# fortunalab/avida

Hardware: AMD Instinct MI355X
Metric: organism-instructions/sec + updates/sec, 1M-org logic-9 world, 1/8 GPUs (higher is better)
Workload: dtype int32; 1 GPU; configs[2]: 1024x1024 torus per GPU, logic-9, default avida.cfg mutation rates, births on, seeded with the detail-50000.pop evolved genotypes (classic instset); environment=logic9, world=1024x1024x1, burn_in_updates=150, organisms=1040165, parallelism=strips1, transport=none, ranks=1, sub_updates=0, stats_every_update=False

## Files before the change

avida_amd/csrc/births.h:

```cpp
#pragma once
#include "device.h"

namespace {

__device__ __forceinline__ int neighbours(const DevWorld& W, int cell, int* out) {
  const int X = W.world_x, R = W.rows;
  const int x = cell % X, y = cell / X;
  int n = 0;
  for (int dy = -1; dy <= 1; dy++)
    for (int dx = -1; dx <= 1; dx++) {
      if (dx == 0 && dy == 0) continue;
      int nx = x + dx, ny = y + dy;
      if (W.geometry == 1) {
        if (nx < 0 || nx >= X) continue;
      } else {
        nx = (nx + X) % X;
      }
      if (ny >= 0 && ny < R) {
        out[n++] = ny * X + nx;
      } else if (!W.tiled) {
        if (W.geometry == 1) continue;
        ny = (ny + R) % R;
        out[n++] = ny * X + nx;
      } else {
        const int gy = W.row0 + ny;
        if (W.geometry == 1 && (gy < 0 || gy >= W.global_rows)) continue;
        out[n++] = (int)W.n + (ny < 0 ? 0 : X) + nx;
      }
    }
  return n;
}

__device__ __forceinline__ void edit_back(int ew, int& src, int& val) {
  if (ew == 0 || val >= 0) return;
  const int kind = ew & 7, a = (ew >> 3) & 0xFFF, b = (ew >> 15) & 0xFFF;
  if (kind == 2) {
    if (src == a) val = b;
  } else if (kind == 3) {
    if (src == a) val = b; else if (src > a) src--;
  } else if (kind == 4) {
    if (src >= a) src++;
  }
}
__device__ __forceinline__ void slip_back(int ew, int sfm, const int32_t* fill, int& src, int& val) {
  if (ew == 0 || val >= 0) return;
  const int a = (ew >> 3) & 0xFFF, b = (ew >> 15) & 0xFFF;
  if (a > b && src >= a && src < 2 * a - b) {
    if (sfm == 4) { val = AVGPU_H_NOP_C; return; }
    if (sfm == 2 && fill) { val = fill[src - a]; return; }
    if (sfm == 3 && fill) { src = fill[src - a]; return; }
  }
  if (src >= a) src = b + (src - a);
}
__device__ __forceinline__ void trans_back(int w0, int w1, const int32_t* fill, int& src, int val) {
  if (val >= 0) return;
  const int ins = (w0 >> 3) & 0xFFF, to = (w0 >> 15) & 0xFFF, L = w1 - to;
  if (L > 0) {
    if (src >= ins + L) src -= L;
    else if (src >= ins) src = fill ? fill[src - ins] : to + (src - ins);
  } else if (L < 0 && src >= ins) {
    src -= L;
  }
}
__device__ __forceinline__ int mut_source(int j, const int* e, int sfm, int tfm, int& val, const int32_t* subs,
                                          const int* pofs, const int* pcnt) {
  constexpr int first[5] = {SEG_OSLIP, SEG_PMUT, SEG_PINS, SEG_PDEL, SEG_SMUT};
  constexpr int last[5] = {SEG_STRANS, SEG_PMUT, SEG_PINS, SEG_PDEL, SEG_SUNI};
  const bool sdata = sfm == 2 || sfm == 3;
  const int tw = tfm == 1 ? 3 : 2;
  int src = j;
  val = -1;
#pragma unroll
  for (int k = 4; k >= 0; k--) {
#pragma unroll
    for (int g = last[k]; g >= first[k]; g--) {
      if (g >= SEG_TTRANS && g <= SEG_STRANS) {
        for (int i = pcnt[g] - tw; i >= 0 && val < 0; i -= tw) {
          const int fo = tw == 3 ? subs[pofs[g] + i + 2] : -1;
          trans_back(subs[pofs[g] + i], subs[pofs[g] + i + 1], fo >= 0 ? subs + fo : nullptr, src, val);
        }
      } else if (g <= SEG_SSLIP && sdata) {
        for (int i = pcnt[g] - 2; i >= 0 && val < 0; i -= 2) {
          const int fo = subs[pofs[g] + i + 1];
          slip_back(subs[pofs[g] + i], sfm, fo >= 0 ? subs + fo : nullptr, src, val);
        }
      } else if (g <= SEG_SSLIP) {
        for (int i = pcnt[g] - 1; i >= 0 && val < 0; i--) slip_back(subs[pofs[g] + i], sfm, nullptr, src, val);
      } else {
        for (int i = pcnt[g] - 1; i >= 0 && val < 0; i--) edit_back(subs[pofs[g] + i], src, val);
      }
    }
    if (k == 0) slip_back(e[0], sfm, nullptr, src, val);
    else edit_back(e[k], src, val);
  }
  return src;
}

__device__ __forceinline__ void wave_lds_sync() {
  __builtin_amdgcn_fence(__ATOMIC_RELEASE, "workgroup");
  __builtin_amdgcn_wave_barrier();
  __builtin_amdgcn_fence(__ATOMIC_ACQUIRE, "workgroup");
}

__device__ __forceinline__ void apply_edits_core(const DevWorld& W, int64_t r, const int* e, int len0, int len,
                                                 uint8_t* child) {
  const int lane = threadIdx.x & 63;
  const int sfm = W.slip_fill_mode, tfm = W.trans_fill_mode;
  int pofs[NSEG], pcnt[NSEG], np = 0;
#pragma unroll
  for (int k = 0; k < NSEG; k++) {
    pofs[k] = W.seg_any ? W.b_pofs[(int64_t)k * W.rcap + r] : 0;
    pcnt[k] = W.seg_any ? W.b_pcnt[(int64_t)k * W.rcap + r] : 0;
    np |= pcnt[k];
  }
  if ((e[0] | e[1] | e[2] | e[3] | e[4] | np) == 0) return;
  uint32_t* g32 = reinterpret_cast<uint32_t*>(W.b_genome + r * TAPE_SLOT);
  uint32_t* c32 = reinterpret_cast<uint32_t*>(child);
  for (int w = lane; (w << 2) < len0; w += 64) c32[w] = g32[w];
  wave_lds_sync();
  for (int w = lane; (w << 2) < len; w += 64) {
    uint32_t word = 0;
#pragma unroll
    for (int k = 0; k < 4; k++) {
      const int j = 4 * w + k;
      int val;
      const int src = mut_source(j, e, sfm, tfm, val, W.b_subs, pofs, pcnt);
      const uint32_t v = val >= 0 ? (uint32_t)val : (uint32_t)child[src];
      word |= (j < len ? v : 0u) << (8 * k);
    }
    g32[w] = word;
  }
  wave_lds_sync();
}
__device__ __forceinline__ void apply_edits_wave(const DevWorld& W, int64_t r, uint8_t* child) {
  int e[5];
#pragma unroll
  for (int k = 0; k < 5; k++) e[k] = W.b_edit[(int64_t)k * W.rcap + r];
  apply_edits_core(W, r, e, W.b_len0[r], W.b_len[r], child);
}

struct Child {
  int len, gen, ccopied, exec, gest;
  double merit, fitness;
  uint32_t lo, hi, ctr;
  const int32_t* ltask;
  int64_t lstride;
  const int32_t* inputs = nullptr;
  uint32_t hs = 0;
};
template <int G>
__device__ __forceinline__ void setup_child(const DevWorld& W, int64_t c, const Child& b,
                                            const uint32_t* src, int lane) {
  static_assert(G == 32 || G == 64, "group = wave or half-wave");
  const int64_t N = W.n;
  const int len = b.len;
  uint32_t* dst = reinterpret_cast<uint32_t*>(W.tape + c * TAPE_SLOT);
  uint64_t gsum = 0;
  for (int w = lane; w < (len + 3) / 4; w += G) {
    const uint32_t v = src[w];
    dst[w] = v;
    gsum += gk_word(v, w, len);
  }
  for (int off = G / 2; off > 0; off >>= 1) gsum += __shfl_xor(gsum, off);
  if (lane == 0) W.gkey[c] = gk_final(gsum, len);
  switch (lane) {
    case 0: W.ctl[c] = CTL_ALIVE | CTL_FRESH | (b.hs << CTL_HS_SHIFT); break;
    case 1: W.mem_size[c] = len; break;
    case 2: {
      int mx = 0;
      if (W.death_method > 0) { mx = W.age_limit; if (W.death_method == 2) mx *= len; if (mx < 1) mx = 1; }
      W.max_exec[c] = mx;
      break; }
    case 3: W.birth_len[c] = len; break;
    case 4: W.merit[c] = b.merit; break;
    case 5: W.fitness[c] = b.fitness; break;
    case 6: W.credit[c] = 0.0; break;
    case 7: W.gest_time[c] = b.gest; break;
    case 8: W.generation[c] = b.gen; break;
    case 9: W.copied[c] = b.ccopied; break;
    case 10: W.executed[c] = b.exec; break;
    case 11: {
      uint32_t ctr = b.ctr;
      if (b.inputs) {
        W.inputs[c] = b.inputs[0]; W.inputs[N + c] = b.inputs[1]; W.inputs[2 * N + c] = b.inputs[2];
      } else {
        W.inputs[c] = (15 << 24) + (int)rng_below(b.lo, b.hi, ctr, 1u << 24);
        W.inputs[N + c] = (51 << 24) + (int)rng_below(b.lo, b.hi, ctr, 1u << 24);
        W.inputs[2 * N + c] = (85 << 24) + (int)rng_below(b.lo, b.hi, ctr, 1u << 24);
      }
      W.rng[c] = b.lo; W.rng[N + c] = b.hi; W.rng[2 * N + c] = ctr;
      if (W.rec_off) W.rec_off[c] = -1;
      break; }
    case 12 + AVGPU_NUM_LOGIC_TASKS: if (W.track_age) W.age[c] = 0; break;
    default:
      if (lane >= 12 && lane < 12 + AVGPU_NUM_LOGIC_TASKS)
        W.last_task[(int64_t)(lane - 12) * N + c] = b.ltask[(int64_t)(lane - 12) * b.lstride];
      break;
  }
}

__device__ __forceinline__ void child_quad(uint4 v, int k, int len, uint4* __restrict__ d4, uint64_t& gsum) {
  const int w = 4 * k;
  uint32_t x[4] = {v.x, v.y, v.z, v.w};
#pragma unroll
  for (int j = 0; j < 4; j++) {
    const int keep = len - 4 * (w + j);
    if (keep <= 0) x[j] = 0u;
    else { if (keep < 4) x[j] &= (1u << (8 * keep)) - 1u; gsum += gk_word(x[j], w + j, len); }
  }
  d4[k] = make_uint4(x[0], x[1], x[2], x[3]);
}
template <int PRE = 0>
__device__ __forceinline__ void setup_child_lane(const DevWorld& W, int64_t c, const Child& b,
                                                 const uint8_t* __restrict__ src, const uint4* pre = nullptr) {
  const int64_t N = W.n;
  const int len = b.len;
  const uint4* __restrict__ s4 = reinterpret_cast<const uint4*>(src);
  uint4* __restrict__ d4 = reinterpret_cast<uint4*>(W.tape + c * TAPE_SLOT);
  uint64_t gsum = 0;
  const int nq = (len + 15) >> 4;
#pragma unroll
  for (int u = 0; u < PRE; u++)
    if (u < nq) child_quad(pre[u], u, len, d4, gsum);
  for (int k0 = PRE; k0 < nq; k0 += 4) {
    uint4 v[4];
#pragma unroll
    for (int u = 0; u < 4; u++)
      if (k0 + u < nq) v[u] = s4[k0 + u];
#pragma unroll
    for (int u = 0; u < 4; u++) {
      if (k0 + u >= nq) break;
      child_quad(v[u], k0 + u, len, d4, gsum);
    }
  }
  W.gkey[c] = gk_final(gsum, len);
  W.ctl[c] = CTL_ALIVE | CTL_FRESH | (b.hs << CTL_HS_SHIFT);
  W.mem_size[c] = len;
  int mx = 0;
  if (W.death_method > 0) { mx = W.age_limit; if (W.death_method == 2) mx *= len; if (mx < 1) mx = 1; }
  W.max_exec[c] = mx;
  W.birth_len[c] = len;
  if (W.track_age) W.age[c] = 0;
  W.merit[c] = b.merit;
  W.fitness[c] = b.fitness;
  W.credit[c] = 0.0;
  W.gest_time[c] = b.gest;
  W.generation[c] = b.gen;
  W.copied[c] = b.ccopied;
  W.executed[c] = b.exec;
  uint32_t ctr = b.ctr;
  W.inputs[c] = (15 << 24) + (int)rng_below(b.lo, b.hi, ctr, 1u << 24);
  W.inputs[N + c] = (51 << 24) + (int)rng_below(b.lo, b.hi, ctr, 1u << 24);
  W.inputs[2 * N + c] = (85 << 24) + (int)rng_below(b.lo, b.hi, ctr, 1u << 24);
  W.rng[c] = b.lo; W.rng[N + c] = b.hi; W.rng[2 * N + c] = ctr;
  if (W.rec_off) W.rec_off[c] = -1;
#pragma unroll
  for (int q = 0; q < AVGPU_NUM_LOGIC_TASKS; q++)
    W.last_task[(int64_t)q * N + c] = b.ltask[(int64_t)q * b.lstride];
}

__device__ __forceinline__ Child child_of_record(const DevWorld& W, int64_t i) {
  Child b;
  const int4* row = reinterpret_cast<const int4*>(W.b_inh + i * BI_WORDS);
  const int4 q0 = row[0], q1 = row[1], q2 = row[2];
  static_assert(BI_MERIT == 0 && BI_GEN == 4 && BI_RLO == 8 && BI_LTASK == 12, "b_inh row layout");
  b.len = W.b_len[i];
  b.merit = __hiloint2double(q0.y, q0.x); b.fitness = __hiloint2double(q0.w, q0.z);
  b.gen = q1.x; b.ccopied = q1.y; b.exec = q1.z; b.gest = q1.w;
  b.lo = (uint32_t)q2.x; b.hi = (uint32_t)q2.y; b.ctr = (uint32_t)q2.z;
  b.hs = 0x10000u - BI_TIME(q2.w);
  b.ltask = W.b_inh + i * BI_WORDS + BI_LTASK; b.lstride = 1;
  return b;
}

}
```

avida_amd/csrc/capi.hip:

```cpp
#include <hip/hip_runtime.h>

#include <algorithm>
#include <chrono>
#include <cmath>
#include <cstdio>
#include <cstdlib>
#include <cstring>
#include <string>
#include <type_traits>
#include <vector>

#include "device.h"

namespace {

thread_local std::string g_err;

int fail(int code, const std::string& msg) {
  g_err = msg;
  return code;
}

#define HIPCHK(x)                                                                   \
  do {                                                                              \
    hipError_t _e = (x);                                                            \
    if (_e != hipSuccess) return fail(AVGPU_EHIP, std::string(#x ": ") + hipGetErrorString(_e)); \
  } while (0)
#define COPY_SYNC(ww, dst, src, bytes, kind)                                        \
  do {                                                                              \
    HIPCHK(hipMemcpyAsync((dst), (src), (bytes), (kind), (ww)->stream));           \
    HIPCHK(hipStreamSynchronize((ww)->stream));                                     \
  } while (0)
#define SET_SYNC(ww, dst, val, bytes)                                               \
  do {                                                                              \
    HIPCHK(hipMemsetAsync((dst), (val), (bytes), (ww)->stream));                    \
    HIPCHK(hipStreamSynchronize((ww)->stream));                                     \
  } while (0)

}

struct avgpu_world {
  avgpu_cfg cfg;
  int device = 0;
  hipStream_t stream = nullptr;
  hipStream_t own_stream = nullptr;
  static const int RING = 512;
  hipEvent_t ring[RING][NUM_CLASSES + 1] = {};
  int ring_head = 0, ring_count = 0;
  int time_every = 1;
  int64_t interp_calls = 0;
  double acc_ms = 0.0;
  double acc_class_ms[NUM_CLASSES] = {};
  int64_t acc_phases = 0;
  DevWorld W;
  DevWorld* d_W = nullptr;
  DevWorld* d_Wv[2] = {};
  DevWorld pushedv[2];
  bool validv[2] = {false, false};
  int cur_w = 0;
  DevWorld* h_stage = nullptr;
  hipEvent_t ev_stage[2] = {};
  std::vector<void*> allocs;
  int n_ops = 0;
  uint8_t op2code[256];
  int16_t code2op[64];
  bool instset_loaded = false;
  int res_geom[AVGPU_MAX_RESOURCES] = {};
  std::vector<avgpu_resource> res_spec;
  std::vector<avgpu_cell_resource> cell_spec;
  bool env_loaded = false;
  double* d_totals = nullptr;
  double* d_stats = nullptr;
  bool stats_stale = false;
  bool use_global = false;
  int64_t update = 0;
  float last_kernel_ms = 0.f;
  int64_t last_launches = 0;
  bool has_test_buffers = false;
  double* rec_buf = nullptr;
  double* srec_buf[2] = {nullptr, nullptr};
  int ntiles_last = 0;
  bool tile_buffers = false;
  long long* h_pred = nullptr;
  long long* d_pred = nullptr;
  bool pred_pending = false;
  long long pred_seq = 0;
  bool reaper_rebuild = false;
  long long pred_acc = 0, pred_n = 0, pred_cnt = 0;
  int last_k = 1;
  int tile_sub = 0, tile_k = 1, tile_sub_next = 0;
  uint32_t tile_key = 0;
  GtScratch gt = {};
  bool gt_ready = false;
  avgpu_genotype* gt_rows = nullptr;
  int64_t gt_rows_cap = 0;
  hipEvent_t ev_gt[4] = {};
  double gt_ms = 0.0;
  int64_t gt_bytes = 0;
  ArbScratch arb = {};
  bool arb_ready = false;
  int64_t arb_n = 0;
  avgpu_arbiter_summary arb_last = {};
  hipEvent_t ev_arb[4] = {};
  double arb_ms = 0.0;
  int64_t arb_bytes = 0;
  avgpu_world* land = nullptr;
  LandScratch land_s = {};
  int64_t land_chunk = 65536;
  hipEvent_t ev_land[2] = {};
  double land_ms = 0.0;
  int64_t land_mutants = 0, land_runs = 0;

  template <typename T>
  int alloc(T** p, size_t count) {
    void* q = nullptr;
    size_t bytes = std::max<size_t>(count * sizeof(T), 16);
    hipError_t e = hipMalloc(&q, bytes);
    if (e != hipSuccess) return fail(AVGPU_ENOMEM, std::string("hipMalloc: ") + hipGetErrorString(e));
    hipMemsetAsync(q, 0, bytes, stream);
    allocs.push_back(q);
    *p = reinterpret_cast<T*>(q);
    return 0;
  }
};

namespace {

int setup_world(avgpu_world* w, int64_t n, bool test_buffers) {
  DevWorld& W = w->W;
  memset(&W, 0, sizeof(W));
  W.n = n;
  const avgpu_cfg& c = w->cfg;
  int rc = 0;
#define A(ptr, cnt) if ((rc = w->alloc(&W.ptr, (size_t)(cnt))) < 0) return rc
  A(xs, (size_t)n * XS_WORDS); A(ctl, n); A(mem_size, n); A(max_exec, n); A(age, n); A(birth_len, n); A(gkey, n); A(rng, 3 * n);
  A(budget, n); A(aclass, n); A(tape, (size_t)n * TAPE_SLOT);
  A(inputs, 3 * n); A(last_task, AVGPU_MAX_REACTIONS * n);
  A(cur_react, AVGPU_MAX_REACTIONS * n);
  A(merit, n); A(fitness, n); A(credit, n); A(gest_time, n); A(num_div, n);
  A(generation, n); A(copied, n); A(child_copied, n); A(executed, n);
  HIPCHK(hipMemsetAsync(W.aclass, ACLASS_NONE, n, w->stream));
  A(class_list, NUM_LISTS * n); A(order, n); A(sub_hist, (size_t)((n + 4095) / 4096) * SORT_BUCKETS); A(class_count, CLASS_COUNT_WORDS); A(counters, CNT_WORDS);
  W.rcap = n + (test_buffers ? 16 : std::max<int64_t>(4096, n / 4));
  const int64_t R = W.rcap;
  A(b_count, BQ_WORDS); A(b_list, n); A(b_parent, R); A(b_seq, R); A(b_len, R); A(b_len0, R); A(b_edit, 5 * R);
  const double pmeans[5] = {c.divide_poisson_slip_mean, c.divide_poisson_mut_mean,
                            c.divide_poisson_ins_mean, c.divide_poisson_del_mean, c.divide_poisson_trans_mean};
  const double psite[6] = {c.div_mut_prob, c.div_ins_prob, c.div_del_prob, c.div_uniform_prob, c.div_slip_prob,
                           c.div_trans_prob};
  const bool sdata = c.slip_fill_mode == 2 || c.slip_fill_mode == 3, tdata = c.trans_fill_mode == 1;
  const double eslip = c.divide_slip_prob + c.divide_poisson_slip_mean + c.div_slip_prob * AVGPU_MAX_GENOME;
  const double etrans = c.divide_trans_prob + c.divide_poisson_trans_mean + c.div_trans_prob * AVGPU_MAX_GENOME;
  bool pois = false, site = c.divide_trans_prob > 0.0 || (sdata && eslip > 0.0);
  for (int q = 0; q < 5; q++) pois = pois || pmeans[q] > 0.0;
  for (int q = 0; q < 6; q++) site = site || psite[q] > 0.0;
  if (pois || site) {
    const int tw = tdata ? 3 : 2, sw = sdata ? 2 : 1;
    int64_t k = 16 + tw + sw;
    for (int q = 0; q < 6; q++)
      if (psite[q] > 0.0)
        k += (q == 5 ? tw : (q == 4 ? sw : 1)) * ((int64_t)std::ceil(AVGPU_MAX_GENOME * std::min(1.0, psite[q]) * 3.0) + 16);
    for (int q = 0; q < 5; q++)
      if (pmeans[q] > 0.0) k += (q == 4 ? tw : (q == 0 ? sw : 1)) * ((int64_t)std::ceil(3.0 * std::min(pmeans[q], 4096.0)) + 16);
    const double efill = (AVGPU_MAX_GENOME / 4.0) / 6.0 * (1.0 + 1.0 / 32.0) + 2.0;
    if (sdata && eslip > 0.0) k += (int64_t)std::ceil(3.0 * std::min(eslip, 4096.0) * efill) + 16;
    if (tdata && etrans > 0.0) k += (int64_t)std::ceil(3.0 * std::min(etrans, 4096.0) * efill) + 16;
    k = std::min<int64_t>(k, (int64_t)INT32_MAX / R);
    W.scap = R * k;
    A(b_subs, W.scap); A(b_pofs, NSEG * R); A(b_pcnt, NSEG * R);
  }
  W.seg_any = (pois || site) ? 1 : 0;
  W.pois_any = pois ? 1 : 0;
  for (int q = 0; q < 5; q++) W.pois_L[q] = pmeans[q] > 0.0 ? std::exp(-pmeans[q]) : 0.0;
  A(b_inh, (size_t)BI_WORDS * R); A(b_target, R); A(b_state, R);
  A(b_prio, R); A(b_genome, (size_t)R * TAPE_SLOT);
  const int64_t ng = n + 2 * (int64_t)c.world_x;
  A(occ, ng); A(claim, ng); A(claim2, ng); A(owner, ng); A(killt, n); A(sdone, n); A(ran, n); A(sched, SCHED_WORDS); A(pacc, NSHARD * PACC_STRIDE);
  W.claim_r[0] = W.claim; W.claim_r[1] = W.claim2;
  A(claim_r[2], ng); A(claim_r[3], ng); A(b_tgt, 4 * R);
  if (c.birth_method == 4) {
    A(e_list, n); A(e_blk, (n + 255) / 256 + 1); A(soup_perm, n);
    std::vector<int32_t> iota((size_t)n);
    for (int64_t i = 0; i < n; i++) iota[(size_t)i] = (int32_t)i;
    HIPCHK(hipMemcpyAsync(W.soup_perm, iota.data(), (size_t)n * sizeof(int32_t), hipMemcpyHostToDevice,
                          w->stream));
    HIPCHK(hipStreamSynchronize(w->stream));
  }
  if (test_buffers) {
    A(t_flags, (size_t)n * TAPE_SLOT); A(t_flags_len, n); A(t_child, (size_t)n * TAPE_SLOT);
    A(t_child_len, n);
  }
  A(rand_cum, 64); A(rand_code, 64); A(task_lut, 256); A(rand_lut, 256);
  A(react_tab, AVGPU_MAX_REACTIONS * RT_STRIDE); A(task_tab, 32);
  A(react_res, AVGPU_MAX_REACTIONS * RR_STRIDE); A(res_param, AVGPU_MAX_RESOURCES);
  A(res_global, AVGPU_MAX_RESOURCES); A(res_cons, AVGPU_MAX_RESOURCES);
  if ((rc = w->alloc(&w->d_Wv[0], 1)) || (rc = w->alloc(&w->d_Wv[1], 1))) return rc;
  w->d_W = w->d_Wv[0];
  w->validv[0] = w->validv[1] = false;
  const int64_t nb = (n + 255) / 256;
  if ((rc = w->alloc(&w->d_totals, (size_t)totals_words(nb)))) return rc;
  W.totals = w->d_totals;
  if ((rc = w->alloc(&W.blk_count, (size_t)nb))) return rc;
  W.tree_cap = 1;
  while (W.tree_cap < nb) W.tree_cap <<= 1;
  if ((rc = w->alloc(&W.tree_scr, (size_t)(2 * W.tree_cap)))) return rc;
  if ((rc = w->alloc(&W.tree_cnt, (size_t)(2 * W.tree_cap)))) return rc;
  if ((rc = w->alloc(&w->d_stats, (size_t)stats_words(nb)))) return rc;
#undef A
  w->has_test_buffers = test_buffers;
  W.world_x = c.world_x; W.world_y = c.world_y; W.geometry = c.world_geometry;
  W.ave_time_slice = c.ave_time_slice; W.slicing = c.slicing_method;
  W.base_merit_method = c.base_merit_method; W.base_const_merit = c.base_const_merit;
  W.default_bonus = c.default_bonus; W.size_range = c.offspring_size_range;
  W.min_copied_lines = c.min_copied_lines; W.min_exe_lines = c.min_exe_lines;
  W.merit_default_bonus = c.merit_default_bonus; W.required_bonus = c.required_bonus;
  W.inherit_merit = c.inherit_merit; W.require_allocate = c.require_allocate;
  W.alloc_method = c.alloc_method; W.max_label_exe = c.max_label_exe_size;
  W.cfg_min_genome = c.min_genome_size; W.cfg_max_genome = c.max_genome_size;
  W.max_genome = (!c.max_genome_size || c.max_genome_size > AVGPU_MAX_GENOME) ? AVGPU_MAX_GENOME : c.max_genome_size;
  W.min_genome = (!c.min_genome_size || c.min_genome_size < AVGPU_MIN_GENOME) ? AVGPU_MIN_GENOME : c.min_genome_size;
  W.death_method = c.death_method; W.age_limit = c.age_limit;
  W.prefer_empty = c.prefer_empty; W.allow_parent = c.allow_parent; W.birth_method = c.birth_method;
  auto th = [](double p) -> uint64_t {
    if (!(p > 0.0)) return 0;
    if (p >= 1.0) return 1ull << 32;
    return (uint64_t)std::ceil(p * 4294967296.0);
  };
  W.th_copy_mut = th(c.copy_mut_prob);
  W.th_copy_ins = th(c.copy_ins_prob); W.p_copy_ins = c.copy_ins_prob;
  W.th_copy_del = th(c.copy_del_prob); W.p_copy_del = c.copy_del_prob;
  W.th_copy_uni = th(c.copy_uniform_prob); W.p_copy_uni = c.copy_uniform_prob;
  W.th_copy_slip = th(c.copy_slip_prob); W.p_copy_slip = c.copy_slip_prob;
  W.copy_ext = (W.th_copy_ins || W.th_copy_del || W.th_copy_uni || W.th_copy_slip) ? 1 : 0;
  W.th_div_mut = th(c.divide_mut_prob);
  W.th_div_ins = th(c.divide_ins_prob);
  W.th_div_del = th(c.divide_del_prob);
  W.th_div_slip = th(c.divide_slip_prob);
  W.th_div_uni = th(c.divide_uniform_prob);
  W.p_copy_mut = c.copy_mut_prob; W.p_div_mut = c.divide_mut_prob; W.p_div_ins = c.divide_ins_prob;
  W.p_div_del = c.divide_del_prob; W.p_div_slip = c.divide_slip_prob; W.p_div_uni = c.divide_uniform_prob;
  W.th_div_site = th(c.div_mut_prob);
  W.p_div_site = c.div_mut_prob;
  W.th_dsite[0] = th(c.div_ins_prob); W.p_dsite[0] = c.div_ins_prob;
  W.th_dsite[1] = th(c.div_del_prob); W.p_dsite[1] = c.div_del_prob;
  W.th_dsite[2] = th(c.div_uniform_prob); W.p_dsite[2] = c.div_uniform_prob;
  W.th_dsite[3] = th(c.div_slip_prob); W.p_dsite[3] = c.div_slip_prob;
  W.th_dsite[4] = th(c.div_trans_prob); W.p_dsite[4] = c.div_trans_prob;
  W.th_dtrans = th(c.divide_trans_prob); W.p_dtrans = c.divide_trans_prob;
  W.th_par_site = th(c.parent_mut_prob);
  W.p_par_site = c.parent_mut_prob;
  W.th_par_ins = th(c.parent_ins_prob); W.p_par_ins = c.parent_ins_prob;
  W.th_par_del = th(c.parent_del_prob); W.p_par_del = c.parent_del_prob;
  W.slip_fill_mode = c.slip_fill_mode;
  W.trans_fill_mode = c.trans_fill_mode;
  W.slip_copy_mode = c.slip_copy_mode;
  W.track_age = (c.birth_method == 1 || c.birth_method == 2) ? 1 : 0;
  W.rec = nullptr; W.rec_n = 0; W.rec_off = nullptr;
  W.seed_lo = (uint32_t)c.seed;
  W.seed_hi = (uint32_t)(c.seed >> 32);
  W.slow_batch = env_int("AVGPU_SLOW_BATCH", 12, 1, 64);
  W.nb_slow_batch = env_int("AVGPU_NB_SLOW_BATCH", 1, 1, 64);
  W.ioq_slow_batch = env_int("AVGPU_IOQ_SLOW_BATCH", 6, 1, 64);
  W.row0 = 0;
  W.global_rows = c.world_y;
  W.rows = c.world_y;
  W.tiled = 0;
  W.cell0 = 0;
  static const int sets[9][6] = {
      {15, 51, 85, -1, -1, -1}, {63, 95, 119, -1, -1, -1}, {136, 160, 192, -1, -1, -1},
      {175, 187, 207, 221, 243, 245}, {238, 250, 252, -1, -1, -1}, {10, 12, 34, 48, 68, 80},
      {3, 5, 17, -1, -1, -1}, {60, 90, 102, -1, -1, -1}, {153, 165, 195, -1, -1, -1}};
  uint16_t lut[256] = {0};
  for (int t = 0; t < 9; t++)
    for (int k = 0; k < 6; k++)
      if (sets[t][k] >= 0) lut[sets[t][k]] |= (uint16_t)(1u << t);
  HIPCHK(hipMemcpyAsync(W.task_lut, lut, sizeof(lut), hipMemcpyHostToDevice, w->stream));
  HIPCHK(hipStreamSynchronize(w->stream));
  return 0;
}

std::string unsupported_cfg(const avgpu_cfg& c) {
  auto nz = [](double v) { return v != 0.0; };
  const bool slips = nz(c.divide_slip_prob) || nz(c.divide_poisson_slip_mean) || nz(c.div_slip_prob);
  if (slips && (c.slip_fill_mode < 0 || c.slip_fill_mode == 1 || c.slip_fill_mode > 4))
    return "SLIP_FILL_MODE 1 (nop-X) or an unknown mode";
  if (nz(c.copy_slip_prob) && c.slip_copy_mode != 0 && c.slip_copy_mode != 1)
    return "SLIP_COPY_MODE other than 0 (read-head jump) and 1 (memory slip)";
  if (nz(c.copy_slip_prob) && c.slip_copy_mode == 1 && c.slip_fill_mode != 0 && c.slip_fill_mode != 2 &&
      c.slip_fill_mode != 4)
    return "SLIP_COPY_MODE 1 with SLIP_FILL_MODE other than 0 (duplication), 2 (random), 4 (nop-C)";
  if ((nz(c.divide_trans_prob) || nz(c.divide_poisson_trans_mean) || nz(c.div_trans_prob)) &&
      (c.trans_fill_mode < 0 || c.trans_fill_mode > 1))
    return "TRANS_FILL_MODE other than 0 (duplication) / 1 (scrambled)";
  if (c.divide_poisson_slip_mean > 700.0 || c.divide_poisson_mut_mean > 700.0 ||
      c.divide_poisson_ins_mean > 700.0 || c.divide_poisson_del_mean > 700.0 ||
      c.divide_poisson_trans_mean > 700.0)
    return "DIVIDE_POISSON_*_MEAN above 700 (exp(-mean) underflows)";
  if (c.divide_method != 1) return "DIVIDE_METHOD other than 1 (split)";
  if (c.sub_updates < 0 || c.sub_updates > 64) return "sub_updates outside 0..64";
  if (c.sub_updates > 1 && c.slicing_method != 1) return "sub_updates > 1 with SLICING_METHOD other than 1";
  if (c.world_geometry != 1 && c.world_geometry != 2) return "WORLD_GEOMETRY other than 1 (grid) or 2 (torus)";
  if (c.slicing_method < 0 || c.slicing_method > 2) return "SLICING_METHOD other than 0, 1, 2";
  if (c.base_merit_method < 0 || c.base_merit_method > 5) return "BASE_MERIT_METHOD other than 0..5";
  if (c.birth_method < 0 || c.birth_method > 5)
    return "BIRTH_METHOD other than 0 (random neighbour), 1 (oldest), 2 (highest age / merit), 3 (empty only), "
           "4 (whole-world soup), 5 (eldest, serial world)";
  if ((c.birth_method == 1 || c.birth_method == 2) && !c.prefer_empty)
    return "BIRTH_METHOD 1 / 2 without PREFER_EMPTY (the reference reads the organism of an empty cell)";
  if (c.death_method < 0 || c.death_method > 2) return "DEATH_METHOD other than 0, 1, 2";
  if (c.alloc_method != 0 && c.alloc_method != 2) return "ALLOC_METHOD other than 0 (default) and 2 (random)";
  if (nz(c.point_mut_prob) || nz(c.point_ins_prob) || nz(c.point_del_prob) || nz(c.inst_point_mut_prob))
    return "POINT_MUT_PROB / POINT_INS_PROB / POINT_DEL_PROB / INST_POINT_MUT_PROB (cosmic-ray mutations)";
  if (nz(c.div_lgt_prob) || nz(c.divide_lgt_prob) || nz(c.divide_poisson_lgt_mean))
    return "DIV_LGT_PROB / DIVIDE_LGT_PROB / DIVIDE_POISSON_LGT_MEAN (lateral gene transfer)";
  if (nz(c.inject_mut_prob) || nz(c.inject_ins_prob) || nz(c.inject_del_prob)) return "INJECT_*_PROB";
  if (nz(c.meta_copy_mut) || nz(c.meta_std_dev)) return "META_COPY_MUT / META_STD_DEV";
  if (nz(c.death_prob)) return "DEATH_PROB";
  if (c.age_deviation != 0) return "AGE_DEVIATION";
  if (c.divide_failure_resets != 0) return "DIVIDE_FAILURE_RESETS";
  if (c.special_mut_line >= 0) return "SPECIAL_MUT_LINE";
  if (c.population_cap > 0) return "POPULATION_CAP";
  if (c.generation_inc_method != 1) return "GENERATION_INC_METHOD other than 1";
  if (c.reset_inputs_on_divide != 0) return "RESET_INPUTS_ON_DIVIDE";
  if (c.epigenetic_method != 0) return "EPIGENETIC_METHOD";
  if (c.min_cycles != 0) return "MIN_CYCLES";
  if (c.required_task < -1 || c.immunity_task < -1 || c.required_reaction < -1 || c.immunity_reaction < -1 ||
      c.required_task >= AVGPU_MAX_REACTIONS || c.immunity_task >= AVGPU_MAX_REACTIONS ||
      c.required_reaction >= 12 || c.immunity_reaction >= 12)
    return "REQUIRED_TASK / IMMUNITY_TASK outside the task library, REQUIRED_REACTION / IMMUNITY_REACTION "
           "beyond reaction 11";
  if (c.require_exact_copy != 0) return "REQUIRE_EXACT_COPY";
  if (c.fitness_method != 0) return "FITNESS_METHOD other than 0";
  if (c.juv_period != 0) return "JUV_PERIOD";
  if (c.no_mut_insts_len < 0 || c.no_mut_insts_len > 63 ||
      (size_t)c.no_mut_insts_len != strnlen(c.no_mut_insts, sizeof(c.no_mut_insts)))
    return "NO_MUT_INSTS longer than 63 symbols, or no_mut_insts_len not its length";
  if (c.test_fitness_measures != 0) return "REVERT_* / STERILIZE_* (Divide_TestFitnessMeasures1)";
  return std::string();
}

avgpu_world* create_world(const avgpu_cfg* cfg, int device, int64_t n, bool test_buffers) {
  if (!cfg) { fail(AVGPU_EINVAL, "cfg is NULL"); return nullptr; }
  {
    const std::string why = unsupported_cfg(*cfg);
    if (!why.empty()) {
      fail(AVGPU_EUNSUPPORTED, why + " is not on the GPU path");
      return nullptr;
    }
  }
  if (hipSetDevice(device) != hipSuccess) { fail(AVGPU_EHIP, "hipSetDevice failed"); return nullptr; }
  avgpu_world* w = new avgpu_world();
  w->cfg = *cfg;
  w->device = device;
  if (n <= 0) n = (int64_t)cfg->world_x * cfg->world_y;
  if (n <= 0 || n > (1ll << 30)) { delete w; fail(AVGPU_EINVAL, "bad cell count"); return nullptr; }
  if (hipStreamCreateWithFlags(&w->own_stream, hipStreamNonBlocking) != hipSuccess ||
      hipHostMalloc((void**)&w->h_pred, PRED_WORDS * sizeof(long long), hipHostMallocMapped | hipHostMallocCoherent) !=
          hipSuccess ||
      hipHostMalloc((void**)&w->h_stage, 2 * sizeof(DevWorld), hipHostMallocDefault) != hipSuccess ||
      hipEventCreateWithFlags(&w->ev_stage[0], hipEventDisableTiming) != hipSuccess ||
      hipEventCreateWithFlags(&w->ev_stage[1], hipEventDisableTiming) != hipSuccess ||
      hipHostGetDevicePointer((void**)&w->d_pred, w->h_pred, 0) != hipSuccess) {
    delete w; fail(AVGPU_EHIP, "stream/event creation failed"); return nullptr;
  }
  for (int k = 0; k < PRED_WORDS; k++) w->h_pred[k] = 0;
  w->stream = w->own_stream;
  for (int i = 0; i < avgpu_world::RING; i++) {
    for (int k = 0; k <= NUM_CLASSES; k++)
      if (hipEventCreate(&w->ring[i][k]) != hipSuccess) {
        fail(AVGPU_EHIP, "event creation failed"); return nullptr;
      }
  }
  for (int i = 0; i < 64; i++) w->code2op[i] = -1;
  if (setup_world(w, n, test_buffers) < 0) {
    std::string e = g_err;
    avgpu_destroy(w);
    g_err = e;
    return nullptr;
  }
  return w;
}

int copy_tables(avgpu_world* dst, const avgpu_world* src) {
  DevWorld& D = dst->W;
  const DevWorld& S = src->W;
  D.n_ops = S.n_ops; D.rand_total = S.rand_total; D.fill_code = S.fill_code;
  D.n_react = S.n_react;
  D.env_simple = S.env_simple; D.env_react_mask = S.env_react_mask; D.env_once_mask = S.env_once_mask;
  D.no_mut_mask = S.no_mut_mask;
  D.req_task = S.req_task; D.imm_task = S.imm_task; D.req_react = S.req_react; D.imm_react = S.imm_react;
  D.single_react = S.single_react; D.max_task_cnt = S.max_task_cnt; D.div_req = S.div_req;
  HIPCHK(hipStreamSynchronize(src->stream));
  HIPCHK(hipMemcpyAsync(D.task_tab, S.task_tab, 32 * sizeof(double), hipMemcpyDeviceToDevice, dst->stream));
  HIPCHK(hipMemcpyAsync(D.react_tab, S.react_tab, AVGPU_MAX_REACTIONS * RT_STRIDE * sizeof(int32_t),
                        hipMemcpyDeviceToDevice, dst->stream));
  HIPCHK(hipMemcpyAsync(D.rand_lut, S.rand_lut, 256, hipMemcpyDeviceToDevice, dst->stream));
  HIPCHK(hipMemcpyAsync(D.rand_cum, S.rand_cum, 64 * sizeof(int32_t), hipMemcpyDeviceToDevice, dst->stream));
  HIPCHK(hipMemcpyAsync(D.rand_code, S.rand_code, 64, hipMemcpyDeviceToDevice, dst->stream));
  HIPCHK(hipStreamSynchronize(dst->stream));
  dst->n_ops = src->n_ops;
  memcpy(dst->op2code, src->op2code, sizeof(dst->op2code));
  memcpy(dst->code2op, src->code2op, sizeof(dst->code2op));
  dst->instset_loaded = src->instset_loaded;
  dst->env_loaded = src->env_loaded;
  return 0;
}

int ready(avgpu_world* w) {
  if (!w) return fail(AVGPU_EINVAL, "NULL world");
  if (!w->instset_loaded) return fail(AVGPU_ESTATE, "avgpu_load_instset not called");
  if (!w->env_loaded) return fail(AVGPU_ESTATE, "avgpu_load_env not called");
  return 0;
}

int batch_ready(avgpu_world* w) {
  const int rc = ready(w);
  if (rc < 0) return rc;
  if (w->cfg.birth_method == 5)
    return fail(AVGPU_EUNSUPPORTED, "BIRTH_METHOD 5 (the reaper queue) runs on the serial world only");
  return 0;
}

int translate_genomes(avgpu_world* w, const uint8_t* genomes, const int32_t* lens, int64_t count,
                      std::vector<uint8_t>& codes, std::vector<int32_t>& offsets) {
  codes.clear();
  offsets.resize(count);
  size_t off = 0;
  for (int64_t i = 0; i < count; i++) {
    const int len = lens[i];
    if (len < 1 || len > AVGPU_MAX_GENOME) return fail(AVGPU_EINVAL, "genome length out of range");
    offsets[i] = (int32_t)codes.size();
    for (int k = 0; k < len; k++) {
      const uint8_t op = genomes[off + k];
      if (op >= w->n_ops) return fail(AVGPU_EINVAL, "genome op outside instruction set");
      codes.push_back(w->op2code[op]);
    }
    off += len;
    while (codes.size() & 3) codes.push_back(0);
  }
  if (codes.empty()) codes.push_back(0);
  return 0;
}

int reaper_read(avgpu_world* w, std::vector<int32_t>& q) {
  const DevWorld& W = w->W;
  int64_t ix[2];
  COPY_SYNC(w, ix, W.reaper_ix, sizeof(ix), hipMemcpyDeviceToHost);
  std::vector<int32_t> ring((size_t)W.reaper_cap);
  COPY_SYNC(w, ring.data(), W.reaper, ring.size() * sizeof(int32_t), hipMemcpyDeviceToHost);
  if (ix[1] < ix[0] || ix[1] - ix[0] > W.reaper_cap) return fail(AVGPU_ESTATE, "reaper queue indices");
  q.clear();
  for (int64_t p = ix[0]; p < ix[1]; p++) q.push_back(ring[(size_t)(p % W.reaper_cap)]);
  return 0;
}
int reaper_write(avgpu_world* w, const std::vector<int32_t>& q) {
  const DevWorld& W = w->W;
  if ((int64_t)q.size() > W.reaper_cap) return fail(AVGPU_EUNSUPPORTED, "reaper queue longer than 2n + 64");
  std::vector<int32_t> ring((size_t)W.reaper_cap, 0);
  std::copy(q.begin(), q.end(), ring.begin());
  const int64_t ix[2] = {W.reaper_cap, W.reaper_cap + (int64_t)q.size()};
  COPY_SYNC(w, W.reaper, ring.data(), ring.size() * sizeof(int32_t), hipMemcpyHostToDevice);
  COPY_SYNC(w, W.reaper_ix, ix, sizeof(ix), hipMemcpyHostToDevice);
  return 0;
}

int reaper_build(avgpu_world* w) {
  const DevWorld& W = w->W;
  std::vector<uint32_t> ctl((size_t)W.n);
  COPY_SYNC(w, ctl.data(), W.ctl, (size_t)W.n * sizeof(uint32_t), hipMemcpyDeviceToHost);
  std::vector<int32_t> q;
  for (int64_t c = 0; c < W.n; c++) q.push_back((int32_t)c);
  for (int64_t c = 0; c < W.n; c++) if (ctl[(size_t)c] & CTL_ALIVE) q.push_back((int32_t)c);
  w->reaper_rebuild = false;
  return reaper_write(w, q);
}

int set_orgs_impl(avgpu_world* w, int64_t first, int64_t count, const uint8_t* genomes,
                  const int32_t* lens, const double* merits, const int32_t* inputs, int det) {
// ... 1982 lines not shown
```

avida_amd/csrc/device.h:

```cpp
#pragma once

#include <hip/hip_runtime.h>
#include <stdint.h>
#include <stdlib.h>

#include "../../include/avida_gpu.h"

#define TAPE_SLOT 2048
enum { BI_MERIT = 0, BI_FITNESS = 2, BI_GEN = 4, BI_CCOPIED = 5, BI_EXEC = 6, BI_GEST = 7,
       BI_RLO = 8, BI_RHI = 9, BI_RCTR = 10, BI_FINAL = 11, BI_LTASK = 12, BI_WORDS = 32 };
#define BI_TIME(w) ((uint32_t)(w) >> 16)
#define CODE_MASK 0x3F
#define TF_COPIED 0x40
#define TF_EXEC 0x80
#define CODE_ERROR 0x3F

#define CTL_SP0(c) ((c) & 0xF)
#define CTL_SP1(c) (((c) >> 4) & 0xF)
#define CTL_CURSTK 0x100u
#define CTL_MAL 0x200u
#define CTL_ALIVE 0x400u
#define CTL_FRESH 0x800u
#define CTL_SPECDIE 0x1000u
#define CTL_HS_SHIFT 14
#define CTL_HS(c) (((c) >> CTL_HS_SHIFT) & 0x1FFFFu)
#define CTL_HS_MASK (0x1FFFFu << CTL_HS_SHIFT)

#define NUM_CLASSES 4
#define ACLASS_NONE 0xFF
#define RR_STRIDE 8
enum { RR_RES = 0, RR_SPATIAL = 1, RR_DEPL = 2, RR_TYPE = 3, RR_FRAC = 4, RR_MIN = 5, RR_MAX = 6, RR_VALUE = 7 };
#define RES_FIX 4294967296.0

struct ResParam {
  int32_t geometry, slot;
  int32_t in_x1, in_x2, in_y1, in_y2, out_x1, out_x2, out_y1, out_y2;
  double in_share;
  double sink_frac;
  double xdiffuse, ydiffuse, xgravity, ygravity;
  double decay100, inflow100;
  double decay99, inflow99;
  int32_t flows, has_sink;
  int32_t in_all, out_all;
};
#define NUM_LISTS 7
#define RT_STRIDE 12
enum { RT_TASK = 0, RT_TYPE = 1, RT_MIN = 2, RT_MAX = 3, RT_HASREQ = 4, RT_USED = 5, RT_MULT = 6, RT_ADD = 8 };
#define BUDGET_PRIM 0x40000000

enum : int {
  XS_REG = 0,
  XS_HEAD = 3,
  XS_RLABEL = 7,
  XS_CYCLES = 8,
  XS_TIME = 9,
  XS_GEST = 10,
  XS_ERRORS = 11,
  XS_INBUF = 12,
  XS_INTOT = 15,
  XS_INPTR = 16,
  XS_OUTBUF = 17,
  XS_OUTTOT = 18,
  XS_BONUS = 20,
  XS_TASK = 22,
  XS_STACK = 32,
  XS_REACT = 52,
  XS_NREACT = 12,
  XS_WORDS = 64
};

struct DevWorld {
  int64_t n;
  int32_t* xs;
  uint32_t* ctl;
  int32_t* mem_size;
  int32_t* max_exec;
  int32_t* birth_len;
  uint64_t* gkey;
  uint32_t* rng;
  int32_t* budget;
  uint8_t* aclass;
  uint8_t* tape;
  int32_t* inputs;
  int32_t* last_task;
  int32_t* cur_react;
  double* merit;
  double* fitness;
  double* credit;
  int32_t* gest_time;
  int32_t* num_div;
  int32_t* generation;
  int32_t* copied;
  int32_t* child_copied;
  int32_t* executed;
  int32_t* class_list;
  int32_t* order;
  int32_t* class_count;
  unsigned long long* counters;
  int64_t rcap;
  int32_t* b_count;
  int32_t* b_list;
  int32_t* b_parent;
  uint32_t* b_seq;
  int32_t* b_len;
  int32_t* b_len0;
  int32_t* b_edit;
  int32_t* b_subs;
  int64_t scap;
  int32_t* b_pofs;
  int32_t* b_pcnt;
  int32_t* b_inh;
  int32_t* b_target;
  int8_t* b_state;
  unsigned long long* b_prio;
  uint8_t* b_genome;
  uint8_t* occ;
  unsigned long long* claim;
  unsigned long long* claim2;
  unsigned long long* claim_r[4];
  int32_t* b_tgt;
  int32_t* owner;
  uint32_t* killt;
  int64_t* blk_count;
  double* tree_scr;
  int64_t* tree_cnt;
  int64_t tree_cap;
  int32_t* sdone;
  uint8_t* t_flags;
  int32_t* t_flags_len;
  uint8_t* t_child;
  int32_t* t_child_len;
  int32_t* rand_cum;
  uint8_t* rand_code;
  uint16_t* task_lut;
  int n_ops;
  int32_t rand_total;
  uint8_t* rand_lut;
  int32_t slow_batch;
  int32_t nb_slow_batch;
  int32_t ioq_slow_batch;
  int n_react;
  int32_t* react_tab;
  int32_t env_simple;
  uint32_t env_react_mask;
  uint32_t env_once_mask;
  uint32_t env_res_mask;
  double* task_tab;
  int32_t n_res, n_cellres, env_resources;
  struct ResParam* res_param;
  double* res_amount;
  double* res_delta;
  double* res_global;
  unsigned long long* res_cons;
  avgpu_cell_resource* res_cells;
  double* react_res;
  int8_t res_spatial_host[AVGPU_MAX_RESOURCES];
  int8_t res_flows_host[AVGPU_MAX_RESOURCES];
  int8_t res_cells_host[AVGPU_MAX_RESOURCES];
  int8_t res_grav_host[AVGPU_MAX_RESOURCES];
  double* res_amount_alt;
  int8_t res_first;
  int32_t n_spatial;
  double* rs_send[2];
  double* rs_recv[2];
  uint8_t fill_code;
  int32_t world_x, world_y, geometry;
  int32_t ave_time_slice, slicing;
  int32_t base_merit_method, base_const_merit;
  double default_bonus, size_range, min_copied_lines, min_exe_lines;
  double merit_default_bonus, required_bonus;
  int32_t inherit_merit, require_allocate, alloc_method, max_label_exe;
  int32_t min_genome, max_genome;
  int32_t cfg_min_genome, cfg_max_genome;
  int32_t death_method, age_limit;
  int32_t prefer_empty, allow_parent, birth_method;
  uint64_t th_copy_mut, th_div_mut, th_div_ins, th_div_del, th_div_slip, th_div_uni;
  double p_copy_mut, p_div_mut, p_div_ins, p_div_del, p_div_slip, p_div_uni;
  uint64_t th_copy_ins, th_copy_del, th_copy_uni, th_copy_slip;
  double p_copy_ins, p_copy_del, p_copy_uni, p_copy_slip;
  int32_t copy_ext;
  uint64_t no_mut_mask;
  int32_t req_task, imm_task, req_react, imm_react, single_react, max_task_cnt, div_req;
  uint64_t th_div_site;
  double p_div_site;
  uint64_t th_par_site;
  double p_par_site;
  uint64_t th_par_ins, th_par_del;
  double p_par_ins, p_par_del;
  double pois_L[5];
  int32_t pois_any;
  uint64_t th_dsite[5];
  double p_dsite[5];
  uint64_t th_dtrans;
  double p_dtrans;
  int32_t seg_any;
  int32_t slip_fill_mode;
  int32_t trans_fill_mode;
  int32_t slip_copy_mode;
  const double* rec;
  int64_t rec_n;
  int64_t* rec_off;
  double* stree;
  int64_t stree_size;
  int32_t* spec;
  uint32_t* grng;
  uint32_t* sctx;
  uint8_t* face;
  const double* srec_sched;
  int64_t srec_sched_n;
  const double* srec_ctx;
  int64_t srec_ctx_n;
  uint32_t seed_lo, seed_hi;
  int32_t row0, global_rows, rows, tiled;
  int64_t cell0;
  uint8_t* h_send[2];
  uint8_t* h_recv[2];
  uint8_t* r_send[2];
  uint8_t* r_recv[2];
  int64_t r_arena;
  int32_t* age;
  int32_t track_age;
  int32_t* sub_hist;
  int32_t* e_list;
  int32_t* e_blk;
  int32_t* soup_perm;
  int32_t* reaper;
  int64_t* reaper_ix;
  int64_t reaper_cap;
  int32_t* ran;
  double* cons;
  long long* sched;
  long long* pacc;
  const double* totals;
};
static_assert(sizeof(DevWorld) == 1664, "DevWorld's size");


enum {
  TOT_WEIGHT = 0,
  TOT_ORGS = 1,
  TOT_HANDED = 2,
  TOT_DIV = 2,
  TOT_UD = 3,
  TOT_WORDS = 8
};
__host__ __device__ inline int64_t totals_words(int64_t nb) { return TOT_WORDS + 2 * nb; }

enum {
  SCHED_CARRY = 1,
  SCHED_CARRY_REM = 2,
  SCHED_UD = 4,
  SCHED_WORDS = 12
};

enum {
  PACC_WEIGHT = 0,
  PACC_Q01 = 1,
  PACC_Q23 = 2
};

enum {
  TAIL_PRED = 0,
  TAIL_CARRY = 1,
  TAIL_QUARTER0 = 2,
  TAIL_WORDS = 6
};
static_assert(TAIL_QUARTER0 + 4 == TAIL_WORDS, "a strip's tail ends with the four quarter counts");
__host__ __device__ inline int64_t tile_tail_off(int64_t nb) { return 2 * nb; }
__host__ __device__ inline int64_t tile_part_stride(int64_t nb) { return tile_tail_off(nb) + TAIL_WORDS; }

enum {
  PRED_ACC = 0,
  PRED_ORGS = 1,
  PRED_DENSEST = 2,
  PRED_SEQ = 3,
  PRED_WORDS = 4
};

enum {
  BQ_PRIMARY = 0,
  BQ_OVERFLOW = 1,
  BQ_SUBS = 2,
  BQ_WORDS = 3
};
enum { LIST_NEWBORN = 0, LIST_SPILL = 3, CLASS_COUNT_WORDS = 8 };
static_assert(NUM_LISTS <= CLASS_COUNT_WORDS, "a length per list row");

#define RES_DELTA_TAIL 64
__host__ __device__ inline int64_t res_delta_words(int64_t n) { return n + RES_DELTA_TAIL; }

enum {
  ST_ORGS = 0,
  ST_MERIT = 1,
  ST_FITNESS = 2,
  ST_GESTATION = 3,
  ST_GENOME_LEN = 4,
  ST_MAX_FITNESS = 5,
  ST_GENERATION = 6,
  ST_MEM_SIZE = 7,
  ST_TASK0 = 8,
  NUSED = ST_TASK0 + AVGPU_NUM_LOGIC_TASKS,
  NPART = 24,
  ST_INSTS = 24,
  ST_DEATHS = 25,
  ST_DIVIDES = 26,
  ST_BIRTHS = 27,
  ST_DROPPED = 28,
  ST_SPILLS = 29,
  ST_CUM_INSTS = 30,
  ST_CUM_BIRTHS = 31,
  ST_SLICES = 32,
  ST_LANESTEPS = 33,
  ST_OVERWRITTEN = 34,
  ST_CANCELLED = 35,
  ST_WASTED = 36,
  ST_PRED = 37,
  ST_CARRY = 38,
  ST_PRED_ORGS = 39,
  ST_PRED_DENSEST = 40,
  ST_QUARTER0 = 41,
  NSTAT = 45
};
static_assert(NUSED <= NPART, "k_stats_partial's rows");
static_assert(ST_INSTS == NPART, "the counters follow the partial sums");
static_assert(ST_CUM_BIRTHS == ST_CUM_INSTS + 1, "avgpu_set_clock writes the pair");
static_assert(ST_QUARTER0 + 4 == NSTAT, "the statistics vector ends with the four quarter counts");
__host__ __device__ inline int64_t stats_words(int64_t nb) { return NSTAT + (int64_t)NPART * nb; }

enum {
  RESET_NONE = 0,
  RESET_COUNTS = 1,
  RESET_QUEUES = 2
};
enum {
  BC_OWN = 0,
  BC_GATHERED = 1,
  BC_HANDED_IN = 2,
  BC_TOTALS_ONLY = 3
};
enum { ACT_WORLD = 1 , ACT_STRIP = 2  };
enum { TP_ROUND = 0, TP_CLAIM0 = 3, TP_PACK = 1, TP_ACTIVATE = 2 };
enum {
  KI_SORTED = 1,
  KI_PRED = 2
};
#define REMOTE_OWNER(k, t) (-2 - ((k) + 4 * (int)(t)))
__host__ __device__ inline int64_t halo_kt_off(int x) { return ((int64_t)x * 33 + 3) / 4 * 4; }
__host__ __device__ inline int64_t halo_bytes(int x) { return (halo_kt_off(x) + 4 * (int64_t)x + 15) / 16 * 16; }
struct HaloHdr { int32_t count, arena_used, overflow, pad; };
struct HaloRec {
  int32_t col, round, len, gen, ccopied, exec, gest;
  uint32_t rng_lo, rng_hi, rng_ctr;
  int32_t off;
  uint32_t t;
  double merit, fitness;
  int32_t last_task[AVGPU_NUM_LOGIC_TASKS], pad2[3];
};
__host__ __device__ inline int64_t record_bytes(int x, int64_t arena) {
  return (int64_t)sizeof(HaloHdr) + (int64_t)x * (int64_t)sizeof(HaloRec) + arena;
}

enum { SEG_OSLIP = 0, SEG_PSLIP, SEG_SSLIP, SEG_TTRANS, SEG_PTRANS, SEG_STRANS, SEG_PMUT, SEG_PINS, SEG_PDEL, SEG_SMUT, SEG_SINS, SEG_SDEL, SEG_SUNI, NSEG };
#define NSHARD 64
#define CNT_STRIDE 64
#define CNT_CUM_BASE (NSHARD * CNT_STRIDE)
#define CNT_WORDS (NSHARD * CNT_STRIDE + CNT_STRIDE)
#define PACC_STRIDE 8
__device__ __forceinline__ long long pacc_sum(const DevWorld& W, int k) {
  long long s = 0;
  for (int sh = 0; sh < NSHARD; sh++) s += W.pacc[sh * PACC_STRIDE + k];
  return s;
}
__device__ __forceinline__ long long quarter_count(const DevWorld& W, int k) {
  return (long long)(((unsigned long long)pacc_sum(W, PACC_Q01 + (k >> 1)) >> (32 * (k & 1))) & 0xFFFFFFFFull);
}
__device__ __forceinline__ long long densest_quarter(const DevWorld& W) {
  return max(max(quarter_count(W, 0), quarter_count(W, 1)), max(quarter_count(W, 2), quarter_count(W, 3)));
}
#define CNT_CUM_INSTS (CNT_CUM_BASE + AVGPU_CNT_INSTS)
#define CNT_CUM_BIRTHS (CNT_CUM_BASE + AVGPU_CNT_BIRTHS)
#define CNT_CUM_FLAG (CNT_CUM_BASE + CNT_STRIDE - 1)

__device__ __forceinline__ int queue_len(const DevWorld& W) {
  const int64_t n = (int64_t)W.b_count[BQ_PRIMARY] + (int64_t)min(W.b_count[BQ_OVERFLOW], (int)(W.rcap - W.n));
  return (int)n;
}
__device__ __forceinline__ int64_t rec_of(const DevWorld& W, int64_t i) {
  const int p = W.b_count[BQ_PRIMARY];
  return i < p ? (int64_t)W.b_list[i] : W.n + (i - p);
}

__device__ __forceinline__ void st_async_u32(void* p, uint32_t v) {
  asm volatile("global_store_dword %0, %1, off\n\ts_waitcnt expcnt(0)" ::"v"(p), "v"(v));
}
__device__ __forceinline__ void st_async_u64(void* p, uint64_t v) {
  asm volatile("global_store_dwordx2 %0, %1, off\n\ts_waitcnt expcnt(0)" ::"v"(p), "v"(v));
}
__device__ __forceinline__ uint32_t ld_sync_u32(const void* p) {
  uint32_t v;
  asm volatile("global_load_dword %0, %1, off\n\ts_waitcnt vmcnt(0)" : "=v"(v) : "v"(p) : "memory");
  return v;
}
__device__ __forceinline__ uint32_t ld_sync_u8(const void* p) {
  uint32_t v;
  asm volatile("global_load_ubyte %0, %1, off\n\ts_waitcnt vmcnt(0)" : "=v"(v) : "v"(p) : "memory");
  return v;
}
__device__ __forceinline__ uint32_t ld_sync_ro_u32(const void* p) {
  uint32_t v;
  asm volatile("global_load_dword %0, %1, off\n\ts_waitcnt vmcnt(0)" : "=v"(v) : "v"(p));
  return v;
}
__device__ __forceinline__ uint32_t ld_sync_ro_u8(const void* p) {
  uint32_t v;
  asm volatile("global_load_ubyte %0, %1, off\n\ts_waitcnt vmcnt(0)" : "=v"(v) : "v"(p));
  return v;
}
typedef const __attribute__((address_space(4))) double const_f64_t;
__device__ __forceinline__ double ld_uniform_f64(const double* p) {
  return *(const_f64_t*)p;
}
__device__ __forceinline__ uint32_t sgather_u8(const uint8_t* tab, uint32_t idx) {
  uint32_t out = 0;
  bool todo = true;
  while (todo) {
    const uint32_t u = __builtin_amdgcn_readfirstlane(idx);
    if (idx == u) {
      const uint64_t a = (uint64_t)(tab + (u & ~3u));
      const uint64_t sa = ((uint64_t)(uint32_t)__builtin_amdgcn_readfirstlane((int)(uint32_t)(a >> 32)) << 32) |
                          (uint64_t)(uint32_t)__builtin_amdgcn_readfirstlane((int)(uint32_t)a);
      uint32_t w;
      asm volatile("s_load_dword %0, %1, 0x0\n\ts_waitcnt lgkmcnt(0)" : "=s"(w) : "s"(sa));
      out = (w >> ((u & 3u) * 8u)) & 0xFFu;
      todo = false;
    }
  }
  return out;
}
__device__ __forceinline__ void st_async_b128(void* p, uint32_t a, uint32_t b, uint32_t c, uint32_t d) {
  typedef uint32_t u32x4 __attribute__((ext_vector_type(4)));
  const u32x4 v = {a, b, c, d};
  asm volatile("global_store_dwordx4 %0, %1, off\n\ts_waitcnt expcnt(0)\n\ts_nop 2" ::"v"(p), "v"(v));
}
__device__ __forceinline__ void st_async_u8(void* p, uint32_t v) {
  asm volatile("global_store_byte %0, %1, off\n\ts_waitcnt expcnt(0)" ::"v"(p), "v"(v));
}

__host__ __device__ __forceinline__ uint32_t lowbias32(uint32_t x) {
  x ^= x >> 16; x *= 0x7feb352dU; x ^= x >> 15; x *= 0x846ca68bU; x ^= x >> 16;
  return x;
}
__device__ __forceinline__ uint32_t rng_next(uint32_t lo, uint32_t hi, uint32_t& ctr) {
  uint32_t a = lowbias32(ctr * 0x9E3779B9U + hi);
  uint32_t b = lowbias32(a ^ lo);
  ++ctr;
  return b;
}
__device__ __forceinline__ uint32_t rng_below(uint32_t lo, uint32_t hi, uint32_t& ctr, uint32_t n) {
  return (uint32_t)(((uint64_t)rng_next(lo, hi, ctr) * n) >> 32);
}
__device__ __forceinline__ bool rng_p(uint32_t lo, uint32_t hi, uint32_t& ctr, uint64_t th) {
  return (uint64_t)rng_next(lo, hi, ctr) < th;
}
__host__ __device__ __forceinline__ void derive_key(uint32_t a_lo, uint32_t a_hi, uint32_t x, uint32_t y,
                                                    uint32_t& lo, uint32_t& hi) {
  lo = lowbias32(lowbias32(x ^ a_lo) + y);
  hi = lowbias32(lowbias32(y ^ a_hi) + x + 0x632BE5ABU);
}

__device__ __forceinline__ uint64_t gk_mix(uint64_t z) {
  z ^= z >> 30; z *= 0xBF58476D1CE4E5B9ull;
  z ^= z >> 27; z *= 0x94D049BB133111EBull;
  return z ^ (z >> 31);
}
__device__ __forceinline__ uint64_t gk_word(uint32_t word, int w, int len) {
  word &= 0x3F3F3F3Fu;
  const int keep = len - 4 * w;
  if (keep < 4) word &= (1u << (8 * keep)) - 1u;
  return gk_mix(((uint64_t)(w + 1) << 32) | word);
}
__device__ __forceinline__ uint64_t gk_final(uint64_t sum, int len) {
  const uint64_t k = gk_mix(sum ^ ((uint64_t)len * 0x9E3779B97F4A7C15ull));
  return k ? k : 1ull;
}
__device__ __forceinline__ uint64_t gk_tape(const uint8_t* t, int len) {
  uint64_t s = 0;
  for (int w = 0; w < (len + 3) / 4; w++) {
    uint32_t v = 0;
    for (int j = 0; j < 4 && 4 * w + j < len; j++) v |= (uint32_t)t[4 * w + j] << (8 * j);
    s += gk_word(v, w, len);
  }
  return gk_final(s, len);
}

__device__ __forceinline__ int head_adjust(int pos, int size) {
  const bool out = (unsigned)pos >= (unsigned)size;
  if (__builtin_expect(__ballot(out) != 0ull, 0)) {
    if (out) pos = pos < 0 ? 0 : (pos < 2 * size ? pos - size : pos % size);
  }
  return pos;
}
__device__ __forceinline__ int head_wrap(int pos, int size) {
  return (unsigned)pos < (unsigned)size ? pos : pos - size;
}

__device__ __forceinline__ uint8_t random_code(const DevWorld& W, uint32_t lo, uint32_t hi,
                                               uint32_t& ctr) {
  uint32_t r = rng_below(lo, hi, ctr, (uint32_t)W.rand_total);
  int i = 0;
  while (i < W.n_ops - 1 && W.rand_cum[i] <= (int32_t)r) i++;
  return W.rand_code[i];
}

__device__ __forceinline__ double det_exp2(double x) {
  const double n = floor(x);
  const double t = __dmul_rn(__dsub_rn(x, n), 0.6931471805599453094);
  double y = 1.0;
  for (int k = 22; k >= 1; k--) y = __dadd_rn(1.0, __dmul_rn(y, __ddiv_rn(t, (double)k)));
  return ldexp(y, (int)n);
}

__device__ __forceinline__ double pow_int(double q, int64_t n) {
  double r = 1.0, b = q;
  while (n) { if (n & 1) r = __dmul_rn(r, b); b = __dmul_rn(b, b); n >>= 1; }
  return r;
}
__constant__ const double INV_K[65] = {0.0,
  1.0 / 1, 1.0 / 2, 1.0 / 3, 1.0 / 4, 1.0 / 5, 1.0 / 6, 1.0 / 7, 1.0 / 8, 1.0 / 9, 1.0 / 10, 1.0 / 11, 1.0 / 12,
  1.0 / 13, 1.0 / 14, 1.0 / 15, 1.0 / 16, 1.0 / 17, 1.0 / 18, 1.0 / 19, 1.0 / 20, 1.0 / 21, 1.0 / 22, 1.0 / 23,
  1.0 / 24, 1.0 / 25, 1.0 / 26, 1.0 / 27, 1.0 / 28, 1.0 / 29, 1.0 / 30, 1.0 / 31, 1.0 / 32, 1.0 / 33, 1.0 / 34,
  1.0 / 35, 1.0 / 36, 1.0 / 37, 1.0 / 38, 1.0 / 39, 1.0 / 40, 1.0 / 41, 1.0 / 42, 1.0 / 43, 1.0 / 44, 1.0 / 45,
  1.0 / 46, 1.0 / 47, 1.0 / 48, 1.0 / 49, 1.0 / 50, 1.0 / 51, 1.0 / 52, 1.0 / 53, 1.0 / 54, 1.0 / 55, 1.0 / 56,
  1.0 / 57, 1.0 / 58, 1.0 / 59, 1.0 / 60, 1.0 / 61, 1.0 / 62, 1.0 / 63, 1.0 / 64};
__device__ __forceinline__ int64_t binom_draw(int64_t n, double p, uint32_t h) {
  if (n <= 0 || !(p > 0.0)) return 0;
  if (p >= 1.0) return n;
  const bool flip = p > 0.5;
  const double pp = flip ? __dsub_rn(1.0, p) : p, q = __dsub_rn(1.0, pp);
  const double mean = __dmul_rn((double)n, pp);
  int64_t k;
  if (mean < 6.0) {
    const double u = __dmul_rn(__dadd_rn((double)h, 0.5), 2.3283064365386962890625e-10);
    const double r = __ddiv_rn(pp, q);
    double f = pow_int(q, n);
    double F = f;
    k = 0;
    while (F < u && k < n && k < 64) {
      f = __dmul_rn(__dmul_rn(f, __dmul_rn((double)(n - k), r)), INV_K[k + 1]);
      k++;
      F = __dadd_rn(F, f);
    }
  } else {
    uint32_t x = lowbias32(h + 0x9E3779B9U);
    uint32_t sum = (x & 0xFFFFu) + (x >> 16);
    x = lowbias32(x + 0x9E3779B9U);
    sum += (x & 0xFFFFu) + (x >> 16);
    const double z = __dmul_rn(__dsub_rn(__dmul_rn(__dadd_rn((double)sum, 2.0), 1.52587890625e-05), 2.0),
                               1.7320508075688772);
    const double sd = __dsqrt_rn(__dmul_rn(mean, q));
    const double skew = __dmul_rn(__dmul_rn(__dsub_rn(q, pp), __dsub_rn(__dmul_rn(z, z), 1.0)), 0.16666666666666666);
    const double v = __dadd_rn(__dadd_rn(__dadd_rn(mean, __dmul_rn(sd, z)), skew), 0.5);
    k = v < 1.0 ? 0 : (int64_t)floor(v);
    if (k > n) k = n;
  }
  return flip ? n - k : k;
}
#define SALT_TOP 0x7A11C0DEu
#define SALT_BLOCK 0x51CEB10Cu
#define SALT_NEWBORN 0x4E3B0A17u
__device__ __forceinline__ uint32_t node_draw(uint32_t slo, uint32_t shi, uint32_t update, uint32_t salt,
                                              uint64_t node) {
  return lowbias32(lowbias32(lowbias32(update * 0x85EBCA6BU + shi) ^ (uint32_t)node ^ salt) +
                   (uint32_t)(node >> 32) + slo);
}
__device__ __forceinline__ bool merit_ok(double m) { return m >= 0.0 && m <= 1.7976931348623157e308; }
#define WEIGHT_CAP 0x1p990
__device__ __forceinline__ double sched_weight(double merit, uint32_t ctl) {
  if (!merit_ok(merit)) return 0.0;
  const uint32_t hs = CTL_HS(ctl);
  const double w = hs ? __dmul_rn(merit, __dadd_rn(1.0, __dmul_rn((double)hs, 1.0 / 65536.0))) : merit;
  return merit_ok(w) ? fmin(w, WEIGHT_CAP) : 0.0;
}

__device__ __forceinline__ int size_merit(int method, int base_const, int glen, int copied, int exe) {
  int s;
  switch (method) {
// ... 234 lines not shown
```

avida_amd/csrc/interp.hip:

```cpp
#include <cstdlib>

#include "device.h"
#include "births.h"

#pragma clang fp contract(off)

namespace {

#define OPB(x) (1u << (x))
constexpr uint32_t MOD_OPS =
    OPB(AVGPU_H_IF_N_EQU) | OPB(AVGPU_H_IF_LESS) | OPB(AVGPU_H_POP) | OPB(AVGPU_H_PUSH) |
    OPB(AVGPU_H_SWAP) | OPB(AVGPU_H_SHIFT_R) | OPB(AVGPU_H_SHIFT_L) | OPB(AVGPU_H_INC) |
    OPB(AVGPU_H_DEC) | OPB(AVGPU_H_ADD) | OPB(AVGPU_H_SUB) | OPB(AVGPU_H_NAND) | OPB(AVGPU_H_IO) |
    OPB(AVGPU_H_MOV_HEAD) | OPB(AVGPU_H_JMP_HEAD) | OPB(AVGPU_H_GET_HEAD) | OPB(AVGPU_H_SET_FLOW);
constexpr uint64_t DEF_OPS =
    (1ull << (2 * AVGPU_H_IF_N_EQU)) | (1ull << (2 * AVGPU_H_IF_LESS)) | (1ull << (2 * AVGPU_H_POP)) |
    (1ull << (2 * AVGPU_H_PUSH)) | (1ull << (2 * AVGPU_H_SWAP)) | (1ull << (2 * AVGPU_H_SHIFT_R)) |
    (1ull << (2 * AVGPU_H_SHIFT_L)) | (1ull << (2 * AVGPU_H_INC)) | (1ull << (2 * AVGPU_H_DEC)) |
    (1ull << (2 * AVGPU_H_ADD)) | (1ull << (2 * AVGPU_H_SUB)) | (1ull << (2 * AVGPU_H_NAND)) |
    (1ull << (2 * AVGPU_H_IO)) | (2ull << (2 * AVGPU_H_SET_FLOW));
constexpr uint32_t FAST_OPS =
    OPB(AVGPU_H_NOP_A) | OPB(AVGPU_H_NOP_B) | OPB(AVGPU_H_NOP_C) | OPB(AVGPU_H_IF_N_EQU) |
    OPB(AVGPU_H_IF_LESS) | OPB(AVGPU_H_SWAP_STK) | OPB(AVGPU_H_SWAP) | OPB(AVGPU_H_SHIFT_R) |
    OPB(AVGPU_H_SHIFT_L) | OPB(AVGPU_H_INC) | OPB(AVGPU_H_DEC) | OPB(AVGPU_H_ADD) |
// ... 1092 lines not shown
            gs = tu;
            dnd = nd;
            const int gen = dgen + 1;
            dgen = gen;
            didv = true;
            errs = 0;
            bonus = p_defb;
            cyc = 0;
            nzm = 0;
#pragma unroll
            for (int i = 0; i < AVGPU_MAX_REACTIONS; i++) rc[i] = i < k_n_react ? 0 : rc[i];
            len = child;
            if (mode == AVGPU_MODE_TEST) {
              st_async_u32(W.t_flags_len + cell, (uint32_t)div);
              st_async_u32(W.t_child_len + cell, (uint32_t)child);
              fl |= F_STOP;
            } else {
              uint64_t t_slip = W.th_div_slip, t_mut = W.th_div_mut, t_ins = W.th_div_ins;
              uint64_t t_del = W.th_div_del, t_uni = DEF ? 0ull : W.th_div_uni;
              double q_slip = W.p_div_slip, q_mut = W.p_div_mut, q_ins = W.p_div_ins;
              double q_del = W.p_div_del, q_uni = W.p_div_uni;
              int g_max = W.max_genome, g_min = W.min_genome;
              OPQ(t_slip); OPQ(t_mut); OPQ(t_ins); OPQ(t_del);
              if (!DEF) OPQ(t_uni);
              OPQ(q_slip); OPQ(q_mut); OPQ(q_ins); OPQ(q_del); OPQ(q_uni); OPQ(g_max); OPQ(g_min);
              const bool segs = !DEF && W.seg_any;
              int lmax = len;
              const bool pois = !DEF && W.pois_any;
              auto draw_u = [&]() -> double {
                if (REC && rbase) return rd();
                return (double)rng_next(klo, khi, kct) * 2.3283064365386963e-10;
              };
              auto npois = [&](int k) -> int {
                const double Lk = W.pois_L[k];
                if (!(Lk > 0.0)) return 0;
                double x = draw_u();
                int n = 0;
                while (x >= Lk && n < 4096) { x = __dmul_rn(x, draw_u()); n++; }
                return n;
              };
              auto nbinom = [&](uint64_t th, double p) -> int {
                int n = 0;
                for (int i = 0; i < len; i++) n += draw_p(th, p) ? 1 : 0;
                return n;
              };
              auto preserve = [&](int k, int n) {
                if (n > 0 && mode == AVGPU_MODE_WORLD)
                  pofs[k] = (int64_t)__atomic_load_n(W.b_count + BQ_SUBS, __ATOMIC_RELAXED) >= W.scap
                                ? (int)W.scap : atomicAdd(W.b_count + BQ_SUBS, n);
              };
              auto pput = [&](int k, int i, int ew) {
                if (mode == AVGPU_MODE_WORLD && pofs[k] >= 0 && (int64_t)pofs[k] + i < W.scap) W.b_subs[pofs[k] + i] = ew;
              };
              const int sfm = DEF ? 0 : W.slip_fill_mode, tfm = DEF ? 0 : W.trans_fill_mode;
              const bool sdata = sfm == 2 || sfm == 3, tdata = tfm == 1;
              bool ftrunc = false;
              auto fill_draws = [&](int kind, int L, int to, int ins_loc) -> int {
                if (L <= 0) return -1;
                const int nbw = kind == 2 ? 0 : (L + 31) >> 5;
                int off = -1;
                if (mode == AVGPU_MODE_WORLD) {
                  if ((int64_t)__atomic_load_n(W.b_count + BQ_SUBS, __ATOMIC_RELAXED) < W.scap) {
                    const int o = atomicAdd(W.b_count + BQ_SUBS, L + nbw);
                    if ((int64_t)o + L + nbw <= W.scap) off = o;
                  }
                  if (off < 0) ftrunc = true;
                }
                int32_t* f = off >= 0 ? W.b_subs + off : nullptr;
                uint32_t* bits = f ? reinterpret_cast<uint32_t*>(f + L) : nullptr;
                if (bits)
                  for (int q = 0; q < nbw; q++) bits[q] = 0u;
                for (int i = 0; i < L; i++) {
                  if (kind == 2) {
                    const int v = rand_code();
                    if (f) f[i] = v;
                    continue;
                  }
                  int rem = (int)draw_below((uint32_t)(L - i));
                  if (!f) continue;
                  int wd = 0;
                  while (true) {
                    const int fr = 32 - __popc(bits[wd]);
                    if (rem < fr) break;
                    rem -= fr;
                    wd++;
                  }
                  uint32_t z = ~bits[wd];
                  for (int q = 0; q < rem; q++) z &= z - 1u;
                  const int bit = __ffs((int)z) - 1;
                  bits[wd] |= 1u << bit;
                  int src = to + wd * 32 + bit;
                  if (kind == 5 && src >= ins_loc && src < ins_loc + i) src = f[src - ins_loc];
                  f[i] = src;
                }
                return off;
              };
              auto slip_edit = [&](int k, int i) {
                const int from = (int)draw_below((uint32_t)len + 1u);
                const int to = from == 0 ? (int)draw_below((uint32_t)len) : (int)draw_below((uint32_t)len + 1u);
                if (sdata) {
                  const int fo = fill_draws(sfm, from - to, to, 0);
                  pput(k, 2 * i, edit_word(E_SLIP, from, to));
                  pput(k, 2 * i + 1, fo);
                } else {
                  pput(k, i, edit_word(E_SLIP, from, to));
                }
                len += from - to;
                lmax = max(lmax, len);
              };
              const int sw = sdata ? 2 : 1, tw = tdata ? 3 : 2;
              auto uniform_edit = [&]() -> int {
                const int mut = (int)draw_below((uint32_t)(2 * k_n_ops + 1));
                int ew = 0;
                if (mut < k_n_ops) {
                  ew = edit_word(E_POINT, (int)draw_below((uint32_t)len), (int)tab_u8(rcode + mut));
                } else if (mut == k_n_ops) {
                  if (len != g_min) { ew = edit_word(E_DEL, (int)draw_below((uint32_t)len), 0); len--; }
                } else if (len != g_max) {
                  ew = edit_word(E_INS, (int)draw_below((uint32_t)len + 1u), (int)tab_u8(rcode + mut - k_n_ops - 1));
                  len++;
                  lmax = max(lmax, len);
                }
                return ew;
              };
              if (draw_p(t_slip, q_slip)) {
                if (segs && sdata) {
                  preserve(SEG_OSLIP, 2);
                  slip_edit(SEG_OSLIP, 0);
                  pcnt[SEG_OSLIP] = 2;
                } else {
                  const int from = (int)draw_below((uint32_t)len + 1u);
                  const int to = from == 0 ? (int)draw_below((uint32_t)len) : (int)draw_below((uint32_t)len + 1u);
                  if (sdata) fill_draws(sfm, from - to, to, 0);
                  e0 = edit_word(E_SLIP, from, to);
                  len += from - to;
                  lmax = max(lmax, len);
                }
              }
              if (pois) {
                const int n = npois(0);
                preserve(SEG_PSLIP, sw * n);
                for (int i = 0; i < n; i++) slip_edit(SEG_PSLIP, i);
                pcnt[SEG_PSLIP] = sw * n;
              }
              if (segs && W.th_dsite[3]) {
                const int n = nbinom(W.th_dsite[3], W.p_dsite[3]);
                preserve(SEG_SSLIP, sw * n);
                for (int i = 0; i < n; i++) slip_edit(SEG_SSLIP, i);
                pcnt[SEG_SSLIP] = sw * n;
              }
              auto trans_edit = [&](int k, int i) {
                const int from = (int)draw_below((uint32_t)len + 1u);
                const int to = from == 0 ? (int)draw_below((uint32_t)len) : (int)draw_below((uint32_t)len + 1u);
                const int ins_loc = (int)draw_below((uint32_t)len + 1u);
                pput(k, tw * i, edit_word(E_TRANS, ins_loc, to));
                pput(k, tw * i + 1, from);
                if (tdata) pput(k, tw * i + 2, fill_draws(5, from - to, to, ins_loc));
                len += from - to;
                lmax = max(lmax, len);
              };
              if (segs && W.th_dtrans && draw_p(W.th_dtrans, W.p_dtrans)) {
                preserve(SEG_TTRANS, tw);
                trans_edit(SEG_TTRANS, 0);
                pcnt[SEG_TTRANS] = tw;
              }
              if (pois) {
                const int n = npois(4);
                preserve(SEG_PTRANS, tw * n);
                for (int i = 0; i < n; i++) trans_edit(SEG_PTRANS, i);
                pcnt[SEG_PTRANS] = tw * n;
              }
              if (segs && W.th_dsite[4]) {
                const int n = nbinom(W.th_dsite[4], W.p_dsite[4]);
                preserve(SEG_STRANS, tw * n);
                for (int i = 0; i < n; i++) trans_edit(SEG_STRANS, i);
                pcnt[SEG_STRANS] = tw * n;
              }
              if (draw_p(t_mut, q_mut)) {
                const int line = (int)draw_below((uint32_t)len);
                e1 = edit_word(E_POINT, line, rand_code());
              }
              if (pois) {
                const int n = npois(1);
                preserve(SEG_PMUT, n);
                for (int i = 0; i < n; i++) {
                  const int line = (int)draw_below((uint32_t)len);
                  pput(SEG_PMUT, i, edit_word(E_POINT, line, rand_code()));
                }
                pcnt[SEG_PMUT] = n;
              }
              if (draw_p(t_ins, q_ins) && len < g_max) {
                const int line = (int)draw_below((uint32_t)len + 1u);
                e2 = edit_word(E_INS, line, rand_code());
                len++;
                lmax = max(lmax, len);
              }
              if (pois) {
                const int n = npois(2);
                preserve(SEG_PINS, n);
                int used = 0;
                for (int i = 0; i < n && len < g_max; i++) {
                  const int line = (int)draw_below((uint32_t)len + 1u);
                  pput(SEG_PINS, i, edit_word(E_INS, line, rand_code()));
                  len++;
                  lmax = max(lmax, len);
                  used++;
                }
                pcnt[SEG_PINS] = used;
              }
              if (draw_p(t_del, q_del) && len > g_min) {
                e3 = edit_word(E_DEL, (int)draw_below((uint32_t)len), 0);
                len--;
              }
              if (pois) {
                const int n = npois(3);
                preserve(SEG_PDEL, n);
                int used = 0;
                for (int i = 0; i < n && len > g_min; i++) {
                  pput(SEG_PDEL, i, edit_word(E_DEL, (int)draw_below((uint32_t)len), 0));
                  len--;
                  used++;
                }
                pcnt[SEG_PDEL] = used;
              }
              if (t_uni && draw_p(t_uni, q_uni)) e4 = uniform_edit();
              if (segs && W.th_div_site) {
                const int n = nbinom(W.th_div_site, W.p_div_site);
                preserve(SEG_SMUT, n);
                for (int i = 0; i < n; i++) {
                  const int site = (int)draw_below((uint32_t)len);
                  pput(SEG_SMUT, i, edit_word(E_POINT, site, rand_code()));
                }
                pcnt[SEG_SMUT] = n;
              }
              if (segs && W.th_dsite[0]) {
                int n = nbinom(W.th_dsite[0], W.p_dsite[0]);
                if (n + len > g_max) n = g_max - len;
                if (n > 0) {
                  preserve(SEG_SINS, n);
                  const bool keep = mode == AVGPU_MODE_WORLD && (int64_t)pofs[SEG_SINS] + n <= W.scap;
                  int32_t* seg = W.b_subs + pofs[SEG_SINS];
                  for (int i = 0; i < n; i++) {
                    const int site = (int)draw_below((uint32_t)len + 1u);
                    if (keep) {
                      int j = i;
                      while (j > 0 && seg[j - 1] < site) { seg[j] = seg[j - 1]; j--; }
                      seg[j] = site;
                    }
                  }
                  for (int i = 0; i < n; i++) {
                    const int code = rand_code();
                    if (keep) seg[i] = edit_word(E_INS, seg[i], code);
                  }
                  len += n;
                  lmax = max(lmax, len);
                  pcnt[SEG_SINS] = n;
                }
              }
              if (segs && W.th_dsite[1]) {
                int n = nbinom(W.th_dsite[1], W.p_dsite[1]);
                if (len - n < g_min) n = len - g_min;
                if (n > 0) {
                  preserve(SEG_SDEL, n);
                  for (int i = 0; i < n; i++) {
                    pput(SEG_SDEL, i, edit_word(E_DEL, (int)draw_below((uint32_t)len), 0));
                    len--;
                  }
                  pcnt[SEG_SDEL] = n;
                }
              }
              if (segs && W.th_dsite[2]) {
                const int n = nbinom(W.th_dsite[2], W.p_dsite[2]);
                preserve(SEG_SUNI, n);
                for (int i = 0; i < n; i++) pput(SEG_SUNI, i, uniform_edit());
                pcnt[SEG_SUNI] = n;
              }
              bool truncated = false;
              if (ftrunc) { count_add(W, AVGPU_CNT_SUB_OVERFLOW, 1ull); truncated = true; }
              if (segs && mode == AVGPU_MODE_WORLD)
#pragma unroll
                for (int k = 0; k < NSEG; k++)
                  if (pcnt[k] > 0 && ((int64_t)pofs[k] < 0 || (int64_t)pofs[k] + pcnt[k] > W.scap)) {
                    count_add(W, AVGPU_CNT_SUB_OVERFLOW, (unsigned long long)pcnt[k]);
                    truncated = true;
                  }
              if (mode == AVGPU_MODE_WORLD && (len > AVGPU_MAX_GENOME || lmax > 4095)) {
                ndrop++;
                noversize++;
              } else if (mode == AVGPU_MODE_WORLD && truncated) {
                ndrop++;
              } else if (mode == AVGPU_MODE_WORLD) {
              rec = cell;
              if (prim) {
                rec = (int)min((int64_t)W.n + atomicAdd(W.b_count + BQ_OVERFLOW, 1), W.rcap);
                if (rec >= W.rcap) { rec = -1; ndrop++; }
              }
              prim = true;
              }
              if (serial && rec >= 0) sbirth = 1;
              if (defer && rec < 0) parent_phenotype();
              if (rec >= 0) {
                uint32_t clo = 0u, chi = 0u;
                if (!defer) derive_key(olo, ohi, (uint32_t)nd, 0x1B873593U, clo, chi);
                int32_t* b_parent = W.b_parent;
                uint32_t* b_seq = W.b_seq;
                int32_t* b_len = W.b_len;
                int32_t* b_len0 = W.b_len0;
                int32_t* b_edit = W.b_edit;
                int8_t* b_state = W.b_state;
                int32_t* b_target = W.b_target;
                int32_t* b_inh = W.b_inh;
                int64_t rcap = W.rcap;
                OPQ(b_parent); OPQ(b_seq); OPQ(b_len); OPQ(b_len0); OPQ(b_edit);
                OPQ(b_state); OPQ(b_target); OPQ(b_inh); OPQ(rcap);
                st_async_u32(b_parent + rec, (uint32_t)cell);
                st_async_u32(b_seq + rec, (uint32_t)nd);
                st_async_u32(b_len + rec, (uint32_t)len);
                st_async_u32(b_len0 + rec, (uint32_t)child);
                st_async_u32(b_edit + rec, (uint32_t)e0);
                st_async_u32(b_edit + rcap + rec, (uint32_t)e1);
                st_async_u32(b_edit + 2 * rcap + rec, (uint32_t)e2);
                st_async_u32(b_edit + 3 * rcap + rec, (uint32_t)e3);
                st_async_u32(b_edit + 4 * rcap + rec, (uint32_t)e4);
                if (!DEF && W.seg_any)
#pragma unroll
                  for (int k = 0; k < NSEG; k++) {
                    W.b_pofs[(int64_t)k * rcap + rec] = pofs[k];
                    W.b_pcnt[(int64_t)k * rcap + rec] = pcnt[k];
                  }
                int32_t* irow = b_inh + (int64_t)rec * BI_WORDS;
                const long long mb = __double_as_longlong(merit);
                const long long fb = defer ? 0ll : __double_as_longlong(__ddiv_rn(__dmul_rn(base, bon), (double)gt));
                st_async_b128(irow, (uint32_t)mb, (uint32_t)(mb >> 32), (uint32_t)fb, (uint32_t)(fb >> 32));
                st_async_b128(irow + 4, (uint32_t)gen, (uint32_t)cop, (uint32_t)exe, (uint32_t)gt);
                const int kdone = sdone + executed;
                const uint32_t tb = (uint32_t)__ddiv_rn(__dmul_rn((double)kdone, 65536.0),
                                                        (double)((int64_t)kdone + budget + 1));
                st_async_b128(irow + 8, clo, chi, 0u, (defer ? 1u : 0u) | (tb << 16));
                st_async_b128(irow + 12, (uint32_t)tc[0], (uint32_t)tc[1], (uint32_t)tc[2], (uint32_t)tc[3]);
                st_async_b128(irow + 16, (uint32_t)tc[4], (uint32_t)tc[5], (uint32_t)tc[6], (uint32_t)tc[7]);
                st_async_b128(irow + 20, (uint32_t)tc[8], 0u, 0u, 0u);
                st_async_u8(b_state + rec, 0u);
                st_async_u32(b_target + rec, 0xFFFFFFFFu);
              }
            }
#pragma unroll
            for (int q = 0; q < AVGPU_NUM_LOGIC_TASKS; q++) tc[q] = 0;
            divides++;
            M = div;
            r0 = r1 = r2 = 0;
            ip = rh = wh = fh = 0;
            ctl = CTL_ALIVE;
            rl = 0;
            adv = false;
          }
        }
        okw = __shfl(okw, L);
        if (okw) {
          rec = __shfl(rec, L); len = __shfl(len, L);
          const int cell_l = __shfl(cell, L);
          if (mode == AVGPU_MODE_TEST) {
            uint8_t* fl = W.t_flags + (int64_t)cell_l * TAPE_SLOT;
            uint8_t* ch = W.t_child + (int64_t)cell_l * TAPE_SLOT;
            for (int w = lane; (w << 2) < div; w += 64) {
              uint32_t wd = 0;
#pragma unroll
              for (int q = 0; q < 4; q++)
                wd |= (uint32_t)((TL[4 * w + q] & TF_EXEC) ? '+' : '-') << (8 * q);
              st_async_u32(fl + 4 * w, wd);
            }
            for (int w = lane; (w << 2) < child; w += 64) {
              uint32_t wd = 0;
#pragma unroll
              for (int q = 0; q < 4; q++) wd |= (uint32_t)(TL[div + 4 * w + q] & CODE_MASK) << (8 * q);
              st_async_u32(ch + 4 * w, wd);
            }
          } else if (mode == AVGPU_MODE_WORLD && rec >= 0) {
            uint8_t* g = W.b_genome + (int64_t)rec * TAPE_SLOT;
            const uint32_t dsh = (uint32_t)(div & 3) * 8u;
            for (int w = lane; (w << 2) < child; w += 64) {
              const int a = (div >> 2) + w;
              const uint32_t lo = TL32[a], hi = TL32[a + 1];
              const uint32_t v = dsh ? ((lo >> dsh) | (hi << (32u - dsh))) : lo;
              st_async_u32(g + 4 * w, v & 0x3F3F3F3Fu & byte_mask(w << 2, 0, child));
            }
          }
          if (!DEF && mode != AVGPU_MODE_TEST && lane == L && (W.th_par_site || W.th_par_ins || W.th_par_del)) {
            int g_max = W.max_genome, g_min = W.min_genome;
            if (W.th_par_site) {
              int npar = 0;
              for (int i = 0; i < M; i++) npar += draw_p(W.th_par_site, W.p_par_site) ? 1 : 0;
              for (int i = 0; i < npar; i++) {
                const int site = (int)draw_below((uint32_t)M);
                T[site] = (uint8_t)((T[site] & ~CODE_MASK) | rand_code());
              }
            }
            if (W.th_par_ins) {
              int nins = 0;
              for (int i = 0; i < M; i++) nins += draw_p(W.th_par_ins, W.p_par_ins) ? 1 : 0;
              if (nins + M > g_max) nins = g_max - M;
              const int nfit = (Scap - M) / 5;
              if (nins > nfit) {
                count_add(W, AVGPU_CNT_MEM_CAP, (unsigned long long)(nins - nfit));
                nins = nfit;
              }
              if (nins > 0) {
                int32_t* srt = reinterpret_cast<int32_t*>(T + Scap - 4 * nins);
                for (int i = 0; i < nins; i++) {
                  const int site = (int)draw_below((uint32_t)M + 1u);
                  int j = i;
                  while (j > 0 && srt[j - 1] > site) { srt[j] = srt[j - 1]; j--; }
                  srt[j] = site;
                }
                for (int i = nins - 1; i >= 0; i--) {
                  const int pos = srt[i];
                  const int code = rand_code();
                  for (int k = M; k > pos; k--) T[k] = T[k - 1];
                  T[pos] = (uint8_t)code;
                  M++;
                }
              }
            }
            if (W.th_par_del) {
              int ndel = 0;
              for (int i = 0; i < M; i++) ndel += draw_p(W.th_par_del, W.p_par_del) ? 1 : 0;
              if (M - ndel < g_min) ndel = M - g_min;
              for (int i = 0; i < ndel; i++) {
                const int site = (int)draw_below((uint32_t)M);
                for (int k = site; k < M - 1; k++) T[k] = T[k + 1];
                M--;
              }
            }
          }
          const int pmem = __shfl(M, L);
          for (int w = lane; (w << 2) < pmem; w += 64) TL32[w] &= 0x3F3F3F3Fu;
          if (VSTK) {
            if (lane == L) {
#pragma unroll
              for (int i = 0; i < 2 * AVGPU_STACK_SIZE; i++) sv[i] = 0;
            }
          } else if (lane < 2 * AVGPU_STACK_SIZE) {
            stk[lane * 64 + L] = 0;
          }
        }
      }
    }

    if (sstep && !(fl & F_STOP)) {
      if (adv) ip = head_adjust(ip + 1, M);
      if (mx > 0 && tu >= mx) {
        if (serial == 2) { sdie = 1; fl |= F_STOP; executed--; }
        else fl |= F_DEAD;
      }
    }
    pop = -1;
    CK(4);
    }
  }
#undef CK
#undef CKC
#undef GETREG
#undef SETREG
#undef GETHEAD
#undef SETHEAD

  if (k_env_res_mask != 0u)
    res_flush<GTAB>(W, N, cell, rpq, bonus, rc, ttab, tmul, tadd, k_env_res_mask, mode == AVGPU_MODE_WORLD);
#ifdef AVGPU_PHASE_CLOCKS
  const uint64_t clk2 = __builtin_amdgcn_s_memtime();
#endif
  __syncthreads();
  if (active) {
    int4* xw = reinterpret_cast<int4*>(xrec);
    const long long bb = __double_as_longlong(bonus);
    if (IOQ) {
      inptr = (qm >> 30) ? (int)((qm >> 28) & 3u)
                         : ((active && !fresh) ? *(volatile const int32_t*)(xrec + XS_INPTR) : 0);
      int h0, h1, h2;
      io_hist(inptr, (int)(qm >> 30), inp0, inp1, inp2, in0, in1, in2, h0, h1, h2);
      in0 = h0; in1 = h1; in2 = h2;
      outv = (qm >> 30) ? q0 : ((active && !fresh) ? *(volatile const int32_t*)(xrec + XS_OUTBUF) : 0);
    }
    xw[0] = make_int4(r0, r1, r2, ip);
    xw[1] = make_int4(rh, wh, fh, (int)rl);
    xw[2] = make_int4(cyc, tu, gs, errs);
    xw[3] = make_int4(in0, in1, in2, intot);
    xw[4] = make_int4(inptr, outv, outtot, 0);
    xw[5] = make_int4((int)(uint32_t)bb, (int)(bb >> 32), tc[0], tc[1]);
    xw[6] = make_int4(tc[2], tc[3], tc[4], tc[5]);
    xw[7] = make_int4(tc[6], tc[7], tc[8], 0);
#pragma unroll
    for (int j = 0; j < 5; j++)
      xw[8 + j] = VSTK ? make_int4(sv[4 * j], sv[4 * j + 1], sv[4 * j + 2], sv[4 * j + 3])
                       : make_int4(stk[(4 * j) * 64 + lane], stk[(4 * j + 1) * 64 + lane],
                                   stk[(4 * j + 2) * 64 + lane], stk[(4 * j + 3) * 64 + lane]);
#pragma unroll
    for (int j = 0; j < 3; j++) xw[13 + j] = make_int4(rc[4 * j], rc[4 * j + 1], rc[4 * j + 2], rc[4 * j + 3]);
    const bool alive = !(fl & F_DEAD);
    const bool spill = (fl & F_SPILL) != 0;
    if (!alive) ctl &= ~CTL_ALIVE;
    if (mode == AVGPU_MODE_WORLD && alive0 && !alive) W.occ[cell] = 0;
    W.ctl[cell] = (ctl & ~CTL_FRESH) | (sdie ? CTL_SPECDIE : 0u);
    W.mem_size[cell] = M;
    if (serial) W.sctx[2] = kct;
    else W.rng[2 * N + cell] = kct;
    W.budget[cell] = spill ? (budget | (prim ? BUDGET_PRIM : 0)) : 0;
    if (spill && mode == AVGPU_MODE_WORLD) W.sdone[cell] = sdone + executed;
    if (!NB && !spill && mode == AVGPU_MODE_WORLD && !serial) W.ran[cell] = sdone + executed;
    if (didv || fresh) { W.num_div[cell] = dnd; W.generation[cell] = dgen; }
    if (!DEF && didv && W.track_age) W.age[cell] = 0;
    if (didv) W.executed[cell] = dexe;
    if (fresh) {
#pragma unroll
      for (int q = AVGPU_NUM_LOGIC_TASKS; q < AVGPU_MAX_REACTIONS; q++) W.last_task[(int64_t)q * N + cell] = 0;
      if (!didv) W.child_copied[cell] = 0;
    }
#pragma unroll
    for (int i = XS_NREACT; i < AVGPU_MAX_REACTIONS; i++) {
      int32_t* p = W.cur_react + (int64_t)i * N + cell;
      if (i < W.n_react) {
        if (didv || fresh) *p = rc[i];
        else if (rc[i]) *p += rc[i];
      } else if (fresh) {
        *p = 0;
      }
    }
    if (spill) {
      if (!(C0W && cls == 0)) {
        const int slot = atomicAdd(&W.class_count[LIST_SPILL + cls + 1], 1);
        W.class_list[(int64_t)(LIST_SPILL + cls + 1) * N + slot] = cell;
      }
      count_add(W, AVGPU_CNT_SPILLS, 1ull);
    }
  }
#pragma unroll QUNR
  for (int it = 0; it < qits; it++) {
    const int i = it * 64 + lane;
    const int j = i / QUADS, q = i - j * QUADS;
    const int c = __shfl(cell, j);
    const int m = __shfl(M, j);
    if (c >= 0 && q * GRAN < m) {
      if (GRAN == 16) {
        const uint4 v = reinterpret_cast<const uint4*>(lds32)[i];
        *reinterpret_cast<uint4*>(W.tape + (int64_t)c * TAPE_SLOT + q * 16) = v;
      } else {
        *reinterpret_cast<uint32_t*>(W.tape + (int64_t)c * TAPE_SLOT + q * 4) = lds32[i];
      }
    }
  }
  if (serial) return executed | (divides << 16) | (sbirth << 24) | (sdie << 25);
  {
    const bool fresh = prim && !prim0;
    const unsigned long long bm = __ballot(fresh);
    if (bm) {
      int base = 0;
      if (lane == 0) base = atomicAdd(W.b_count + BQ_PRIMARY, (int)__popcll(bm));
      base = __shfl(base, 0);
      if (fresh) W.b_list[base + (int)__popcll(bm & ((1ull << lane) - 1ull))] = cell;
    }
  }
  if (pred) {
    long long pt = 0;
    int q = -1;
    if (active && !(fl & (F_DEAD | F_SPILL)) && alive0 && gs <= tu - executed - sdone)
      pt = pred_term(W, cell, tu, gs, blen, dcop, dexe, bonus, q);
    for (int off = 32; off > 0; off >>= 1) pt += __shfl_xor(pt, off);
    unsigned long long* pa = reinterpret_cast<unsigned long long*>(W.pacc) + (blockIdx.x & (NSHARD - 1)) * PACC_STRIDE;
    if (lane == 0 && pt) atomicAdd(pa + PACC_WEIGHT, (unsigned long long)pt);
    const unsigned long long q01 = (unsigned long long)__popcll(__ballot(q == 0)) |
                                   ((unsigned long long)__popcll(__ballot(q == 1)) << 32);
    const unsigned long long q23 = (unsigned long long)__popcll(__ballot(q == 2)) |
                                   ((unsigned long long)__popcll(__ballot(q == 3)) << 32);
    if (lane == 0 && q01) atomicAdd(pa + PACC_Q01, q01);
    if (lane == 0 && q23) atomicAdd(pa + PACC_Q23, q23);
  }
  unsigned long long e = (unsigned long long)executed;
  int dead = (active && (fl & F_DEAD)) ? 1 : 0;
  int dv = divides;
  int mxe = executed;
  int sl = active ? 1 : 0;
  int sites = active ? m_in + M : 0;
  int nover = noversize, nrover = rover ? 1 : 0;
  for (int off = 32; off > 0; off >>= 1) {
    ndrop += __shfl_down(ndrop, off);
    nover += __shfl_down(nover, off);
    if (REC) nrover += __shfl_down(nrover, off);
    e += __shfl_down(e, off);
    dead += __shfl_down(dead, off);
    dv += __shfl_down(dv, off);
    mxe = max(mxe, __shfl_down(mxe, off));
    sl += __shfl_down(sl, off);
    sites += __shfl_down(sites, off);
  }
  if (lane == 0) {
    count_add(W, AVGPU_CNT_LANESTEPS, 64ull * (unsigned long long)mxe);
    count_add(W, AVGPU_CNT_INSTS, e);
    if (dead) count_add(W, AVGPU_CNT_DEATHS, (unsigned long long)dead);
    if (dv) count_add(W, AVGPU_CNT_DIVIDES, (unsigned long long)dv);
    if (ndrop) count_add(W, AVGPU_CNT_DROPPED, (unsigned long long)ndrop);
    if (nover) count_add(W, AVGPU_CNT_OVERSIZE, (unsigned long long)nover);
    if (REC && nrover) count_add(W, AVGPU_CNT_REC_EXHAUSTED, (unsigned long long)nrover);
    if (S == CLASS0_SIZE && !NB) {
      count_add(W, AVGPU_CNT_C0_SLICES, (unsigned long long)sl);
      count_add(W, AVGPU_CNT_C0_SITES, (unsigned long long)sites);
    }
  }
#ifdef AVGPU_PHASE_CLOCKS
  {
    const uint64_t clk3 = __builtin_amdgcn_s_memtime();
    for (int off = 32; off > 0; off >>= 1) {
      it_fast = max(it_fast, __shfl_down(it_fast, off));
      it_copy = max(it_copy, __shfl_down(it_copy, off));
      it_slow = max(it_slow, __shfl_down(it_slow, off));
    }
    if (lane == 0 && cls == 0) {
      count_add(W, AVGPU_CNT_CLK_STAGE, clk1 - clk0);
      count_add(W, AVGPU_CNT_CLK_LOOP, clk2 - clk1);
      count_add(W, AVGPU_CNT_CLK_WB, clk3 - clk2);
      count_add(W, AVGPU_CNT_ITERS, (unsigned long long)it_loop);
      count_add(W, AVGPU_CNT_IT_FAST, (unsigned long long)it_fast);
      count_add(W, AVGPU_CNT_IT_COPY, (unsigned long long)it_copy);
      count_add(W, AVGPU_CNT_IT_SLOW, (unsigned long long)it_slow);
      count_add(W, AVGPU_CNT_WAVES, 1ull);
      for (int k = 0; k < 6; k++) count_add(W, AVGPU_CNT_CB0 + k, cb[k]);
      for (int k = 0; k < 10; k++) count_add(W, AVGPU_CNT_CASE0 + k, cc[k]);
    }
  }
#endif
  return (C0W && cls == 0 && active && (fl & F_SPILL)) ? cell + 1 : 0;
}

#define MIX_B1 512
#define MIX_B2 16
#define MIX_B3 8
#define MIX_BLOCKS (MIX_B1 + MIX_B2 + MIX_B3)
static_assert(MIX_BLOCKS % 8 == 0, "class 0's XCD mapping needs whole rounds of 8 blocks");
template <int S, bool REC, bool C0W = false, bool SIMPLE = false, bool DEF = false, bool RES = false, bool NB = false>
__global__ __launch_bounds__(64, (S == CLASS0_SIZE) ? 2 : 1) void k_interpret(const DevWorld* __restrict__ Wp, int cls, int row, int mode,
                                                  int64_t first, int64_t count, int sorted_arg, int lpw, int nmix = 0) {
  constexpr int TAB_WORDS = 128 + 64 + 16 + 64 + AVGPU_MAX_REACTIONS * RT_STRIDE + 64;
  constexpr int STK = (S == CLASS0_SIZE) ? 0 : 2 * AVGPU_STACK_SIZE * 64;
  constexpr int TAB = (S == CLASS0_SIZE) ? 0 : TAB_WORDS;
  __shared__ __attribute__((aligned(16))) uint32_t lds32[64 * tape_stride(S) / 4 + STK + TAB];
  const int sorted = sorted_arg & KI_SORTED;
  const bool pred = (sorted_arg & KI_PRED) != 0;
  if (cls == 0) {
// ... 428 lines not shown
```

avida_amd/csrc/world.hip:

```cpp
#include "device.h"
#include "births.h"

#pragma clang fp contract(off)

namespace {

template <int WAVES = 4>
__device__ __forceinline__ void enqueue_class(const DevWorld& W, int cell, bool want, int cls) {
  __shared__ int s_pc[NUM_CLASSES][WAVES], s_base[NUM_CLASSES];
  const int lane = threadIdx.x & 63, wv = threadIdx.x >> 6;
  unsigned long long masks[NUM_CLASSES];
  __syncthreads();
#pragma unroll
  for (int k = 1; k < NUM_CLASSES; k++) {
    masks[k] = __ballot(want && cls == k);
    if (lane == 0) s_pc[k][wv] = __popcll(masks[k]);
  }
  __syncthreads();
  if (threadIdx.x > 0 && threadIdx.x < NUM_CLASSES) {
    const int k = threadIdx.x;
    int tot = 0;
    for (int w = 0; w < WAVES; w++) tot += s_pc[k][w];
    s_base[k] = tot ? atomicAdd(&W.class_count[k], tot) : 0;
  }
// ... 421 lines not shown
  const int64_t nloc = (W.n + 255) / 256;
  const int64_t lo = b0 >> sh, hi = (b0 + nloc - 1) >> sh;
  for (int l = 0; l < L; l++) {
    const int64_t w0 = (int64_t)1 << l;
    const int64_t ilo = lo >> (L - l), ihi = hi >> (L - l);
    for (int64_t i = ilo + tid; i <= ihi; i += 1024) {
      const int64_t h = w0 + i;
      const long long n = cnt[h];
      const long long left = binom_draw(n, __ddiv_rn(scr[2 * h], scr[h]),
                                        node_draw(W.seed_lo, W.seed_hi, update, SALT_TOP, (uint64_t)h));
      cnt[2 * h] = left;
      cnt[2 * h + 1] = n - left;
    }
    __syncthreads();
  }
  if (chunked) {
    for (int64_t j = lo + tid; j <= hi; j += 1024) W.tree_cnt[P + j] = cnt[P + j];
  } else {
    for (int64_t j = tid; j < nloc; j += 1024) W.blk_count[j] = cnt[P + b0 + j];
  }
}

__device__ __forceinline__ long long chunk_sums(double* t, long long* s_cnt, const double* part,
                                                const int32_t* alive_part, int64_t nb, int64_t nbt, int mode,
                                                int64_t k) {
  constexpr int C = 1 << TREE_C_LOG;
  const int tid = threadIdx.x;
  long long a = 0;
  for (int i = tid; i < C; i += 1024) t[C + i] = tree_leaf(part, alive_part, nb, nbt, mode, k * C + i, a);
  s_cnt[tid] = a;
  __syncthreads();
  for (int st = 512; st >= 1; st >>= 1) {
    if (tid < st) s_cnt[tid] += s_cnt[tid + st];
    __syncthreads();
  }
  for (int l = TREE_C_LOG - 1; l >= 0; l--) {
    const int w0 = 1 << l;
    for (int i = tid; i < w0; i += 1024) t[w0 + i] = __dadd_rn(t[2 * (w0 + i)], t[2 * (w0 + i) + 1]);
    __syncthreads();
  }
  return s_cnt[0];
}
__global__ __launch_bounds__(1024) void k_tree_up(DevWorld W, const double* part, const int32_t* alive_part,
                                                  int64_t nb, int ntiles, int mode) {
  __shared__ double t[2 << TREE_C_LOG];
  __shared__ long long s_cnt[1024];
  const int64_t nbt = mode == BC_GATHERED ? nb * ntiles : nb;
  const long long a = chunk_sums(t, s_cnt, part, alive_part, nb, nbt, mode, blockIdx.x);
  if (threadIdx.x == 0) {
    W.tree_scr[blockIdx.x] = t[1];
    W.tree_cnt[blockIdx.x] = a;
  }
}
__global__ __launch_bounds__(1024) void k_tree_down(DevWorld W, const double* part, const int32_t* alive_part,
                                                    int64_t nb, int ntiles, int mode, int64_t K, uint32_t update) {
  constexpr int C = 1 << TREE_C_LOG;
  __shared__ double t[2 * C];
  __shared__ long long c[2 * C];
  __shared__ long long s_cnt[1024];
  const int tid = threadIdx.x;
  const int64_t nbt = mode == BC_GATHERED ? nb * ntiles : nb;
  const int64_t b0 = mode == BC_GATHERED ? W.cell0 / 256 : 0;
  const int64_t nloc = (W.n + 255) / 256;
  const int64_t k = (b0 >> TREE_C_LOG) + blockIdx.x;
  chunk_sums(t, s_cnt, part, alive_part, nb, nbt, mode, k);
  if (tid == 0) c[1] = W.tree_cnt[K + k];
  __syncthreads();
  const int64_t g0 = k * C;
  const int lo = (int)(max(b0, g0) - g0), hi = (int)(min(b0 + nloc, g0 + C) - 1 - g0);
  for (int l = 0; l < TREE_C_LOG; l++) {
    const int w0 = 1 << l;
    const int ilo = lo >> (TREE_C_LOG - l), ihi = hi >> (TREE_C_LOG - l);
    for (int i = ilo + tid; i <= ihi; i += 1024) {
      const int h = w0 + i;
      const long long n = c[h];
      const uint64_t H = (uint64_t)(K + k) * (uint64_t)w0 + (uint64_t)i;
      const long long left = binom_draw(n, __ddiv_rn(t[2 * h], t[h]),
                                        node_draw(W.seed_lo, W.seed_hi, update, SALT_TOP, H));
      c[2 * h] = left;
      c[2 * h + 1] = n - left;
    }
    __syncthreads();
  }
  for (int i = lo + tid; i <= hi; i += 1024) W.blk_count[g0 + i - b0] = c[C + i];
}

__device__ __forceinline__ void occ_init_cell(const DevWorld& W, int64_t c) {
  W.occ[c] = (c < W.n && (W.ctl[c] & CTL_ALIVE)) ? 1 : 0;
  W.owner[c] = -1;
}

__device__ __forceinline__ int window_bucket(bool c0, int budget) {
  return c0 ? SORT_BUCKETS - 2 - min(max(budget, 0), SORT_BUCKETS - 2) : SORT_BUCKETS - 1;
}
__global__ __launch_bounds__(1024) void k_allot(DevWorld W, const double* totals, uint32_t update, int tick) {
  const int lane = threadIdx.x & 63;
  const int64_t b = (int64_t)blockIdx.x * 16 + (threadIdx.x >> 6);
  const int64_t nb = (W.n + 255) / 256;
  const double total = totals[TOT_DIV];
  const bool consts = W.slicing == AVGPU_SLICE_CONSTANT || !(total > 0.0);
  const bool prob = !consts && W.slicing != AVGPU_SLICE_INTEGRATED;
  uint32_t ctl[4];
  double wt[4];
  bool alive[4];
  int msz[4];
#pragma unroll
  for (int j = 0; j < 4; j++) {
    const int64_t c = b * 256 + lane + 64 * j;
    ctl[j] = (b < nb && c < W.n) ? W.ctl[c] : 0u;
    alive[j] = (ctl[j] & CTL_ALIVE) != 0;
    msz[j] = alive[j] ? W.mem_size[c] : 0;
    const double m = alive[j] ? W.merit[c] : 0.0;
    if (alive[j] && !merit_ok(m)) count_add(W, AVGPU_CNT_BAD_RECORD, 1ull);
    wt[j] = alive[j] ? sched_weight(m, ctl[j]) : 0.0;
  }
  long long cnt[4] = {0, 0, 0, 0};
  if (prob && b < nb) {
    const uint64_t gb = (uint64_t)(W.cell0 / 256 + b);
    const uint32_t slo = W.seed_lo, shi = W.seed_hi;
    const double l7a = __dadd_rn(wt[0], wt[2]), l7b = __dadd_rn(wt[1], wt[3]);
    const double l6 = __dadd_rn(l7a, l7b);
    double lv[7];
    lv[6] = l6;
#pragma unroll
    for (int k = 5; k >= 0; k--) {
      const double o = __shfl_down(lv[k + 1], 1 << k);
      lv[k] = __dadd_rn(lv[k + 1], o);
    }
    long long c = lane == 0 ? (long long)W.blk_count[b] : 0;
#pragma unroll
    for (int k = 0; k < 6; k++) {
      long long left = 0;
      const bool act = lane < (1 << k);
      if (act)
        left = binom_draw(c, __ddiv_rn(lv[k + 1], lv[k]),
                          node_draw(slo, shi, update, SALT_BLOCK, (gb << 9) | (uint64_t)((1 << k) + lane)));
      const long long right = c - left;
      const long long got = __shfl_up(right, 1 << k);
      if (act) c = left;
      else if (lane < (2 << k)) c = got;
    }
    const long long l6l = binom_draw(c, __ddiv_rn(l7a, l6),
                                     node_draw(slo, shi, update, SALT_BLOCK, (gb << 9) | (uint64_t)(64 + lane)));
    const long long c7a = l6l, c7b = c - l6l;
    const long long x0 = binom_draw(c7a, __ddiv_rn(wt[0], l7a),
                                    node_draw(slo, shi, update, SALT_BLOCK, (gb << 9) | (uint64_t)(128 + lane)));
    const long long x1 = binom_draw(c7b, __ddiv_rn(wt[1], l7b),
                                    node_draw(slo, shi, update, SALT_BLOCK, (gb << 9) | (uint64_t)(192 + lane)));
    cnt[0] = x0; cnt[2] = c7a - x0; cnt[1] = x1; cnt[3] = c7b - x1;
  }
  bool want[4] = {false, false, false, false};
  int cls[4] = {0, 0, 0, 0}, buds[4] = {0, 0, 0, 0};
#pragma unroll
  for (int j = 0; j < 4; j++) {
    const int64_t c = b * 256 + lane + 64 * j;
    if (b >= nb || c >= W.n) continue;
    int bud = 0;
    if (alive[j]) {
      if (consts) {
        bud = W.ave_time_slice;
      } else if (prob) {
        bud = (int)min(cnt[j], (long long)(BUDGET_PRIM - 1));
      } else {
        double lam = __ddiv_rn(__dmul_rn(totals[TOT_UD], wt[j]), total);
        if (lam > 1.0e8) lam = 1.0e8;
        const double cr = __dadd_rn(W.credit[c], lam);
        const double fl = floor(cr);
        bud = (int)fl;
        W.credit[c] = __dsub_rn(cr, fl);
      }
      if (ctl[j] & CTL_HS_MASK) W.ctl[c] = ctl[j] & ~CTL_HS_MASK;
      if (tick && W.track_age) W.age[c] += 1;
      want[j] = bud > 0;
      if (want[j]) cls[j] = class_of(need_of(msz[j], ctl[j], W.size_range));
    }
    buds[j] = bud;
    W.budget[c] = bud;
    W.aclass[c] = want[j] ? (uint8_t)cls[j] : (uint8_t)ACLASS_NONE;
    W.ran[c] = 0;
    if (W.env_resources)
      for (int r = 0; r < W.n_res; r++) W.cons[(int64_t)r * W.n + c] = 0.0;
    occ_init_cell(W, c);
    W.killt[c] = 0u;
    W.claim_r[3][c] = 0ull;
  }
  unsigned long long ns = 0;
#pragma unroll
  for (int j = 0; j < 4; j++) ns += (unsigned long long)__popcll(__ballot(want[j]));
  if (lane == 0 && ns) count_add(W, AVGPU_CNT_SLICES, ns);
  int cells[4];
#pragma unroll
  for (int j = 0; j < 4; j++) cells[j] = (int)(b * 256 + lane + 64 * j);
  enqueue_class_multi<16, 4>(W, cells, want, cls);
  __shared__ int sh[SORT_BUCKETS];
  for (int i = threadIdx.x; i < SORT_BUCKETS; i += 1024) sh[i] = 0;
  __syncthreads();
#pragma unroll
  for (int j = 0; j < 4; j++) {
    const int64_t c = b * 256 + lane + 64 * j;
    if (b < nb && c < W.n) atomicAdd(&sh[window_bucket(want[j] && cls[j] == 0, buds[j])], 1);
  }
  __syncthreads();
  for (int i = threadIdx.x; i < SORT_BUCKETS; i += 1024) W.sub_hist[(int64_t)blockIdx.x * SORT_BUCKETS + i] = sh[i];
}

__device__ __forceinline__ void bucket_scan(int* h) {
  const int tid = threadIdx.x;
  if (tid < 64) {
    constexpr int PER = (SORT_BUCKETS + 63) / 64;
    int loc[PER], t = 0;
#pragma unroll
    for (int k = 0; k < PER; k++) {
      const int i = tid * PER + k;
      loc[k] = i < SORT_BUCKETS ? h[i] : 0;
      t += loc[k];
    }
    int incl = t;
    for (int off = 1; off < 64; off <<= 1) {
      const int o = __shfl_up(incl, off);
      if (tid >= off) incl += o;
    }
    int run = incl - t;
#pragma unroll
    for (int k = 0; k < PER; k++) {
      const int i = tid * PER + k;
      if (i < SORT_BUCKETS) h[i] = run;
      run += loc[k];
    }
  }
}

__global__ __launch_bounds__(1024) void k_window_order(DevWorld W) {
  constexpr int SUBS = SORT_WIN / 4096;
  __shared__ int start[SORT_BUCKETS];
  const int tid = threadIdx.x;
  const int64_t sub = blockIdx.x;
  const int64_t s0 = (sub / SUBS) * SUBS, nsub = (W.n + 4095) / 4096;
  int before = 0;
  if (tid < SORT_BUCKETS) {
    int tot = 0;
    for (int64_t k = s0; k < s0 + SUBS && k < nsub; k++) {
      const int v = W.sub_hist[k * SORT_BUCKETS + tid];
      tot += v;
      if (k < sub) before += v;
    }
    start[tid] = tot;
  }
  __syncthreads();
  bucket_scan(start);
  __syncthreads();
  if (tid < SORT_BUCKETS) start[tid] += before;
  __syncthreads();
  const int64_t wbase = (sub / SUBS) * SORT_WIN;
#pragma unroll
  for (int h = 0; h < 4; h++) {
    const int64_t c = sub * 4096 + h * 1024 + tid;
    if (c < W.n) {
      const int pos = atomicAdd(&start[window_bucket(W.aclass[c] == 0, W.budget[c])], 1);
      W.order[wbase + pos] = (int32_t)c;
    }
  }
}



__device__ __forceinline__ int64_t edge_cell(const DevWorld& W, int d, int x) {
  return d == 0 ? (int64_t)x : (int64_t)(W.rows - 1) * W.world_x + x;
}
__device__ __forceinline__ int64_t ghost_cell(const DevWorld& W, int d, int x) {
  return W.n + (int64_t)d * W.world_x + x;
}
__device__ __forceinline__ unsigned long long* halo_cl(uint8_t* b, int X, int p, int k) {
  return reinterpret_cast<unsigned long long*>(b) + (int64_t)(2 * p + k) * X;
}
__device__ __forceinline__ uint8_t* halo_occ(uint8_t* b, int X) { return b + (int64_t)X * 32; }
__device__ __forceinline__ uint32_t* halo_kt(uint8_t* b, int X) { return reinterpret_cast<uint32_t*>(b + halo_kt_off(X)); }
__device__ __forceinline__ bool halo_slot(const DevWorld& W, int64_t c, int& d, int& x, bool& ghost) {
  const int X = W.world_x;
  if (c >= W.n) { const int64_t k = c - W.n; d = (int)(k / X); x = (int)(k - (int64_t)d * X); ghost = true; return true; }
  ghost = false;
  if (c < X) { d = 0; x = (int)c; return true; }
  if (c >= W.n - X) { d = 1; x = (int)(c - (W.n - X)); return true; }
  return false;
}
__device__ __forceinline__ bool tile_taken(const DevWorld& W, int64_t c, int m) {
  int d, x;
  bool ghost;
  const bool h = halo_slot(W, c, d, x, ghost);
  if (m == 0) return (h && ghost) ? halo_occ(W.h_recv[d], W.world_x)[x] != 0 : W.occ[c] != 0;
  if (W.occ[c] || W.claim_r[m - 1][c] != 0ull) return true;
  return h && halo_cl(W.h_recv[d], W.world_x, (m - 1) & 1, ghost ? 1 : 0)[x] != 0ull;
}
__device__ __forceinline__ unsigned long long tile_merged(const DevWorld& W, int64_t t, int m) {
  unsigned long long v = W.claim_r[m][t];
  int d, x;
  bool ghost;
  if (halo_slot(W, t, d, x, ghost)) {
    const unsigned long long o = halo_cl(W.h_recv[d], W.world_x, m & 1, ghost ? 1 : 0)[x];
    if (o > v) v = o;
  }
  return v;
}

__device__ __forceinline__ void finalize_key(const DevWorld& W, int64_t r, int parent) {
  int32_t* row = W.b_inh + r * BI_WORDS;
  if ((row[BI_FINAL] & 1) == 0) return;
  uint32_t clo, chi;
  derive_key(W.rng[parent], W.rng[W.n + parent], W.b_seq[r], 0x1B873593U, clo, chi);
  row[BI_RLO] = (int32_t)clo;
  row[BI_RHI] = (int32_t)chi;
}
__device__ __forceinline__ void finalize_phenotype(const DevWorld& W, int64_t r) {
  static_assert(BI_LTASK == 12 && BI_FINAL == 11 && AVGPU_NUM_LOGIC_TASKS <= 12, "row quads");
  int32_t* row = W.b_inh + r * BI_WORDS;
  const int4* q = reinterpret_cast<const int4*>(row);
  const int4 q0 = q[0], q1 = q[1], q2 = q[2], q3 = q[3], q4 = q[4], q5 = q[5];
  const int parent = W.b_parent[r];
  const int seq = (int)W.b_seq[r];
  if ((q2.w & 1) == 0) return;
  const int nd = W.num_div[parent];
  const double merit = __hiloint2double(q0.y, q0.x);
  const int gt = q1.w;
  const double fit = __ddiv_rn(merit, (double)gt);
  const long long fb = __double_as_longlong(fit);
  row[BI_FITNESS] = (int32_t)fb;
  row[BI_FITNESS + 1] = (int32_t)(fb >> 32);
  if (seq == nd) {
    W.merit[parent] = merit;
    W.fitness[parent] = fit;
    W.gest_time[parent] = gt;
    W.child_copied[parent] = q1.y;
    W.executed[parent] = q1.z;
    const int lt[12] = {q3.x, q3.y, q3.z, q3.w, q4.x, q4.y, q4.z, q4.w, q5.x, q5.y, q5.z, q5.w};
#pragma unroll
    for (int k = 0; k < AVGPU_NUM_LOGIC_TASKS; k++) W.last_task[(int64_t)k * W.n + parent] = lt[k];
  }
}

__device__ __forceinline__ unsigned long long claim_key(uint32_t t, bool kill, uint32_t draw, int64_t gparent,
                                                        uint32_t seq) {
  const unsigned long long tk = kill ? (unsigned long long)(t & 0xFFFFu) : (unsigned long long)(0xFFFFu - (t & 0xFFFFu));
  return (tk << 48) | ((unsigned long long)(kill ? 1 : 0) << 47) | ((unsigned long long)(draw >> 17) << 32) |
         ((unsigned long long)(gparent & 0xFFFFFF) << 8) | (unsigned long long)(seq & 0xFF);
}
__device__ __forceinline__ bool key_kill(unsigned long long k) { return ((k >> 47) & 1ull) != 0ull; }
__device__ __forceinline__ uint32_t key_time(unsigned long long k) {
  const uint32_t tk = (uint32_t)(k >> 48);
  return key_kill(k) ? tk : 0xFFFFu - tk;
}
enum : int8_t { BS_PENDING = 0, BS_WON = 1 , BS_KILL_LOST = 8 ,
                BS_CANCELLED = -1, BS_NO_CELL = -2  };
__device__ __forceinline__ uint32_t rec_time(const DevWorld& W, int64_t r) {
  return BI_TIME(W.b_inh[r * BI_WORDS + BI_FINAL]);
}
__device__ __forceinline__ uint32_t owner_time(const DevWorld& W, int o) {
  return o >= 0 ? rec_time(W, o) : (uint32_t)((-2 - o) >> 2);
}
__device__ __forceinline__ bool takes_cell(const DevWorld& W, int owner, uint32_t t) {
  return owner == -1 || owner_time(W, owner) <= t;
}
__device__ __forceinline__ int last_claim_round(int st) {
  if (st == BS_PENDING) return 3;
  if (st >= BS_WON && st < BS_WON + 4) return st - BS_WON;
  if (st >= BS_KILL_LOST && st < BS_KILL_LOST + 4) return st - BS_KILL_LOST;
  if (st <= BS_NO_CELL) return BS_NO_CELL - st - 1;
  return -1;
}

__device__ __forceinline__ bool tile_taken(const DevWorld& W, int64_t c, int m);
__device__ __forceinline__ double position_value(const DevWorld& W, int c) {
  if (c >= W.n || !(W.ctl[c] & CTL_ALIVE)) return 0.0;
  const double age = (double)W.age[c];
  if (W.birth_method == 1) return age;
  const double m = W.merit[c];
  return m > 0.0 ? __ddiv_rn(age, m) : age;
}
template <bool TILE>
__device__ __forceinline__ bool place_pick_one(const DevWorld& W, int64_t r, int m) {
  const int parent = W.b_parent[r];
  if (m == 0) finalize_key(W, r, parent);
  const unsigned long long* prev = m > 0 ? W.claim_r[m - 1] : nullptr;
  auto taken = [&](int c) -> bool {
    if (TILE) return tile_taken(W, c, m);
    return W.occ[c] != 0 || (prev && prev[c] != 0ull);
  };
  if (!TILE && W.birth_method == 4) {
    int32_t* const inh = W.b_inh + (int64_t)r * BI_WORDS;
    const uint32_t lo = (uint32_t)inh[BI_RLO], hi = (uint32_t)inh[BI_RHI];
    uint32_t ctr = (uint32_t)inh[BI_RCTR];
    const uint32_t n = (uint32_t)W.n;
    int t = -1;
    if (W.prefer_empty) {
      const uint32_t ne = (uint32_t)W.e_blk[(W.n + 255) / 256];
      t = ne > 0u ? W.e_list[rng_below(lo, hi, ctr, ne)] : (int)rng_below(lo, hi, ctr, n);
    } else {
      t = (int)rng_below(lo, hi, ctr, n);
      while (!W.allow_parent && n > 1u && t == parent) t = (int)rng_below(lo, hi, ctr, n);
    }
    if (t == parent && !W.allow_parent) {
      inh[BI_RCTR] = (int32_t)ctr;
      W.b_target[r] = -1;
      W.b_state[r] = (int8_t)(BS_NO_CELL - m);
      return false;
    }
    const unsigned long long key = claim_key(BI_TIME(inh[BI_FINAL]), taken(t), rng_next(lo, hi, ctr),
                                             W.cell0 + parent, W.b_seq[r]);
    inh[BI_RCTR] = (int32_t)ctr;
    W.b_target[r] = t;
    W.b_prio[r] = key;
    W.b_tgt[(int64_t)m * W.rcap + r] = t;
    return true;
  }
  int nbr[8];
  const int nn = neighbours(W, parent, nbr);
  int cand[9];
  int nc = 0;
  if (W.prefer_empty)
    for (int k = 0; k < nn; k++)
      if (!taken(nbr[k])) cand[nc++] = nbr[k];
  if (nc == 0 && (W.birth_method == 1 || W.birth_method == 2)) {
    double best = W.allow_parent ? position_value(W, parent) : -1.0;
    cand[nc++] = parent;
    for (int k = 0; k < nn; k++) {
      const double v = position_value(W, nbr[k]);
      if (v > best) { best = v; nc = 0; cand[nc++] = nbr[k]; }
      else if (v == best) cand[nc++] = nbr[k];
    }
  } else if (nc == 0 && W.birth_method != 3) {
    for (int k = 0; k < nn; k++) cand[nc++] = nbr[k];
    if (W.allow_parent) cand[nc++] = parent;
  }
  if (nc == 0 && !W.allow_parent) {
    W.b_target[r] = -1;
    W.b_state[r] = (int8_t)(BS_NO_CELL - m);
    return false;
  }
  int32_t* const inh = W.b_inh + (int64_t)r * BI_WORDS;
  const uint32_t lo = (uint32_t)inh[BI_RLO], hi = (uint32_t)inh[BI_RHI];
  uint32_t ctr = (uint32_t)inh[BI_RCTR];
  const int t = nc > 0 ? cand[rng_below(lo, hi, ctr, (uint32_t)nc)] : parent;
  const unsigned long long key = claim_key(BI_TIME(inh[BI_FINAL]), taken(t), rng_next(lo, hi, ctr),
                                           W.cell0 + parent, W.b_seq[r]);
  inh[BI_RCTR] = (int32_t)ctr;
  W.b_target[r] = t;
  W.b_prio[r] = key;
  W.b_tgt[(int64_t)m * W.rcap + r] = t;
  return true;
}

#define QUEUE_LOOP(i) \
  for (int64_t i = (int64_t)blockIdx.x * blockDim.x + threadIdx.x, _qn = queue_len(W); i < _qn; \
       i += (int64_t)gridDim.x * blockDim.x)
__device__ __forceinline__ bool soup_free(const DevWorld& W, int64_t c, int m) {
  return c < W.n && W.occ[c] == 0 && (m == 0 || W.claim_r[m - 1][c] == 0ull);
}
__global__ __launch_bounds__(256) void k_empty_count(DevWorld W, int m) {
  __shared__ int ws[4];
  const int64_t c = (int64_t)blockIdx.x * 256 + threadIdx.x;
  const bool e = soup_free(W, c, m);
  const int cnt = __popcll(__ballot(e));
  if ((threadIdx.x & 63) == 0) ws[threadIdx.x >> 6] = cnt;
  __syncthreads();
  if (threadIdx.x == 0) W.e_blk[blockIdx.x] = ws[0] + ws[1] + ws[2] + ws[3];
}
__global__ __launch_bounds__(1024) void k_empty_scan(DevWorld W, int nb) {
  __shared__ int part[1024];
  const int per = (nb + 1023) / 1024;
  const int b0 = (int)threadIdx.x * per, b1 = min(nb, b0 + per);
  int sum = 0;
  for (int b = b0; b < b1; b++) sum += W.e_blk[b];
  part[threadIdx.x] = sum;
  __syncthreads();
  for (int off = 1; off < 1024; off <<= 1) {
    const int v = (int)threadIdx.x >= off ? part[threadIdx.x - off] : 0;
    __syncthreads();
    part[threadIdx.x] += v;
    __syncthreads();
  }
  int run = threadIdx.x > 0 ? part[threadIdx.x - 1] : 0;
  for (int b = b0; b < b1; b++) {
    const int v = W.e_blk[b];
    W.e_blk[b] = run;
    run += v;
  }
  if (threadIdx.x == 1023) W.e_blk[nb] = part[1023];
}
__global__ __launch_bounds__(256) void k_empty_scatter(DevWorld W, int m) {
  __shared__ int ws[4];
  const int lane = threadIdx.x & 63, wv = threadIdx.x >> 6;
  const int64_t c = (int64_t)blockIdx.x * 256 + threadIdx.x;
  const bool e = soup_free(W, c, m);
  const unsigned long long bm = __ballot(e);
  if (lane == 0) ws[wv] = __popcll(bm);
  __syncthreads();
  int base = W.e_blk[blockIdx.x];
  for (int k = 0; k < wv; k++) base += ws[k];
  if (e) W.e_list[base + __popcll(bm & ((1ull << lane) - 1ull))] = (int)c;
}

#define MUT_PER_WAVE 8
#define MUT_PER_BLOCK (4 * MUT_PER_WAVE)
__device__ __forceinline__ void mutation_block(const DevWorld& W, int64_t blk, int64_t nblk,
                                               uint8_t (*child)[TAPE_SLOT + 16]) {
  __shared__ int ml[MUT_PER_BLOCK][8];
  __shared__ int mn;
  const int nb = queue_len(W);
  const int lane = threadIdx.x & 63, wv = threadIdx.x >> 6;
  for (int64_t q0 = blk * MUT_PER_BLOCK; q0 < nb; q0 += nblk * MUT_PER_BLOCK) {
    if (threadIdx.x == 0) mn = 0;
    __syncthreads();
    const int64_t q = q0 + wv * MUT_PER_WAVE + lane;
    if (lane < MUT_PER_WAVE && q < nb) {
      const int64_t r = rec_of(W, q);
      int e[5];
#pragma unroll
      for (int k = 0; k < 5; k++) e[k] = W.b_edit[(int64_t)k * W.rcap + r];
      const int l0 = W.b_len0[r], l1 = W.b_len[r];
      int x = e[0] | e[1] | e[2] | e[3] | e[4];
      if (W.seg_any)
        for (int k = 0; k < NSEG; k++) x |= W.b_pcnt[(int64_t)k * W.rcap + r];
      if (x) {
        const int i = atomicAdd(&mn, 1);
        ml[i][0] = (int)(uint32_t)r; ml[i][1] = (int)(r >> 32);
#pragma unroll
        for (int k = 0; k < 5; k++) ml[i][2 + k] = e[k];
        ml[i][7] = l0 | (l1 << 16);
      }
    }
    __syncthreads();
    const int n = mn;
    for (int i = wv; i < n; i += 4) {
      const int64_t r = (int64_t)(uint32_t)ml[i][0] | ((int64_t)ml[i][1] << 32);
      const int e[5] = {ml[i][2], ml[i][3], ml[i][4], ml[i][5], ml[i][6]};
      apply_edits_core(W, r, e, ml[i][7] & 0xFFFF, ml[i][7] >> 16, child[wv]);
    }
    __syncthreads();
  }
}

__global__ void k_place_round(DevWorld W, int m) {
  const unsigned long long* prev = W.claim_r[m - 1];
  unsigned long long* cur = W.claim_r[m];
  QUEUE_LOOP(q) {
    const int64_t r = rec_of(W, q);
    if (W.b_state[r] != BS_PENDING) continue;
    const int t = W.b_target[r];
    const unsigned long long key = W.b_prio[r];
    if (prev[t] == key) {
      W.b_state[r] = (int8_t)(BS_WON + m - 1);
      W.occ[t] = 1;
      if (takes_cell(W, W.owner[t], rec_time(W, r))) W.owner[t] = (int)r;
      continue;
    }
    if (key_kill(key)) { W.b_state[r] = (int8_t)(BS_KILL_LOST + m - 1); continue; }
    if (place_pick_one<false>(W, r, m)) atomicMax(&cur[W.b_target[r]], W.b_prio[r]);
  }
}
__global__ void k_place_claim0(DevWorld W, long long* pred_out, long long pred_seq) {
  if (blockIdx.x == 0 && threadIdx.x < NUM_LISTS) W.class_count[threadIdx.x] = 0;
  if (pred_out && blockIdx.x == 0 && threadIdx.x == 0) {
    pred_out[PRED_ACC] = pacc_sum(W, PACC_WEIGHT);
    pred_out[PRED_ORGS] = (long long)W.totals[TOT_ORGS];
    pred_out[PRED_DENSEST] = densest_quarter(W);
    __threadfence_system();
    __hip_atomic_store(pred_out + PRED_SEQ, pred_seq, __ATOMIC_RELAXED, __HIP_MEMORY_SCOPE_SYSTEM);
  }
  QUEUE_LOOP(q) {
    const int64_t r = rec_of(W, q);
    if (W.b_state[r] != BS_PENDING) continue;
    const int p = W.b_parent[r];
    if (W.killt[p] > 0x10000u - rec_time(W, r)) { W.b_state[r] = BS_CANCELLED; continue; }
    atomicMax(&W.claim_r[0][W.b_target[r]], W.b_prio[r]);
  }
}
__global__ __launch_bounds__(256) void k_place_pick_mut(DevWorld W, int pblocks, int fblocks, int boff, int nblocks) {
  __shared__ uint8_t child[4][TAPE_SLOT + 16];
  const int nb = queue_len(W);
  const int bid = (int)blockIdx.x + boff;
  if (bid < pblocks) {
    for (int64_t i = (int64_t)bid * 256 + threadIdx.x; i < nb; i += (int64_t)pblocks * 256) {
      const int64_t r = rec_of(W, i);
      if (!place_pick_one<false>(W, r, 0)) continue;
      const unsigned long long key = W.b_prio[r];
      if (key_kill(key)) atomicMax(&W.killt[W.b_target[r]], 0x10000u - key_time(key));
    }
    return;
  }
  if (bid < pblocks + fblocks) {
    for (int64_t i = (int64_t)(bid - pblocks) * 256 + threadIdx.x; i < nb; i += (int64_t)fblocks * 256)
      finalize_phenotype(W, rec_of(W, i));
    return;
  }
  pblocks += fblocks;
  mutation_block(W, bid - pblocks, nblocks - pblocks, child);
}


__global__ __launch_bounds__(256) void k_tile_prep(DevWorld W, int mblocks, int fblocks) {
  __shared__ uint8_t child[4][TAPE_SLOT + 16];
  if ((int)blockIdx.x >= mblocks && (int)blockIdx.x < mblocks + fblocks) {
    const int nb = queue_len(W);
    for (int64_t i = (int64_t)(blockIdx.x - mblocks) * 256 + threadIdx.x; i < nb; i += (int64_t)fblocks * 256)
      finalize_phenotype(W, rec_of(W, i));
    return;
  }
  if ((int)blockIdx.x < mblocks) {
    mutation_block(W, blockIdx.x, mblocks, child);
    return;
  }
  const int X = W.world_x;
  const int g = (blockIdx.x - mblocks - fblocks) * blockDim.x + threadIdx.x;
  if (g >= 2 * X) return;
  const int d = g / X, x = g - d * X;
  const int64_t gc = ghost_cell(W, d, x);
  W.occ[gc] = 0;
  W.owner[gc] = -1;
#pragma unroll
  for (int k = 0; k < 4; k++) W.claim_r[k][gc] = 0ull;
  uint8_t* b = W.h_send[d];
  halo_occ(b, X)[x] = W.occ[edge_cell(W, d, x)];
#pragma unroll
  for (int k = 0; k < 4; k++) halo_cl(b, X, k >> 1, k & 1)[x] = 0ull;
  halo_kt(b, X)[x] = 0u;
}

__global__ __launch_bounds__(256) void k_tile_round(DevWorld W, int m, int rblocks) {
  const int X = W.world_x;
  if ((int)blockIdx.x < rblocks) {
    const int nb = queue_len(W);
    for (int64_t q = (int64_t)blockIdx.x * blockDim.x + threadIdx.x; q < nb; q += (int64_t)rblocks * blockDim.x) {
      const int64_t r = rec_of(W, q);
      if (W.b_state[r] != BS_PENDING) continue;
      if (m == 0) {
        if (!place_pick_one<true>(W, r, 0)) continue;
        const unsigned long long key = W.b_prio[r];
        if (!key_kill(key)) continue;
        const int t = W.b_target[r];
        const uint32_t kv = 0x10000u - key_time(key);
        if (t >= W.n) {
          const int64_t k = t - W.n;
          const int d = (int)(k / X), x = (int)(k - (int64_t)d * X);
          atomicMax(&halo_kt(W.h_send[d], X)[x], kv);
        } else {
          atomicMax(&W.killt[t], kv);
        }
        continue;
      }
      const int t = W.b_target[r];
      const unsigned long long key = W.b_prio[r];
      if (tile_merged(W, t, m - 1) == key) {
        W.b_state[r] = (int8_t)(BS_WON + m - 1);
        W.occ[t] = 1;
        if (takes_cell(W, W.owner[t], rec_time(W, r))) W.owner[t] = (int)r;
        continue;
      }
      if (key_kill(key)) { W.b_state[r] = (int8_t)(BS_KILL_LOST + m - 1); continue; }
      if (m < 4 && place_pick_one<true>(W, r, m)) {
        const int nt = W.b_target[r];
        const unsigned long long nk = W.b_prio[r];
        atomicMax(&W.claim_r[m][nt], nk);
        int d, x;
        bool ghost;
        if (halo_slot(W, nt, d, x, ghost)) atomicMax(&halo_cl(W.h_send[d], X, m & 1, ghost ? 0 : 1)[x], nk);
      }
    }
    return;
  }
  const int g = (blockIdx.x - rblocks) * blockDim.x + threadIdx.x;
  if (m == 4 && g < 2) {
    HaloHdr* hdr = reinterpret_cast<HaloHdr*>(W.r_send[g]);
    hdr->count = 0;
    hdr->arena_used = 0;
    hdr->overflow = 0;
  }
  if (g >= 2 * X) return;
  const int d = g / X, x = g - d * X;
  const int64_t gc = ghost_cell(W, d, x);
  if (m == 0) {
    W.occ[gc] = halo_occ(W.h_recv[d], X)[x];
    return;
  }
  const int p = (m - 1) & 1;
  const int64_t c = edge_cell(W, d, x);
  const unsigned long long rc = halo_cl(W.h_recv[d], X, p, 0)[x], rg = halo_cl(W.h_recv[d], X, p, 1)[x];
  const unsigned long long lg = W.claim_r[m - 1][gc];
  if (rc != 0ull && rc > W.claim_r[m - 1][c]) {
    const uint32_t tr = key_time(rc);
    if (takes_cell(W, W.owner[c], tr)) W.owner[c] = REMOTE_OWNER(m - 1, tr);
    W.occ[c] = 1;
  }
  if (rg != 0ull && rg > lg) {
    const uint32_t tr = key_time(rg);
    if (takes_cell(W, W.owner[gc], tr)) W.owner[gc] = REMOTE_OWNER(m - 1, tr);
  }
  if (lg != 0ull || rg != 0ull) W.occ[gc] = 1;
  if (m == 1 || m == 2) {
    uint8_t* b = W.h_send[d];
    halo_cl(b, X, p, 0)[x] = 0ull;
    halo_cl(b, X, p, 1)[x] = 0ull;
  }
}
__global__ __launch_bounds__(256) void k_tile_claim0(DevWorld W) {
  const int X = W.world_x;
  if (blockIdx.x == 0 && threadIdx.x < NUM_LISTS) W.class_count[threadIdx.x] = 0;
  QUEUE_LOOP(q) {
    const int64_t r = rec_of(W, q);
    if (W.b_state[r] != BS_PENDING) continue;
    const int p = W.b_parent[r];
    uint32_t kt = W.killt[p];
    int d, x;
    bool ghost;
    if (halo_slot(W, p, d, x, ghost)) kt = max(kt, halo_kt(W.h_recv[d], X)[x]);
    if (kt > 0x10000u - rec_time(W, r)) { W.b_state[r] = BS_CANCELLED; continue; }
    const int t = W.b_target[r];
    const unsigned long long key = W.b_prio[r];
    atomicMax(&W.claim_r[0][t], key);
    if (halo_slot(W, t, d, x, ghost)) atomicMax(&halo_cl(W.h_send[d], X, 0, ghost ? 0 : 1)[x], key);
  }
}

__device__ __forceinline__ double nb_frac(uint32_t t) { return __dmul_rn((double)(0x10000u - t), 1.0 / 65536.0); }
__device__ __forceinline__ long long newborn_budget(const DevWorld& W, int64_t c, uint32_t t, double merit,
                                                    uint32_t key, long long uds, double total) {
  if (!(total > 0.0) || uds <= 0) return 0;
  const long long n = (long long)floor(__dadd_rn(__dmul_rn((double)uds, nb_frac(t)), 0.5));
  const double p = __ddiv_rn(sched_weight(merit, 0u), total);
  const long long b = binom_draw(n, p, node_draw(W.seed_lo, W.seed_hi, key, SALT_NEWBORN, (uint64_t)(W.cell0 + c)));
  return min(b, (long long)(BUDGET_PRIM - 1));
}
__device__ __forceinline__ void newborn_credit(const DevWorld& W, int64_t c, uint32_t t) {
  const double f = nb_frac(t);
  for (int r = 0; r < W.n_res; r++) {
    const double v = W.cons[(int64_t)r * W.n + c];
    if (v == 0.0) continue;
    const double back = __dmul_rn(v, f);
    const ResParam& q = W.res_param[r];
    if (q.geometry != AVGPU_RES_GLOBAL) {
      double* p = W.res_amount + (int64_t)q.slot * W.n + c;
      *p = __dadd_rn(*p, back);
    } else {
      atomicAdd(W.res_cons + r, 0ull - (unsigned long long)__dmul_rn(back, RES_FIX));
    }
  }
}
__device__ __forceinline__ int newborn_setup(const DevWorld& W, int64_t c, uint32_t t, double merit, int len,
                                             uint32_t key, long long uds, double total, long long& carry,
                                             unsigned long long& wasted, int ran) {
  if (W.env_resources) newborn_credit(W, c, t);
  const long long left = (long long)__dmul_rn((double)ran, nb_frac(t));
  const long long bud = newborn_budget(W, c, t, merit, key, uds, total);
  carry += bud - left;
  wasted += (unsigned long long)left;
  W.budget[c] = (int32_t)bud;
  return bud > 0 ? class_of(::need_of(len, CTL_ALIVE, W.size_range)) : -1;
}
__device__ __forceinline__ void newborn_enqueue(const DevWorld& W, int cell, int row) {
  const int lane = threadIdx.x & 63;
#pragma unroll
  for (int k = 0; k < NUM_CLASSES; k++) {
    const unsigned long long m = __ballot(row == k);
    if (!m) continue;
    int base = 0;
    if (lane == 0) base = atomicAdd(&W.class_count[k], (int)__popcll(m));
    base = __shfl(base, 0);
    if (row == k) W.class_list[(int64_t)k * W.n + base + (int)__popcll(m & ((1ull << lane) - 1ull))] = cell;
  }
}

#ifndef ACT_PRE
#define ACT_PRE 8
#endif
__global__ __launch_bounds__(64) void k_activate(DevWorld W, int fused, uint32_t key, int sub, int nsub) {
  const int nb = queue_len(W);
  const int64_t ncell = W.n + (W.tiled ? 2 * (int64_t)W.world_x : 0);
  const int lane = threadIdx.x & 63;
  const double total = W.totals[TOT_DIV];
  const long long uds = sub_share((long long)W.totals[TOT_UD], sub, nsub);
  unsigned long long born = 0, over = 0, canc = 0, nocell = 0, bad = 0, wasted = 0, nbs = 0;
  long long carry = 0;
  for (int64_t q0 = (int64_t)blockIdx.x * 64; q0 < nb; q0 += (int64_t)gridDim.x * 64) {
    const int64_t q = q0 + lane;
    int nrow = -1, ncell_nb = 0;
    do {
      if (q >= nb) break;
      const int64_t i = rec_of(W, q);
      const uint4* g4 = reinterpret_cast<const uint4*>(W.b_genome + i * TAPE_SLOT);
      uint4 pre[ACT_PRE];
#pragma unroll
      for (int u = 0; u < ACT_PRE; u++) pre[u] = g4[u];
      const int tgt = W.b_target[i];
      const int8_t st = W.b_state[i];
      Child b = child_of_record(W, i);
      const int ran = (tgt >= 0 && (int64_t)tgt < W.n) ? W.ran[tgt] : 0;
      const int lastr = last_claim_round(st);
      bool ok = true;
      for (int k = 0; k <= lastr && k < 3; k++) {
        const int tk = (k == lastr && tgt >= 0) ? tgt : W.b_tgt[(int64_t)k * W.rcap + i];
        if (tk >= 0 && (int64_t)tk < ncell) W.claim_r[k][tk] = 0ull;
        else ok = false;
      }
      if (st == BS_CANCELLED) { canc++; break; }
      if (st <= BS_NO_CELL) { nocell++; break; }
      if (!ok || tgt < 0 || (int64_t)tgt >= ncell) { bad++; break; }
      const uint32_t t = 0x10000u - b.hs;
      bool won = false;
      if (fused == ACT_STRIP) {
        won = st >= BS_WON && st < BS_WON + 4 && W.owner[tgt] == (int)i;
      } else if (st == BS_PENDING) {
        won = W.claim_r[3][tgt] == W.b_prio[i] && takes_cell(W, W.owner[tgt], t);
      } else if (st >= BS_WON && st < BS_WON + 4) {
        const unsigned long long c3 = W.claim_r[3][tgt];
        won = W.owner[tgt] == (int)i && !(c3 != 0ull && key_time(c3) >= t);
      }
      if (!won) { over++; break; }
      if (b.len < 0 || b.len > AVGPU_MAX_GENOME) { bad++; break; }
      if (tgt >= W.n) break;
      born++;
      b.hs = 0;
      setup_child_lane<ACT_PRE>(W, tgt, b, W.b_genome + i * TAPE_SLOT, pre);
      nrow = newborn_setup(W, tgt, t, b.merit, b.len, key, uds, total, carry, wasted, ran);
      ncell_nb = tgt;
    } while (0);
    nbs += nrow >= 0 ? 1ull : 0ull;
    newborn_enqueue(W, ncell_nb, nrow);
  }
  for (int off = 32; off > 0; off >>= 1) {
    born += __shfl_xor(born, off);
    over += __shfl_xor(over, off);
    canc += __shfl_xor(canc, off);
    nocell += __shfl_xor(nocell, off);
    bad += __shfl_xor(bad, off);
    wasted += __shfl_xor(wasted, off);
    nbs += __shfl_xor(nbs, off);
    carry += __shfl_xor(carry, off);
  }
  if (threadIdx.x == 0) {
    if (born) count_add(W, AVGPU_CNT_BIRTHS, born);
    if (over) count_add(W, AVGPU_CNT_OVERWRITTEN, over);
    if (canc) count_add(W, AVGPU_CNT_CANCELLED, canc);
    if (nocell) count_add(W, AVGPU_CNT_DROPPED, nocell);
    if (bad) count_add(W, AVGPU_CNT_BAD_RECORD, bad);
    if (wasted) count_add(W, AVGPU_CNT_WASTED, wasted);
    if (nbs) count_add(W, AVGPU_CNT_SLICES, nbs);
    if (carry) atomicAdd(reinterpret_cast<unsigned long long*>(W.sched + SCHED_CARRY), (unsigned long long)carry);
  }
}

__global__ __launch_bounds__(64) void k_halo_pack(DevWorld W) {
  const int nb = queue_len(W);
  const int lane = threadIdx.x;
  const int X = W.world_x;
  unsigned long long sent = 0, lost = 0;
  for (int64_t q0 = (int64_t)blockIdx.x * 64; q0 < nb; q0 += (int64_t)gridDim.x * 64) {
    const int64_t q = q0 + lane;
    int64_t mine = -1;
    if (q < nb) {
      const int64_t i = rec_of(W, q);
      const int tgt = W.b_target[i];
      const int8_t st = W.b_state[i];
      if (st >= BS_WON && st < BS_WON + 4 && tgt >= W.n && (int64_t)tgt < W.n + 2 * (int64_t)X &&
          W.b_len[i] >= 0 && W.b_len[i] <= AVGPU_MAX_GENOME && W.owner[tgt] == (int)i)
        mine = i;
    }
    for (unsigned long long m = __ballot(mine >= 0); m; m &= m - 1ull) {
    const int64_t i = (int64_t)__shfl((long long)mine, __ffsll((long long)m) - 1);
    const int tgt = W.b_target[i];
    const int d = (tgt - (int)W.n) / X, col = (tgt - (int)W.n) - d * X;
    const int len = W.b_len[i];
    HaloHdr* hdr = reinterpret_cast<HaloHdr*>(W.r_send[d]);
    HaloRec* recs = reinterpret_cast<HaloRec*>(W.r_send[d] + sizeof(HaloHdr));
    uint8_t* arena = W.r_send[d] + sizeof(HaloHdr) + (int64_t)X * sizeof(HaloRec);
    int slot = 0, off = 0;
    if (lane == 0) {
      slot = atomicAdd(&hdr->count, 1);
      off = atomicAdd(&hdr->arena_used, (len + 3) & ~3);
    }
    slot = __shfl(slot, 0);
    off = __shfl(off, 0);
    const bool fits = (int64_t)off + len <= W.r_arena;
    if (lane == 0) {
      HaloRec r;
      r.col = col; r.round = W.b_state[i] - BS_WON; r.len = fits ? len : -1;
      const Child b = child_of_record(W, i);
      r.gen = b.gen; r.ccopied = b.ccopied; r.exec = b.exec; r.gest = b.gest;
      r.rng_lo = b.lo; r.rng_hi = b.hi; r.rng_ctr = b.ctr;
      r.off = off; r.t = 0x10000u - b.hs; r.merit = b.merit; r.fitness = b.fitness;
#pragma unroll
      for (int t = 0; t < AVGPU_NUM_LOGIC_TASKS; t++) r.last_task[t] = b.ltask[t];
      r.pad2[0] = r.pad2[1] = r.pad2[2] = 0;
      recs[slot] = r;
      if (!fits) atomicAdd(&hdr->overflow, 1);
    }
    if (fits) {
      const uint32_t* src = reinterpret_cast<const uint32_t*>(W.b_genome + i * TAPE_SLOT);
      uint32_t* dst = reinterpret_cast<uint32_t*>(arena + off);
      for (int w = lane; w < (len + 3) / 4; w += 64) dst[w] = src[w];
      sent++;
    } else {
      lost++;
    }
    }
  }
  if (lane == 0) {
    if (sent) count_add(W, AVGPU_CNT_HALO_SENT, sent);
    if (lost) { count_add(W, AVGPU_CNT_HALO_LOST, lost); count_add(W, AVGPU_CNT_DROPPED, lost); }
  }
}

__global__ __launch_bounds__(64) void k_activate_remote(DevWorld W, uint32_t key, int sub, int nsub) {
  const int lane = threadIdx.x;
  const double total = W.totals[TOT_DIV];
  const long long uds = sub_share((long long)W.totals[TOT_UD], sub, nsub);
  long long carry = 0;
  unsigned long long wasted = 0, nbs = 0;
  const int X = W.world_x;
  const int half = gridDim.x >> 1;
  const int d = (int)blockIdx.x >= half ? 1 : 0;
  const int b0 = (int)blockIdx.x - d * half;
  const HaloHdr* hdr = reinterpret_cast<const HaloHdr*>(W.r_recv[d]);
  const HaloRec* recs = reinterpret_cast<const HaloRec*>(W.r_recv[d] + sizeof(HaloHdr));
  const uint8_t* arena = W.r_recv[d] + sizeof(HaloHdr) + (int64_t)X * sizeof(HaloRec);
  const int nrec = min(hdr->count, X);
  unsigned long long born = 0, lost = 0;
  for (int q = b0; q < nrec; q += half) {
    const HaloRec r = recs[q];
    if (r.len < 0) continue;
    if (r.col < 0 || r.col >= X || r.len > AVGPU_MAX_GENOME || r.off < 0 || (r.off & 3) ||
        (int64_t)r.off + r.len > W.r_arena || r.round < 0 || r.round > 3) {
      if (lane == 0) count_add(W, AVGPU_CNT_BAD_RECORD, 1ull);
      continue;
    }
    const int64_t c = edge_cell(W, d, r.col);
    if (W.owner[c] != REMOTE_OWNER(r.round, r.t)) { lost++; continue; }
    born++;
    Child b;
    b.len = r.len; b.gen = r.gen; b.ccopied = r.ccopied; b.exec = r.exec; b.gest = r.gest;
    b.hs = 0;
    b.merit = r.merit; b.fitness = r.fitness; b.lo = r.rng_lo; b.hi = r.rng_hi; b.ctr = r.rng_ctr;
    b.ltask = recs[q].last_task; b.lstride = 1;
    const int ran = W.ran[c];
    setup_child<64>(W, c, b, reinterpret_cast<const uint32_t*>(arena + r.off), lane);
    if (lane == 0) {
      const int row = newborn_setup(W, c, r.t, r.merit, r.len, key, uds, total, carry, wasted, ran);
      if (row >= 0) {
        nbs++;
        const int slot = atomicAdd(&W.class_count[row], 1);
        W.class_list[(int64_t)row * W.n + slot] = (int)c;
      }
    }
  }
  if (lane == 0) {
    if (born) count_add(W, AVGPU_CNT_BIRTHS, born);
    if (lost) count_add(W, AVGPU_CNT_OVERWRITTEN, lost);
    if (wasted) count_add(W, AVGPU_CNT_WASTED, wasted);
    if (nbs) count_add(W, AVGPU_CNT_SLICES, nbs);
    if (carry) atomicAdd(reinterpret_cast<unsigned long long*>(W.sched + SCHED_CARRY), (unsigned long long)carry);
  }
}

__device__ __forceinline__ double wave_sum(double v) {
  for (int off = 32; off > 0; off >>= 1) v += __shfl_xor(v, off);
  return v;
}
__device__ __forceinline__ double wave_max(double v) {
  for (int off = 32; off > 0; off >>= 1) v = fmax(v, __shfl_xor(v, off));
  return v;
}
__device__ __forceinline__ int wave_sum_i(int v) {
  for (int off = 32; off > 0; off >>= 1) v += __shfl_xor(v, off);
  return v;
}
__device__ __forceinline__ unsigned long long wave_sum_u64(unsigned long long v) {
  for (int off = 32; off > 0; off >>= 1) v += __shfl_xor(v, off);
  return v;
}
__global__ __launch_bounds__(256) void k_stats_partial(DevWorld W, double* part) {
  __shared__ double s[4][NPART];
  const int64_t c = (int64_t)blockIdx.x * 256 + threadIdx.x;
  const int wv = threadIdx.x >> 6, lane = threadIdx.x & 63;
  double merit = 0.0, fit = 0.0;
  int iv[5] = {0, 0, 0, 0, 0};
  unsigned long long tasks = 0;
  if (c < W.n && (W.ctl[c] & CTL_ALIVE)) {
    merit = W.merit[c];
    fit = W.fitness[c];
    iv[0] = 1;
    iv[1] = W.gest_time[c];
    iv[2] = W.birth_len[c];
    iv[3] = W.generation[c];
    iv[4] = W.mem_size[c];
#pragma unroll
    for (int t = 0; t < AVGPU_NUM_LOGIC_TASKS; t++)
      tasks |= (W.last_task[t * W.n + c] > 0 ? 1ull : 0ull) << (7 * t);
  }
  const double rm = wave_sum(merit), rf = wave_sum(fit), rx = wave_max(fit);
  int ri[5];
#pragma unroll
  for (int k = 0; k < 5; k++) ri[k] = wave_sum_i(iv[k]);
  const unsigned long long rt = wave_sum_u64(tasks);
  if (lane == 0) {
    s[wv][ST_ORGS] = (double)ri[0]; s[wv][ST_MERIT] = rm; s[wv][ST_FITNESS] = rf;
    s[wv][ST_GESTATION] = (double)ri[1]; s[wv][ST_GENOME_LEN] = (double)ri[2]; s[wv][ST_MAX_FITNESS] = rx;
    s[wv][ST_GENERATION] = (double)ri[3]; s[wv][ST_MEM_SIZE] = (double)ri[4];
#pragma unroll
    for (int t = 0; t < AVGPU_NUM_LOGIC_TASKS; t++) s[wv][ST_TASK0 + t] = (double)((rt >> (7 * t)) & 127ull);
  }
  __syncthreads();
  if (threadIdx.x < NUSED) {
    const int k = threadIdx.x;
    double r = s[0][k];
    for (int q = 1; q < 4; q++) r = (k == ST_MAX_FITNESS) ? fmax(r, s[q][k]) : r + s[q][k];
    part[(int64_t)k * gridDim.x + blockIdx.x] = r;
  }
}

__global__ __launch_bounds__(256) void k_stats_final(DevWorld W, const double* part, int64_t nb,
                                                     double* out) {
  __shared__ double sd[256];
  constexpr int NG = 256 / CNT_STRIDE;
  __shared__ unsigned long long cs[NG][CNT_STRIDE];
  const int tid = threadIdx.x;
  const int k = blockIdx.x;
  if (k >= NUSED && k < NPART) {
    if (tid == 0) out[k] = 0.0;
    return;
  }
  if (k < NPART) {
    const bool mx = k == ST_MAX_FITNESS;
    double acc = 0.0;
    for (int64_t b = tid; b < nb; b += 256) {
      const double o = part[(int64_t)k * nb + b];
      acc = mx ? fmax(acc, o) : acc + o;
    }
    sd[tid] = acc;
    __syncthreads();
    for (int stride = 128; stride >= 1; stride >>= 1) {
      if (tid < stride) sd[tid] = mx ? fmax(sd[tid], sd[tid + stride]) : sd[tid] + sd[tid + stride];
      __syncthreads();
    }
    if (tid == 0) out[k] = sd[0];
    return;
  }
  {
    const int slot = tid & (CNT_STRIDE - 1), g = tid / CNT_STRIDE;
    unsigned long long a = 0;
    for (int sh = g; sh < NSHARD; sh += NG) a += W.counters[sh * CNT_STRIDE + slot];
    cs[g][slot] = a;
  }
  __syncthreads();
  const bool fold = W.counters[CNT_CUM_FLAG] == 0ull;
  __syncthreads();
  if (tid < CNT_STRIDE) {
    unsigned long long t = 0;
    for (int g = 0; g < NG; g++) t += cs[g][tid];
    cs[0][tid] = t;
    if (tid == CNT_STRIDE - 1) W.counters[CNT_CUM_FLAG] = 1ull;
    else if (fold) W.counters[CNT_CUM_BASE + tid] += t;
  }
  __syncthreads();
  if (tid == 0) {
    out[ST_INSTS] = (double)cs[0][AVGPU_CNT_INSTS];
    out[ST_DEATHS] = (double)cs[0][AVGPU_CNT_DEATHS];
    out[ST_DIVIDES] = (double)cs[0][AVGPU_CNT_DIVIDES];
    out[ST_BIRTHS] = (double)cs[0][AVGPU_CNT_BIRTHS];
    out[ST_DROPPED] = (double)cs[0][AVGPU_CNT_DROPPED];
    out[ST_SPILLS] = (double)cs[0][AVGPU_CNT_SPILLS];
    out[ST_CUM_INSTS] = (double)W.counters[CNT_CUM_INSTS];
    out[ST_CUM_BIRTHS] = (double)W.counters[CNT_CUM_BIRTHS];
    out[ST_SLICES] = (double)cs[0][AVGPU_CNT_SLICES];
    out[ST_LANESTEPS] = (double)cs[0][AVGPU_CNT_LANESTEPS];
    out[ST_OVERWRITTEN] = (double)cs[0][AVGPU_CNT_OVERWRITTEN];
    out[ST_CANCELLED] = (double)cs[0][AVGPU_CNT_CANCELLED];
    out[ST_WASTED] = (double)cs[0][AVGPU_CNT_WASTED];
    out[ST_PRED] = __longlong_as_double(pacc_sum(W, PACC_WEIGHT));
    out[ST_CARRY] = __longlong_as_double(W.sched[SCHED_CARRY] + W.sched[SCHED_CARRY_REM]);
    out[ST_PRED_ORGS] = W.totals[TOT_ORGS];
    out[ST_PRED_DENSEST] = __longlong_as_double(densest_quarter(W));
    for (int q = 0; q < 4; q++) out[ST_QUARTER0 + q] = __longlong_as_double(quarter_count(W, q));
  }
}

}

static inline unsigned nblk(int64_t n, int b) { return (unsigned)((n + b - 1) / b); }

void launch_set_orgs(const DevWorld& W, hipStream_t s, int64_t first, int64_t count,
                     const uint8_t* codes, const int32_t* offsets, const int32_t* lens,
                     const double* merits, const int32_t* inputs, int deterministic) {
  hipLaunchKernelGGL(k_set_orgs, dim3(nblk(count, 64)), dim3(64), 0, s, W, first, count, codes,
                     offsets, lens, merits, inputs, deterministic);
}

void launch_get_states(const DevWorld& W, hipStream_t s, int64_t first, int64_t count,
                       avgpu_cpu_state* states, uint8_t* codes, int cap) {
  hipLaunchKernelGGL(k_get_states, dim3(nblk(count, 64)), dim3(64), 0, s, W, first, count, states,
                     codes, cap);
}

void launch_state_digest(const DevWorld& W, hipStream_t s, int64_t first, int64_t count, uint64_t* d_out) {
  if (count <= 0) return;
  k_state_digest<<<(unsigned)((count + 127) / 128), 128, 0, s>>>(W, first, count, d_out);
}

void launch_get_census(const DevWorld& W, hipStream_t s, int64_t first, int64_t count, avgpu_census* d_out) {
  if (count <= 0) return;
  k_census<<<(unsigned)((count + 255) / 256), 256, 0, s>>>(W, first, count, d_out);
}
void launch_set_states(const DevWorld& W, hipStream_t s, int64_t first, int64_t count, const avgpu_cpu_state* in,
                       const uint8_t* codes, int cap) {
  hipLaunchKernelGGL(k_set_states, dim3((unsigned)((count + 127) / 128)), dim3(128), 0, s, W, first, count, in,
                     codes, cap);
}

void launch_classify_uniform(const DevWorld& W, hipStream_t s, int64_t first, int64_t count,
                             const int32_t* budget, int32_t uniform) {
  hipMemsetAsync(W.class_count, 0, sizeof(int32_t) * CLASS_COUNT_WORDS, s);
  hipLaunchKernelGGL(k_classify_uniform, dim3(nblk(count, 256)), dim3(256), 0, s, W, first, count,
                     budget, uniform);
}

static void launch_block_counts(const DevWorld& W, hipStream_t s, const double* part, const int32_t* alive,
                                int64_t nb, int ntiles, int L, double* totals, uint32_t update, int mode,
                                int sub = 0, int nsub = 1) {
  if (((int64_t)1 << L) <= TREE_LDS_P) {
    hipLaunchKernelGGL(k_block_counts<true>, dim3(1), dim3(1024), 0, s, W, part, alive, nb, ntiles, L, totals, update,
                       mode, 0, sub, nsub);
    return;
  }
  const int Lt = L - TREE_C_LOG;
  const int64_t K = (int64_t)1 << Lt;
  hipLaunchKernelGGL(k_tree_up, dim3((unsigned)K), dim3(1024), 0, s, W, part, alive, nb, ntiles, mode);
  hipLaunchKernelGGL(k_block_counts<true>, dim3(1), dim3(1024), 0, s, W, part, alive, nb, ntiles, Lt, totals,
                     update, mode, 1, sub, nsub);
  if (mode == BC_TOTALS_ONLY) return;
  const int64_t b0 = mode == BC_GATHERED ? W.cell0 / 256 : 0, nloc = (W.n + 255) / 256;
  const int64_t nk = ((b0 + nloc - 1) >> TREE_C_LOG) - (b0 >> TREE_C_LOG) + 1;
  hipLaunchKernelGGL(k_tree_down, dim3((unsigned)nk), dim3(1024), 0, s, W, part, alive, nb, ntiles, mode, K, update);
}

static int tree_levels(int64_t nbt) {
  int L = 0;
  while (((int64_t)1 << L) < nbt) L++;
  return L;
}

void launch_merit_total(const DevWorld& W, hipStream_t s, double* totals, double* scratch) {
  const int64_t nb = (W.n + 255) / 256;
  int32_t* alive_partial = reinterpret_cast<int32_t*>(scratch + nb);
  hipLaunchKernelGGL(k_merit_partial, dim3((unsigned)((nb + 3) / 4)), dim3(256), 0, s, W, scratch, alive_partial,
                     (double*)nullptr, RESET_NONE);
  launch_block_counts(W, s, scratch, alive_partial, nb, 1, tree_levels(nb), totals, 0u, BC_TOTALS_ONLY);
}

__global__ __launch_bounds__(256) void k_reset_counts(DevWorld W) { reset_counts_block(W); }

static void launch_allot(const DevWorld& W, hipStream_t s, const double* totals, uint32_t update, int tick) {
  hipLaunchKernelGGL(k_allot, dim3(nblk(W.n, 4096)), dim3(1024), 0, s, W, totals, update, tick);
  hipLaunchKernelGGL(k_window_order, dim3(nblk(W.n, 4096)), dim3(1024), 0, s, W);
}

void launch_world_begin(const DevWorld& W, hipStream_t s, double* totals, double* scratch, uint32_t update,
                        int sub, int nsub, bool own_totals) {
  const int64_t nb = (W.n + 255) / 256;
  int32_t* alive_partial = reinterpret_cast<int32_t*>(scratch + nb);
  if (sub == 0) launch_resources_begin(W, s);
  hipLaunchKernelGGL(k_merit_partial, dim3((unsigned)((nb + 3) / 4)), dim3(256), 0, s, W, scratch, alive_partial,
                     (double*)nullptr, sub == 0 ? RESET_COUNTS : RESET_QUEUES);
  launch_block_counts(W, s, scratch, alive_partial, nb, 1, tree_levels(nb), totals, update,
                      own_totals ? BC_OWN : BC_HANDED_IN, sub, nsub);
  launch_allot(W, s, totals, update, sub == 0 ? 1 : 0);
}

void launch_tile_pre(const DevWorld& W, hipStream_t s, const double* gathered, int ntiles, double* totals,
                     uint32_t update, int sub, int nsub) {
  const int64_t nb = (W.n + 255) / 256;
  if (sub == 0) launch_resources_begin(W, s);
  launch_block_counts(W, s, gathered, nullptr, nb, ntiles, tree_levels(nb * ntiles), totals, update, BC_GATHERED, sub,
                      nsub);
  launch_allot(W, s, totals, update, sub == 0 ? 1 : 0);
}

void launch_stats(const DevWorld& W, hipStream_t s, double* stats) {
  const int64_t nb = (W.n + 255) / 256;
  double* part = stats + NSTAT;
  hipLaunchKernelGGL(k_stats_partial, dim3((unsigned)nb), dim3(256), 0, s, W, part);
  hipLaunchKernelGGL(k_stats_final, dim3(NPART + 1), dim3(256), 0, s, W, part, nb, stats);
}

static unsigned lane_grid(const DevWorld& W) { return (unsigned)std::min<int64_t>(nblk(W.rcap, 64), 2048); }
static unsigned place_grid(const DevWorld& W) {
  static const int cap = env_int("AVGPU_PLACE_GRID", 2048, 1, INT32_MAX);
  return (unsigned)std::min<int64_t>(nblk(W.rcap, 256), cap);
}

static bool has_divide_mutations(const DevWorld& W) {
  return (W.th_div_mut | W.th_div_ins | W.th_div_del | W.th_div_slip | W.th_div_uni) != 0 || W.seg_any;
}
static unsigned mut_grid(const DevWorld& W) { return (unsigned)std::min<int64_t>(nblk(W.rcap, MUT_PER_WAVE), 8192); }

void launch_serial_post(const DevWorld& W, hipStream_t s, double* stats) {
  launch_resources_end(W, s);
  launch_stats(W, s, stats);
}

__global__ void k_age_tick(DevWorld W) {
  const int64_t c = (int64_t)blockIdx.x * blockDim.x + threadIdx.x;
  if (c < W.n && W.track_age && (W.ctl[c] & CTL_ALIVE)) W.age[c] += 1;
}
void launch_age_tick(const DevWorld& W, hipStream_t s) {
  hipLaunchKernelGGL(k_age_tick, dim3(nblk(W.n, 256)), dim3(256), 0, s, W);
}

void launch_reset_counts(const DevWorld& W, hipStream_t s) {
  hipLaunchKernelGGL(k_reset_counts, dim3(1), dim3(256), 0, s, W);
}

void launch_world_post(const DevWorld& W, hipStream_t s, uint32_t key, int sub, int nsub, long long* pred_out,
                       long long pred_seq) {
  const unsigned bb = place_grid(W);
  const int pm = has_divide_mutations(W) ? (int)((mut_grid(W) + 3) / 4) : 0;
  const int pf = (int)std::min<unsigned>(bb, 256u);
  const int nbk = (int)bb + pf + pm;
  const bool soup = W.birth_method == 4 && W.prefer_empty;
  auto soup_cells = [&](int m) {
    const int eb = (int)nblk(W.n, 256);
    hipLaunchKernelGGL(k_empty_count, dim3(eb), dim3(256), 0, s, W, m);
    hipLaunchKernelGGL(k_empty_scan, dim3(1), dim3(1024), 0, s, W, eb);
    hipLaunchKernelGGL(k_empty_scatter, dim3(eb), dim3(256), 0, s, W, m);
  };
  if (soup) soup_cells(0);
#ifdef AVGPU_SPLIT_PICK_MUT
  hipLaunchKernelGGL(k_place_pick_mut, dim3(bb), dim3(256), 0, s, W, (int)bb, pf, 0, nbk);
  hipLaunchKernelGGL(k_place_pick_mut, dim3(pf), dim3(256), 0, s, W, (int)bb, pf, (int)bb, nbk);
  if (pm) hipLaunchKernelGGL(k_place_pick_mut, dim3(pm), dim3(256), 0, s, W, (int)bb, pf, (int)bb + pf, nbk);
#else
  hipLaunchKernelGGL(k_place_pick_mut, dim3(nbk), dim3(256), 0, s, W, (int)bb, pf, 0, nbk);
#endif
  hipLaunchKernelGGL(k_place_claim0, dim3(bb), dim3(256), 0, s, W, pred_out, pred_seq);
  for (int m = 1; m < 4; m++) {
    if (soup) soup_cells(m);
    hipLaunchKernelGGL(k_place_round, dim3(bb), dim3(256), 0, s, W, m);
  }
  hipLaunchKernelGGL(k_activate, dim3(lane_grid(W)), dim3(64), 0, s, W, ACT_WORLD, key, sub, nsub);
}

void launch_world_end(const DevWorld& W, hipStream_t s, double* stats, bool eager) {
  launch_resources_end(W, s);
  if (eager) launch_stats(W, s, stats);
}

void launch_tile_partials(const DevWorld& W, hipStream_t s, double* out, int reset) {
  const int64_t nb = (W.n + 255) / 256;
  hipLaunchKernelGGL(k_merit_partial, dim3((unsigned)((nb + 3) / 4)), dim3(256), 0, s, W, out, (int32_t*)nullptr,
                     out + nb, reset);
}

void launch_tile_after_interpret(const DevWorld& W, hipStream_t s) {
  const unsigned hb = nblk(2 * (int64_t)W.world_x, 256);
  const int mb = has_divide_mutations(W) ? (int)((mut_grid(W) + 3) / 4) : 0;
  const int fb = (int)std::min<unsigned>(place_grid(W), 256u);
  hipLaunchKernelGGL(k_tile_prep, dim3(mb + fb + hb), dim3(256), 0, s, W, mb, fb);
}

void launch_tile_place(const DevWorld& W, hipStream_t s, int round, int phase, uint32_t key, int sub, int nsub) {
  const unsigned bb = place_grid(W);
  const unsigned hb = nblk(2 * (int64_t)W.world_x, 256);
  if (phase == TP_ROUND) {
    hipLaunchKernelGGL(k_tile_round, dim3(bb + hb), dim3(256), 0, s, W, round, (int)bb);
  } else if (phase == TP_CLAIM0) {
    hipLaunchKernelGGL(k_tile_claim0, dim3(bb), dim3(256), 0, s, W);
  } else if (phase == TP_PACK) {
    hipLaunchKernelGGL(k_tile_round, dim3(bb + hb), dim3(256), 0, s, W, 4, (int)bb);
    hipLaunchKernelGGL(k_halo_pack, dim3(lane_grid(W)), dim3(64), 0, s, W);
  } else {
    hipLaunchKernelGGL(k_activate, dim3(lane_grid(W)), dim3(64), 0, s, W, ACT_STRIP, key, sub, nsub);
  }
}

void launch_tile_finish(const DevWorld& W, hipStream_t s, uint32_t key, int sub, int nsub) {
  const unsigned rb = (unsigned)std::max(1, std::min(W.world_x, 4096));
  hipLaunchKernelGGL(k_activate_remote, dim3(2 * rb), dim3(64), 0, s, W, key, sub, nsub);
}
```

Measured before the change: 24.98 billion organism-instructions/s.

## Pack birth-record placement fields into the b_inh row and batch neighbour loads

Moves the per-record parent, seq, length, state, target and priority arrays into spare quads of the 32-word b_inh row, so placement and activation kernels read a record with a few 128-bit loads instead of many scattered arrays. The pick logic is restructured to preload neighbour occupancy and claim words into a bitmask before choosing a cell, and k_activate prefetches the next list entry. This reduces the number of separate memory transactions in the birth pipeline, at the cost of more complex code and row layout constraints.

```diff
diff --git a/avida_amd/csrc/births.h b/avida_amd/csrc/births.h
--- a/avida_amd/csrc/births.h
+++ b/avida_amd/csrc/births.h
@@ -30,6 +30,36 @@
     }
   return n;
 }
+__device__ __forceinline__ uint32_t neighbours_mask(const DevWorld& W, int cell, int (&out)[8]) {
+  const int X = W.world_x, R = W.rows;
+  const int x = cell % X, y = cell / X;
+  const bool bounded = W.geometry == 1;
+  uint32_t mask = 0;
+#pragma unroll
+  for (int k = 0; k < 8; k++) {
+    const int j = k < 4 ? k : k + 1;
+    const int dx = j % 3 - 1, dy = j / 3 - 1;
+    int nx = x + dx, ny = y + dy;
+    bool ok = true;
+    if (bounded) ok = nx >= 0 && nx < X;
+    else nx = nx < 0 ? nx + X : (nx >= X ? nx - X : nx);
+    int c;
+    if (ny >= 0 && ny < R) {
+      c = ny * X + nx;
+    } else if (!W.tiled) {
+      if (bounded) ok = false;
+      ny = ny < 0 ? ny + R : ny - R;
+      c = ny * X + nx;
+    } else {
+      const int gy = W.row0 + ny;
+      if (bounded && (gy < 0 || gy >= W.global_rows)) ok = false;
+      c = (int)W.n + (ny < 0 ? 0 : X) + nx;
+    }
+    out[k] = ok ? c : cell;
+    mask |= (ok ? 1u : 0u) << k;
+  }
+  return mask;
+}
 
 __device__ __forceinline__ void edit_back(int ew, int& src, int& val) {
   if (ew == 0 || val >= 0) return;
@@ -136,7 +166,7 @@
   int e[5];
 #pragma unroll
   for (int k = 0; k < 5; k++) e[k] = W.b_edit[(int64_t)k * W.rcap + r];
-  apply_edits_core(W, r, e, W.b_len0[r], W.b_len[r], child);
+  apply_edits_core(W, r, e, W.b_len0[r], W.b_inh[r * BI_WORDS + BI_LEN], child);
 }
 
 struct Child {
@@ -212,7 +242,8 @@
 }
 template <int PRE = 0>
 __device__ __forceinline__ void setup_child_lane(const DevWorld& W, int64_t c, const Child& b,
-                                                 const uint8_t* __restrict__ src, const uint4* pre = nullptr) {
+                                                 const uint8_t* __restrict__ src, const uint4* pre,
+                                                 const int (&lt)[12]) {
   const int64_t N = W.n;
   const int len = b.len;
   const uint4* __restrict__ s4 = reinterpret_cast<const uint4*>(src);
@@ -256,15 +287,15 @@
   if (W.rec_off) W.rec_off[c] = -1;
 #pragma unroll
   for (int q = 0; q < AVGPU_NUM_LOGIC_TASKS; q++)
-    W.last_task[(int64_t)q * N + c] = b.ltask[(int64_t)q * b.lstride];
-}
-
-__device__ __forceinline__ Child child_of_record(const DevWorld& W, int64_t i) {
+    W.last_task[(int64_t)q * N + c] = lt[q];
+}
+
+__device__ __forceinline__ Child child_of_row(const DevWorld& W, int64_t i, int4 q0, int4 q1, int4 q2, int4 q6) {
   Child b;
-  const int4* row = reinterpret_cast<const int4*>(W.b_inh + i * BI_WORDS);
-  const int4 q0 = row[0], q1 = row[1], q2 = row[2];
-  static_assert(BI_MERIT == 0 && BI_GEN == 4 && BI_RLO == 8 && BI_LTASK == 12, "b_inh row layout");
-  b.len = W.b_len[i];
+  static_assert(BI_MERIT == 0 && BI_FITNESS == 2 && BI_GEN == 4 && BI_CCOPIED == 5 && BI_EXEC == 6 && BI_GEST == 7 &&
+                BI_RLO == 8 && BI_RHI == 9 && BI_RCTR == 10 && BI_FINAL == 11 && BI_LTASK == 12 &&
+                BI_PARENT == 24 && BI_LEN == 26, "b_inh row layout");
+  b.len = q6.z;
   b.merit = __hiloint2double(q0.y, q0.x); b.fitness = __hiloint2double(q0.w, q0.z);
   b.gen = q1.x; b.ccopied = q1.y; b.exec = q1.z; b.gest = q1.w;
   b.lo = (uint32_t)q2.x; b.hi = (uint32_t)q2.y; b.ctr = (uint32_t)q2.z;
@@ -272,5 +303,10 @@
   b.ltask = W.b_inh + i * BI_WORDS + BI_LTASK; b.lstride = 1;
   return b;
 }
-
-}
+__device__ __forceinline__ Child child_of_record(const DevWorld& W, int64_t i) {
+  const int4* row = reinterpret_cast<const int4*>(W.b_inh + i * BI_WORDS);
+  const int4 q0 = row[0], q1 = row[1], q2 = row[2], q6 = row[BI_PARENT / 4];
+  return child_of_row(W, i, q0, q1, q2, q6);
+}
+
+}
diff --git a/avida_amd/csrc/capi.hip b/avida_amd/csrc/capi.hip
--- a/avida_amd/csrc/capi.hip
+++ b/avida_amd/csrc/capi.hip
@@ -143,7 +143,7 @@
   A(class_list, NUM_LISTS * n); A(order, n); A(sub_hist, (size_t)((n + 4095) / 4096) * SORT_BUCKETS); A(class_count, CLASS_COUNT_WORDS); A(counters, CNT_WORDS);
   W.rcap = n + (test_buffers ? 16 : std::max<int64_t>(4096, n / 4));
   const int64_t R = W.rcap;
-  A(b_count, BQ_WORDS); A(b_list, n); A(b_parent, R); A(b_seq, R); A(b_len, R); A(b_len0, R); A(b_edit, 5 * R);
+  A(b_count, BQ_WORDS); A(b_list, n); A(b_len0, R); A(b_edit, 5 * R);
   const double pmeans[5] = {c.divide_poisson_slip_mean, c.divide_poisson_mut_mean,
                             c.divide_poisson_ins_mean, c.divide_poisson_del_mean, c.divide_poisson_trans_mean};
   const double psite[6] = {c.div_mut_prob, c.div_ins_prob, c.div_del_prob, c.div_uniform_prob, c.div_slip_prob,
@@ -172,8 +172,7 @@
   W.seg_any = (pois || site) ? 1 : 0;
   W.pois_any = pois ? 1 : 0;
   for (int q = 0; q < 5; q++) W.pois_L[q] = pmeans[q] > 0.0 ? std::exp(-pmeans[q]) : 0.0;
-  A(b_inh, (size_t)BI_WORDS * R); A(b_target, R); A(b_state, R);
-  A(b_prio, R); A(b_genome, (size_t)R * TAPE_SLOT);
+  A(b_inh, (size_t)BI_WORDS * R); A(b_genome, (size_t)R * TAPE_SLOT);
   const int64_t ng = n + 2 * (int64_t)c.world_x;
   A(occ, ng); A(claim, ng); A(claim2, ng); A(owner, ng); A(killt, n); A(sdone, n); A(ran, n); A(sched, SCHED_WORDS); A(pacc, NSHARD * PACC_STRIDE);
   W.claim_r[0] = W.claim; W.claim_r[1] = W.claim2;
diff --git a/avida_amd/csrc/device.h b/avida_amd/csrc/device.h
--- a/avida_amd/csrc/device.h
+++ b/avida_amd/csrc/device.h
@@ -8,7 +8,10 @@
 
 #define TAPE_SLOT 2048
 enum { BI_MERIT = 0, BI_FITNESS = 2, BI_GEN = 4, BI_CCOPIED = 5, BI_EXEC = 6, BI_GEST = 7,
-       BI_RLO = 8, BI_RHI = 9, BI_RCTR = 10, BI_FINAL = 11, BI_LTASK = 12, BI_WORDS = 32 };
+       BI_RLO = 8, BI_RHI = 9, BI_RCTR = 10, BI_FINAL = 11, BI_LTASK = 12,
+       BI_PARENT = 24, BI_SEQ = 25, BI_LEN = 26, BI_STATE = 27, BI_TARGET = 28, BI_PRIO = 30, BI_WORDS = 32 };
+static_assert(BI_LTASK + 12 <= BI_PARENT && BI_PARENT % 4 == 0 && BI_TARGET % 4 == 0 && BI_PRIO % 2 == 0 &&
+              BI_PRIO + 2 == BI_WORDS, "b_inh row: the placement words are its last two quads");
 #define BI_TIME(w) ((uint32_t)(w) >> 16)
 #define CODE_MASK 0x3F
 #define TF_COPIED 0x40
@@ -100,9 +103,6 @@
   int64_t rcap;
   int32_t* b_count;
   int32_t* b_list;
-  int32_t* b_parent;
-  uint32_t* b_seq;
-  int32_t* b_len;
   int32_t* b_len0;
   int32_t* b_edit;
   int32_t* b_subs;
@@ -110,9 +110,6 @@
   int32_t* b_pofs;
   int32_t* b_pcnt;
   int32_t* b_inh;
-  int32_t* b_target;
-  int8_t* b_state;
-  unsigned long long* b_prio;
   uint8_t* b_genome;
   uint8_t* occ;
   unsigned long long* claim;
@@ -233,7 +230,7 @@
   long long* pacc;
   const double* totals;
 };
-static_assert(sizeof(DevWorld) == 1664, "DevWorld's size");
+static_assert(sizeof(DevWorld) == 1616, "DevWorld's size");
 
 
 enum {
@@ -281,7 +278,8 @@
   BQ_PRIMARY = 0,
   BQ_OVERFLOW = 1,
   BQ_SUBS = 2,
-  BQ_WORDS = 3
+  BQ_PICKED = 3,
+  BQ_WORDS = 7
 };
 enum { LIST_NEWBORN = 0, LIST_SPILL = 3, CLASS_COUNT_WORDS = 8 };
 static_assert(NUM_LISTS <= CLASS_COUNT_WORDS, "a length per list row");
diff --git a/avida_amd/csrc/interp.hip b/avida_amd/csrc/interp.hip
--- a/avida_amd/csrc/interp.hip
+++ b/avida_amd/csrc/interp.hip
@@ -1418,20 +1418,11 @@
               if (rec >= 0) {
                 uint32_t clo = 0u, chi = 0u;
                 if (!defer) derive_key(olo, ohi, (uint32_t)nd, 0x1B873593U, clo, chi);
-                int32_t* b_parent = W.b_parent;
-                uint32_t* b_seq = W.b_seq;
-                int32_t* b_len = W.b_len;
                 int32_t* b_len0 = W.b_len0;
                 int32_t* b_edit = W.b_edit;
-                int8_t* b_state = W.b_state;
-                int32_t* b_target = W.b_target;
                 int32_t* b_inh = W.b_inh;
                 int64_t rcap = W.rcap;
-                OPQ(b_parent); OPQ(b_seq); OPQ(b_len); OPQ(b_len0); OPQ(b_edit);
-                OPQ(b_state); OPQ(b_target); OPQ(b_inh); OPQ(rcap);
-                st_async_u32(b_parent + rec, (uint32_t)cell);
-                st_async_u32(b_seq + rec, (uint32_t)nd);
-                st_async_u32(b_len + rec, (uint32_t)len);
+                OPQ(b_len0); OPQ(b_edit); OPQ(b_inh); OPQ(rcap);
                 st_async_u32(b_len0 + rec, (uint32_t)child);
                 st_async_u32(b_edit + rec, (uint32_t)e0);
                 st_async_u32(b_edit + rcap + rec, (uint32_t)e1);
@@ -1456,8 +1447,10 @@
                 st_async_b128(irow + 12, (uint32_t)tc[0], (uint32_t)tc[1], (uint32_t)tc[2], (uint32_t)tc[3]);
                 st_async_b128(irow + 16, (uint32_t)tc[4], (uint32_t)tc[5], (uint32_t)tc[6], (uint32_t)tc[7]);
                 st_async_b128(irow + 20, (uint32_t)tc[8], 0u, 0u, 0u);
-                st_async_u8(b_state + rec, 0u);
-                st_async_u32(b_target + rec, 0xFFFFFFFFu);
+                static_assert(BI_PARENT == 24 && BI_SEQ == 25 && BI_LEN == 26 && BI_STATE == 27 &&
+                              BI_TARGET == 28 && BI_PRIO == 30, "b_inh row: placement quads");
+                st_async_b128(irow + BI_PARENT, (uint32_t)cell, (uint32_t)nd, (uint32_t)len, 0u);
+                st_async_b128(irow + BI_TARGET, 0xFFFFFFFFu, 0u, 0u, 0u);
               }
             }
 #pragma unroll
diff --git a/avida_amd/csrc/world.hip b/avida_amd/csrc/world.hip
--- a/avida_amd/csrc/world.hip
+++ b/avida_amd/csrc/world.hip
@@ -747,21 +747,43 @@
   return v;
 }
 
-__device__ __forceinline__ void finalize_key(const DevWorld& W, int64_t r, int parent) {
+struct PlaceRow {
+  uint32_t lo, hi, ctr, fin;
+  int parent;
+  uint32_t seq;
+  int len, state, target;
+  unsigned long long prio;
+};
+__device__ __forceinline__ PlaceRow place_row(const DevWorld& W, int64_t r) {
+  static_assert(BI_RLO == 8 && BI_RHI == 9 && BI_RCTR == 10 && BI_FINAL == 11 && BI_PARENT == 24 && BI_SEQ == 25 &&
+                BI_LEN == 26 && BI_STATE == 27 && BI_TARGET == 28 && BI_PRIO == 30, "row quads");
+  const int4* q = reinterpret_cast<const int4*>(W.b_inh + r * BI_WORDS);
+  const int4 q2 = q[2], q6 = q[6], q7 = q[7];
+  PlaceRow p;
+  p.lo = (uint32_t)q2.x; p.hi = (uint32_t)q2.y; p.ctr = (uint32_t)q2.z; p.fin = (uint32_t)q2.w;
+  p.parent = q6.x; p.seq = (uint32_t)q6.y; p.len = q6.z; p.state = q6.w;
+  p.target = q7.x;
+  p.prio = (unsigned long long)(uint32_t)q7.z | ((unsigned long long)(uint32_t)q7.w << 32);
+  return p;
+}
+__device__ __forceinline__ void set_state(const DevWorld& W, int64_t r, int st) {
+  W.b_inh[r * BI_WORDS + BI_STATE] = st;
+}
+__device__ __forceinline__ void finalize_key(const DevWorld& W, int64_t r, PlaceRow& p, uint32_t rlo, uint32_t rhi) {
+  if ((p.fin & 1u) == 0u) return;
   int32_t* row = W.b_inh + r * BI_WORDS;
-  if ((row[BI_FINAL] & 1) == 0) return;
-  uint32_t clo, chi;
-  derive_key(W.rng[parent], W.rng[W.n + parent], W.b_seq[r], 0x1B873593U, clo, chi);
-  row[BI_RLO] = (int32_t)clo;
-  row[BI_RHI] = (int32_t)chi;
+  derive_key(rlo, rhi, p.seq, 0x1B873593U, p.lo, p.hi);
+  row[BI_RLO] = (int32_t)p.lo;
+  row[BI_RHI] = (int32_t)p.hi;
 }
 __device__ __forceinline__ void finalize_phenotype(const DevWorld& W, int64_t r) {
-  static_assert(BI_LTASK == 12 && BI_FINAL == 11 && AVGPU_NUM_LOGIC_TASKS <= 12, "row quads");
+  static_assert(BI_LTASK == 12 && BI_FINAL == 11 && AVGPU_NUM_LOGIC_TASKS <= 12 && BI_PARENT == 24 && BI_SEQ == 25,
+                "row quads");
   int32_t* row = W.b_inh + r * BI_WORDS;
   const int4* q = reinterpret_cast<const int4*>(row);
-  const int4 q0 = q[0], q1 = q[1], q2 = q[2], q3 = q[3], q4 = q[4], q5 = q[5];
-  const int parent = W.b_parent[r];
-  const int seq = (int)W.b_seq[r];
+  const int4 q0 = q[0], q1 = q[1], q2 = q[2], q3 = q[3], q4 = q[4], q5 = q[5], q6 = q[6];
+  const int parent = q6.x;
+  const int seq = q6.y;
   if ((q2.w & 1) == 0) return;
   const int nd = W.num_div[parent];
   const double merit = __hiloint2double(q0.y, q0.x);
@@ -820,21 +842,64 @@
   const double m = W.merit[c];
   return m > 0.0 ? __ddiv_rn(age, m) : age;
 }
+struct PickIn {
+  uint32_t rlo, rhi;
+  int nbr[8];
+  uint32_t valid, tk;
+};
 template <bool TILE>
-__device__ __forceinline__ bool place_pick_one(const DevWorld& W, int64_t r, int m) {
-  const int parent = W.b_parent[r];
-  if (m == 0) finalize_key(W, r, parent);
-  const unsigned long long* prev = m > 0 ? W.claim_r[m - 1] : nullptr;
-  auto taken = [&](int c) -> bool {
-    if (TILE) return tile_taken(W, c, m);
-    return W.occ[c] != 0 || (prev && prev[c] != 0ull);
+__device__ __forceinline__ PickIn pick_loads(const DevWorld& W, int parent, int m) {
+  PickIn in;
+  in.rlo = in.rhi = 0u;
+  in.valid = in.tk = 0u;
+  if (m == 0) { in.rlo = W.rng[parent]; in.rhi = W.rng[W.n + parent]; }
+  if (!TILE && W.birth_method == 4) {
+#pragma unroll
+    for (int k = 0; k < 8; k++) in.nbr[k] = parent;
+    return in;
+  }
+  in.valid = neighbours_mask(W, parent, in.nbr);
+  if (TILE) {
+#pragma unroll
+    for (int k = 0; k < 8; k++)
+      if ((in.valid >> k) & 1u) in.tk |= (tile_taken(W, in.nbr[k], m) ? 1u : 0u) << k;
+    in.tk |= (tile_taken(W, parent, m) ? 1u : 0u) << 8;
+    return in;
+  }
+  uint8_t o[9];
+  unsigned long long c[9];
+#pragma unroll
+  for (int k = 0; k < 8; k++) o[k] = W.occ[in.nbr[k]];
+  o[8] = W.occ[parent];
+#pragma unroll
+  for (int k = 0; k < 9; k++) c[k] = 0ull;
+  if (m > 0) {
+    const unsigned long long* prev = W.claim_r[m - 1];
+#pragma unroll
+    for (int k = 0; k < 8; k++) c[k] = prev[in.nbr[k]];
+    c[8] = prev[parent];
+  }
+#pragma unroll
+  for (int k = 0; k < 9; k++) in.tk |= ((o[k] != 0 || c[k] != 0ull) ? 1u : 0u) << k;
+  return in;
+}
+template <bool TILE>
+__device__ __forceinline__ bool place_pick_one(const DevWorld& W, int64_t r, int m, PlaceRow& p, const PickIn& in) {
+  int32_t* const row = W.b_inh + r * BI_WORDS;
+  const int parent = p.parent;
+  if (m == 0) finalize_key(W, r, p, in.rlo, in.rhi);
+  const uint32_t lo = p.lo, hi = p.hi;
+  uint32_t ctr = p.ctr;
+  auto no_cell = [&]() {
+    p.target = -1;
+    p.state = BS_NO_CELL - m;
+    row[BI_TARGET] = -1;
+    row[BI_STATE] = p.state;
   };
+  int t = parent;
+  bool tkn = false;
   if (!TILE && W.birth_method == 4) {
-    int32_t* const inh = W.b_inh + (int64_t)r * BI_WORDS;
-    const uint32_t lo = (uint32_t)inh[BI_RLO], hi = (uint32_t)inh[BI_RHI];
-    uint32_t ctr = (uint32_t)inh[BI_RCTR];
     const uint32_t n = (uint32_t)W.n;
-    int t = -1;
     if (W.prefer_empty) {
       const uint32_t ne = (uint32_t)W.e_blk[(W.n + 255) / 256];
       t = ne > 0u ? W.e_list[rng_below(lo, hi, ctr, ne)] : (int)rng_below(lo, hi, ctr, n);
@@ -843,64 +908,74 @@
       while (!W.allow_parent && n > 1u && t == parent) t = (int)rng_below(lo, hi, ctr, n);
     }
     if (t == parent && !W.allow_parent) {
-      inh[BI_RCTR] = (int32_t)ctr;
-      W.b_target[r] = -1;
-      W.b_state[r] = (int8_t)(BS_NO_CELL - m);
+      p.ctr = ctr;
+      row[BI_RCTR] = (int32_t)ctr;
+      no_cell();
       return false;
     }
-    const unsigned long long key = claim_key(BI_TIME(inh[BI_FINAL]), taken(t), rng_next(lo, hi, ctr),
-                                             W.cell0 + parent, W.b_seq[r]);
-    inh[BI_RCTR] = (int32_t)ctr;
-    W.b_target[r] = t;
-    W.b_prio[r] = key;
-    W.b_tgt[(int64_t)m * W.rcap + r] = t;
-    return true;
-  }
-  int nbr[8];
-  const int nn = neighbours(W, parent, nbr);
-  int cand[9];
-  int nc = 0;
-  if (W.prefer_empty)
-    for (int k = 0; k < nn; k++)
-      if (!taken(nbr[k])) cand[nc++] = nbr[k];
-  if (nc == 0 && (W.birth_method == 1 || W.birth_method == 2)) {
-    double best = W.allow_parent ? position_value(W, parent) : -1.0;
-    cand[nc++] = parent;
-    for (int k = 0; k < nn; k++) {
-      const double v = position_value(W, nbr[k]);
-      if (v > best) { best = v; nc = 0; cand[nc++] = nbr[k]; }
-      else if (v == best) cand[nc++] = nbr[k];
-    }
-  } else if (nc == 0 && W.birth_method != 3) {
-    for (int k = 0; k < nn; k++) cand[nc++] = nbr[k];
-    if (W.allow_parent) cand[nc++] = parent;
-  }
-  if (nc == 0 && !W.allow_parent) {
-    W.b_target[r] = -1;
-    W.b_state[r] = (int8_t)(BS_NO_CELL - m);
-    return false;
-  }
-  int32_t* const inh = W.b_inh + (int64_t)r * BI_WORDS;
-  const uint32_t lo = (uint32_t)inh[BI_RLO], hi = (uint32_t)inh[BI_RHI];
-  uint32_t ctr = (uint32_t)inh[BI_RCTR];
-  const int t = nc > 0 ? cand[rng_below(lo, hi, ctr, (uint32_t)nc)] : parent;
-  const unsigned long long key = claim_key(BI_TIME(inh[BI_FINAL]), taken(t), rng_next(lo, hi, ctr),
-                                           W.cell0 + parent, W.b_seq[r]);
-  inh[BI_RCTR] = (int32_t)ctr;
-  W.b_target[r] = t;
-  W.b_prio[r] = key;
+    tkn = W.occ[t] != 0 || (m > 0 && W.claim_r[m - 1][t] != 0ull);
+  } else {
+    const uint32_t nbrs = in.valid & 0xFFu;
+    uint32_t cm = W.prefer_empty ? nbrs & ~in.tk : 0u;
+    int sel = 8;
+    if (cm == 0u && (W.birth_method == 1 || W.birth_method == 2)) {
+      int cs[9];
+      int nc = 0;
+      double best = W.allow_parent ? position_value(W, parent) : -1.0;
+      cs[nc++] = 8;
+      for (int k = 0; k < 8; k++) {
+        if (!((nbrs >> k) & 1u)) continue;
+        const double v = position_value(W, in.nbr[k]);
+        if (v > best) { best = v; nc = 0; cs[nc++] = k; }
+        else if (v == best) cs[nc++] = k;
+      }
+      sel = cs[rng_below(lo, hi, ctr, (uint32_t)nc)];
+    } else {
+      if (cm == 0u && W.birth_method != 3) cm = nbrs | (W.allow_parent ? 0x100u : 0u);
+      if (cm == 0u) {
+        if (!W.allow_parent) { no_cell(); return false; }
+      } else {
+        const int j = (int)rng_below(lo, hi, ctr, (uint32_t)__popc(cm));
+        int cnt = 0;
+#pragma unroll
+        for (int k = 0; k < 9; k++)
+          if ((cm >> k) & 1u) { if (cnt == j) sel = k; cnt++; }
+      }
+    }
+    tkn = ((in.tk >> 8) & 1u) != 0u;
+#pragma unroll
+    for (int k = 0; k < 8; k++)
+      if (sel == k) { t = in.nbr[k]; tkn = ((in.tk >> k) & 1u) != 0u; }
+  }
+  const unsigned long long key = claim_key(BI_TIME(p.fin), tkn, rng_next(lo, hi, ctr), W.cell0 + parent, p.seq);
+  p.ctr = ctr;
+  p.target = t;
+  p.prio = key;
+  row[BI_RCTR] = (int32_t)ctr;
+  *reinterpret_cast<int4*>(row + BI_TARGET) = make_int4(t, 0, (int)(uint32_t)key, (int)(uint32_t)(key >> 32));
   W.b_tgt[(int64_t)m * W.rcap + r] = t;
   return true;
 }
 
-#define QUEUE_LOOP(i) \
-  for (int64_t i = (int64_t)blockIdx.x * blockDim.x + threadIdx.x, _qn = queue_len(W); i < _qn; \
-       i += (int64_t)gridDim.x * blockDim.x)
+__device__ __forceinline__ int list_entry(const DevWorld& W, int64_t i) { return W.b_list[i < W.n ? i : W.n - 1]; }
+__device__ __forceinline__ int64_t rec_from(const DevWorld& W, int64_t i, int64_t p, int64_t e) {
+  return i < p ? e : W.n + (i - p);
+}
+#define QUEUE_RECS(i, r, first, stride) \
+  for (int64_t i = (first), _qs = (stride), _e = list_entry(W, i), _p = W.b_count[BQ_PRIMARY], \
+               _qn = queue_len(W), r = rec_from(W, i, _p, _e); \
+       i < _qn; i += _qs, _e = i < _qn ? list_entry(W, i) : 0, r = rec_from(W, i, _p, _e))
+#define QUEUE_LOOP(i, r) \
+  QUEUE_RECS(i, r, (int64_t)blockIdx.x * blockDim.x + threadIdx.x, (int64_t)gridDim.x * blockDim.x)
 __device__ __forceinline__ bool soup_free(const DevWorld& W, int64_t c, int m) {
   return c < W.n && W.occ[c] == 0 && (m == 0 || W.claim_r[m - 1][c] == 0ull);
 }
+__device__ __forceinline__ bool soup_round_skipped(const DevWorld& W, int m) {
+  return m > 1 && W.b_count[BQ_PICKED + m - 1] == 0;
+}
 __global__ __launch_bounds__(256) void k_empty_count(DevWorld W, int m) {
   __shared__ int ws[4];
+  if (soup_round_skipped(W, m)) return;
   const int64_t c = (int64_t)blockIdx.x * 256 + threadIdx.x;
   const bool e = soup_free(W, c, m);
   const int cnt = __popcll(__ballot(e));
@@ -908,8 +983,9 @@
   __syncthreads();
   if (threadIdx.x == 0) W.e_blk[blockIdx.x] = ws[0] + ws[1] + ws[2] + ws[3];
 }
-__global__ __launch_bounds__(1024) void k_empty_scan(DevWorld W, int nb) {
+__global__ __launch_bounds__(1024) void k_empty_scan(DevWorld W, int nb, int m) {
   __shared__ int part[1024];
+  if (soup_round_skipped(W, m)) return;
   const int per = (nb + 1023) / 1024;
   const int b0 = (int)threadIdx.x * per, b1 = min(nb, b0 + per);
   int sum = 0;
@@ -932,6 +1008,7 @@
 }
 __global__ __launch_bounds__(256) void k_empty_scatter(DevWorld W, int m) {
   __shared__ int ws[4];
+  if (soup_round_skipped(W, m)) return;
   const int lane = threadIdx.x & 63, wv = threadIdx.x >> 6;
   const int64_t c = (int64_t)blockIdx.x * 256 + threadIdx.x;
   const bool e = soup_free(W, c, m);
@@ -949,18 +1026,22 @@
                                                uint8_t (*child)[TAPE_SLOT + 16]) {
   __shared__ int ml[MUT_PER_BLOCK][8];
   __shared__ int mn;
+  const int lane = threadIdx.x & 63, wv = threadIdx.x >> 6;
+  int64_t le = lane < MUT_PER_WAVE ? list_entry(W, blk * MUT_PER_BLOCK + wv * MUT_PER_WAVE + lane) : 0;
+  const int64_t np = W.b_count[BQ_PRIMARY];
   const int nb = queue_len(W);
-  const int lane = threadIdx.x & 63, wv = threadIdx.x >> 6;
   for (int64_t q0 = blk * MUT_PER_BLOCK; q0 < nb; q0 += nblk * MUT_PER_BLOCK) {
     if (threadIdx.x == 0) mn = 0;
     __syncthreads();
     const int64_t q = q0 + wv * MUT_PER_WAVE + lane;
+    const int64_t r = rec_from(W, q, np, le);
+    const int64_t qx = q + nblk * MUT_PER_BLOCK;
+    le = (lane < MUT_PER_WAVE && qx < nb) ? list_entry(W, qx) : 0;
     if (lane < MUT_PER_WAVE && q < nb) {
-      const int64_t r = rec_of(W, q);
       int e[5];
 #pragma unroll
       for (int k = 0; k < 5; k++) e[k] = W.b_edit[(int64_t)k * W.rcap + r];
-      const int l0 = W.b_len0[r], l1 = W.b_len[r];
+      const int l0 = W.b_len0[r], l1 = W.b_inh[r * BI_WORDS + BI_LEN];
       int x = e[0] | e[1] | e[2] | e[3] | e[4];
       if (W.seg_any)
         for (int k = 0; k < NSEG; k++) x |= W.b_pcnt[(int64_t)k * W.rcap + r];
@@ -984,21 +1065,43 @@
 }
 
 __global__ void k_place_round(DevWorld W, int m) {
+  if (m > 1 && W.b_count[BQ_PICKED + m - 1] == 0) return;
   const unsigned long long* prev = W.claim_r[m - 1];
   unsigned long long* cur = W.claim_r[m];
-  QUEUE_LOOP(q) {
-    const int64_t r = rec_of(W, q);
-    if (W.b_state[r] != BS_PENDING) continue;
-    const int t = W.b_target[r];
-    const unsigned long long key = W.b_prio[r];
-    if (prev[t] == key) {
-      W.b_state[r] = (int8_t)(BS_WON + m - 1);
-      W.occ[t] = 1;
-      if (takes_cell(W, W.owner[t], rec_time(W, r))) W.owner[t] = (int)r;
-      continue;
-    }
-    if (key_kill(key)) { W.b_state[r] = (int8_t)(BS_KILL_LOST + m - 1); continue; }
-    if (place_pick_one<false>(W, r, m)) atomicMax(&cur[W.b_target[r]], W.b_prio[r]);
+  const int lane = threadIdx.x & 63;
+  const int64_t stride = (int64_t)gridDim.x * blockDim.x;
+  int64_t le = list_entry(W, (int64_t)blockIdx.x * blockDim.x + threadIdx.x);
+  const int64_t np = W.b_count[BQ_PRIMARY];
+  for (int64_t q0 = (int64_t)blockIdx.x * blockDim.x + threadIdx.x - lane, qn = queue_len(W); q0 < qn;
+       q0 += stride) {
+    const int64_t q = q0 + lane;
+    const int64_t r = rec_from(W, q, np, le);
+    le = q + stride < qn ? list_entry(W, q + stride) : 0;
+    bool picked = false;
+    do {
+      if (q >= qn) break;
+      PlaceRow p = place_row(W, r);
+      const bool pend = p.state == BS_PENDING;
+      const int t = pend && p.target >= 0 ? p.target : 0;
+      const unsigned long long pv = prev[t];
+      const int own = W.owner[t];
+      if (!pend) break;
+      const unsigned long long key = p.prio;
+      if (pv == key) {
+        set_state(W, r, BS_WON + m - 1);
+        W.occ[t] = 1;
+        if (takes_cell(W, own, BI_TIME(p.fin))) W.owner[t] = (int)r;
+        break;
+      }
+      if (key_kill(key)) { set_state(W, r, BS_KILL_LOST + m - 1); break; }
+      const PickIn in = pick_loads<false>(W, p.parent, m);
+      if (place_pick_one<false>(W, r, m, p, in)) {
+        atomicMax(&cur[p.target], p.prio);
+        picked = true;
+      }
+    } while (0);
+    const unsigned long long bm = __ballot(picked);
+    if (bm && lane == 0) atomicAdd(&W.b_count[BQ_PICKED + m], (int)__popcll(bm));
   }
 }
 __global__ void k_place_claim0(DevWorld W, long long* pred_out, long long pred_seq) {
@@ -1010,30 +1113,29 @@
     __threadfence_system();
     __hip_atomic_store(pred_out + PRED_SEQ, pred_seq, __ATOMIC_RELAXED, __HIP_MEMORY_SCOPE_SYSTEM);
   }
-  QUEUE_LOOP(q) {
-    const int64_t r = rec_of(W, q);
-    if (W.b_state[r] != BS_PENDING) continue;
-    const int p = W.b_parent[r];
-    if (W.killt[p] > 0x10000u - rec_time(W, r)) { W.b_state[r] = BS_CANCELLED; continue; }
-    atomicMax(&W.claim_r[0][W.b_target[r]], W.b_prio[r]);
+  QUEUE_LOOP(q, r) {
+    const PlaceRow p = place_row(W, r);
+    const uint32_t kt = W.killt[p.parent];
+    if (p.state != BS_PENDING) continue;
+    if (kt > 0x10000u - BI_TIME(p.fin)) { set_state(W, r, BS_CANCELLED); continue; }
+    atomicMax(&W.claim_r[0][p.target], p.prio);
   }
 }
 __global__ __launch_bounds__(256) void k_place_pick_mut(DevWorld W, int pblocks, int fblocks, int boff, int nblocks) {
   __shared__ uint8_t child[4][TAPE_SLOT + 16];
-  const int nb = queue_len(W);
   const int bid = (int)blockIdx.x + boff;
   if (bid < pblocks) {
-    for (int64_t i = (int64_t)bid * 256 + threadIdx.x; i < nb; i += (int64_t)pblocks * 256) {
-      const int64_t r = rec_of(W, i);
-      if (!place_pick_one<false>(W, r, 0)) continue;
-      const unsigned long long key = W.b_prio[r];
-      if (key_kill(key)) atomicMax(&W.killt[W.b_target[r]], 0x10000u - key_time(key));
+    QUEUE_RECS(i, r, (int64_t)bid * 256 + threadIdx.x, (int64_t)pblocks * 256) {
+      PlaceRow p = place_row(W, r);
+      const PickIn in = pick_loads<false>(W, p.parent, 0);
+      if (!place_pick_one<false>(W, r, 0, p, in)) continue;
+      if (key_kill(p.prio)) atomicMax(&W.killt[p.target], 0x10000u - key_time(p.prio));
     }
     return;
   }
   if (bid < pblocks + fblocks) {
-    for (int64_t i = (int64_t)(bid - pblocks) * 256 + threadIdx.x; i < nb; i += (int64_t)fblocks * 256)
-      finalize_phenotype(W, rec_of(W, i));
+    QUEUE_RECS(i, r, (int64_t)(bid - pblocks) * 256 + threadIdx.x, (int64_t)fblocks * 256)
+      finalize_phenotype(W, r);
     return;
   }
   pblocks += fblocks;
@@ -1044,9 +1146,8 @@
 __global__ __launch_bounds__(256) void k_tile_prep(DevWorld W, int mblocks, int fblocks) {
   __shared__ uint8_t child[4][TAPE_SLOT + 16];
   if ((int)blockIdx.x >= mblocks && (int)blockIdx.x < mblocks + fblocks) {
-    const int nb = queue_len(W);
-    for (int64_t i = (int64_t)(blockIdx.x - mblocks) * 256 + threadIdx.x; i < nb; i += (int64_t)fblocks * 256)
-      finalize_phenotype(W, rec_of(W, i));
+    QUEUE_RECS(i, r, (int64_t)(blockIdx.x - mblocks) * 256 + threadIdx.x, (int64_t)fblocks * 256)
+      finalize_phenotype(W, r);
     return;
   }
   if ((int)blockIdx.x < mblocks) {
@@ -1072,15 +1173,15 @@
 __global__ __launch_bounds__(256) void k_tile_round(DevWorld W, int m, int rblocks) {
   const int X = W.world_x;
   if ((int)blockIdx.x < rblocks) {
-    const int nb = queue_len(W);
-    for (int64_t q = (int64_t)blockIdx.x * blockDim.x + threadIdx.x; q < nb; q += (int64_t)rblocks * blockDim.x) {
-      const int64_t r = rec_of(W, q);
-      if (W.b_state[r] != BS_PENDING) continue;
+    QUEUE_RECS(q, r, (int64_t)blockIdx.x * blockDim.x + threadIdx.x, (int64_t)rblocks * blockDim.x) {
+      PlaceRow p = place_row(W, r);
+      if (p.state != BS_PENDING) continue;
       if (m == 0) {
-        if (!place_pick_one<true>(W, r, 0)) continue;
-        const unsigned long long key = W.b_prio[r];
+        const PickIn in = pick_loads<true>(W, p.parent, 0);
+        if (!place_pick_one<true>(W, r, 0, p, in)) continue;
+        const unsigned long long key = p.prio;
         if (!key_kill(key)) continue;
-        const int t = W.b_target[r];
+        const int t = p.target;
         const uint32_t kv = 0x10000u - key_time(key);
         if (t >= W.n) {
           const int64_t k = t - W.n;
@@ -1091,18 +1192,21 @@
         }
         continue;
       }
-      const int t = W.b_target[r];
-      const unsigned long long key = W.b_prio[r];
+      const int t = p.target;
+      const unsigned long long key = p.prio;
+      const int own = W.owner[t];
       if (tile_merged(W, t, m - 1) == key) {
-        W.b_state[r] = (int8_t)(BS_WON + m - 1);
+        set_state(W, r, BS_WON + m - 1);
         W.occ[t] = 1;
-        if (takes_cell(W, W.owner[t], rec_time(W, r))) W.owner[t] = (int)r;
+        if (takes_cell(W, own, BI_TIME(p.fin))) W.owner[t] = (int)r;
         continue;
       }
-      if (key_kill(key)) { W.b_state[r] = (int8_t)(BS_KILL_LOST + m - 1); continue; }
-      if (m < 4 && place_pick_one<true>(W, r, m)) {
-        const int nt = W.b_target[r];
-        const unsigned long long nk = W.b_prio[r];
+      if (key_kill(key)) { set_state(W, r, BS_KILL_LOST + m - 1); continue; }
+      if (m >= 4) continue;
+      const PickIn in = pick_loads<true>(W, p.parent, m);
+      if (place_pick_one<true>(W, r, m, p, in)) {
+        const int nt = p.target;
+        const unsigned long long nk = p.prio;
         atomicMax(&W.claim_r[m][nt], nk);
         int d, x;
         bool ghost;
@@ -1148,17 +1252,17 @@
 __global__ __launch_bounds__(256) void k_tile_claim0(DevWorld W) {
   const int X = W.world_x;
   if (blockIdx.x == 0 && threadIdx.x < NUM_LISTS) W.class_count[threadIdx.x] = 0;
-  QUEUE_LOOP(q) {
-    const int64_t r = rec_of(W, q);
-    if (W.b_state[r] != BS_PENDING) continue;
-    const int p = W.b_parent[r];
+  QUEUE_LOOP(q, r) {
+    const PlaceRow pr = place_row(W, r);
+    const int p = pr.parent;
     uint32_t kt = W.killt[p];
+    if (pr.state != BS_PENDING) continue;
     int d, x;
     bool ghost;
     if (halo_slot(W, p, d, x, ghost)) kt = max(kt, halo_kt(W.h_recv[d], X)[x]);
-    if (kt > 0x10000u - rec_time(W, r)) { W.b_state[r] = BS_CANCELLED; continue; }
-    const int t = W.b_target[r];
-    const unsigned long long key = W.b_prio[r];
+    if (kt > 0x10000u - BI_TIME(pr.fin)) { set_state(W, r, BS_CANCELLED); continue; }
+    const int t = pr.target;
+    const unsigned long long key = pr.prio;
     atomicMax(&W.claim_r[0][t], key);
     if (halo_slot(W, t, d, x, ghost)) atomicMax(&halo_cl(W.h_send[d], X, 0, ghost ? 0 : 1)[x], key);
   }
@@ -1216,27 +1320,40 @@
 #define ACT_PRE 8
 #endif
 __global__ __launch_bounds__(64) void k_activate(DevWorld W, int fused, uint32_t key, int sub, int nsub) {
+  const int lane = threadIdx.x & 63;
+  int64_t le = list_entry(W, (int64_t)blockIdx.x * 64 + lane);
+  const int64_t np = W.b_count[BQ_PRIMARY];
   const int nb = queue_len(W);
   const int64_t ncell = W.n + (W.tiled ? 2 * (int64_t)W.world_x : 0);
-  const int lane = threadIdx.x & 63;
   const double total = W.totals[TOT_DIV];
   const long long uds = sub_share((long long)W.totals[TOT_UD], sub, nsub);
   unsigned long long born = 0, over = 0, canc = 0, nocell = 0, bad = 0, wasted = 0, nbs = 0;
   long long carry = 0;
   for (int64_t q0 = (int64_t)blockIdx.x * 64; q0 < nb; q0 += (int64_t)gridDim.x * 64) {
     const int64_t q = q0 + lane;
+    const int64_t i = rec_from(W, q, np, le);
+    le = q + (int64_t)gridDim.x * 64 < nb ? list_entry(W, q + (int64_t)gridDim.x * 64) : 0;
     int nrow = -1, ncell_nb = 0;
     do {
       if (q >= nb) break;
-      const int64_t i = rec_of(W, q);
       const uint4* g4 = reinterpret_cast<const uint4*>(W.b_genome + i * TAPE_SLOT);
       uint4 pre[ACT_PRE];
 #pragma unroll
       for (int u = 0; u < ACT_PRE; u++) pre[u] = g4[u];
-      const int tgt = W.b_target[i];
-      const int8_t st = W.b_state[i];
-      Child b = child_of_record(W, i);
-      const int ran = (tgt >= 0 && (int64_t)tgt < W.n) ? W.ran[tgt] : 0;
+      static_assert(BI_LTASK == 12 && AVGPU_NUM_LOGIC_TASKS <= 12 && BI_STATE == 27 && BI_TARGET == 28 && BI_PRIO == 30,
+                    "row quads");
+      const int4* rq = reinterpret_cast<const int4*>(W.b_inh + i * BI_WORDS);
+      const int4 q0 = rq[0], q1 = rq[1], q2 = rq[2], q3 = rq[3], q4 = rq[4], q5 = rq[5], q6 = rq[6], q7 = rq[7];
+      const int tgt = q7.x;
+      const int st = q6.w;
+      const unsigned long long prio = (unsigned long long)(uint32_t)q7.z | ((unsigned long long)(uint32_t)q7.w << 32);
+      Child b = child_of_row(W, i, q0, q1, q2, q6);
+      const int lt[12] = {q3.x, q3.y, q3.z, q3.w, q4.x, q4.y, q4.z, q4.w, q5.x, q5.y, q5.z, q5.w};
+      const bool tin = tgt >= 0 && (int64_t)tgt < ncell;
+      const int64_t tl = tin ? tgt : 0;
+      const int ran = (tin && (int64_t)tgt < W.n) ? W.ran[tl] : 0;
+      const unsigned long long c3 = W.claim_r[3][tl];
+      const int own = W.owner[tl];
       const int lastr = last_claim_round(st);
       bool ok = true;
       for (int k = 0; k <= lastr && k < 3; k++) {
@@ -1250,19 +1367,18 @@
       const uint32_t t = 0x10000u - b.hs;
       bool won = false;
       if (fused == ACT_STRIP) {
-        won = st >= BS_WON && st < BS_WON + 4 && W.owner[tgt] == (int)i;
+        won = st >= BS_WON && st < BS_WON + 4 && own == (int)i;
       } else if (st == BS_PENDING) {
-        won = W.claim_r[3][tgt] == W.b_prio[i] && takes_cell(W, W.owner[tgt], t);
+        won = c3 == prio && takes_cell(W, own, t);
       } else if (st >= BS_WON && st < BS_WON + 4) {
-        const unsigned long long c3 = W.claim_r[3][tgt];
-        won = W.owner[tgt] == (int)i && !(c3 != 0ull && key_time(c3) >= t);
+        won = own == (int)i && !(c3 != 0ull && key_time(c3) >= t);
       }
       if (!won) { over++; break; }
       if (b.len < 0 || b.len > AVGPU_MAX_GENOME) { bad++; break; }
       if (tgt >= W.n) break;
       born++;
       b.hs = 0;
-      setup_child_lane<ACT_PRE>(W, tgt, b, W.b_genome + i * TAPE_SLOT, pre);
+      setup_child_lane<ACT_PRE>(W, tgt, b, W.b_genome + i * TAPE_SLOT, pre, lt);
       nrow = newborn_setup(W, tgt, t, b.merit, b.len, key, uds, total, carry, wasted, ran);
       ncell_nb = tgt;
     } while (0);
@@ -1301,17 +1417,18 @@
     int64_t mine = -1;
     if (q < nb) {
       const int64_t i = rec_of(W, q);
-      const int tgt = W.b_target[i];
-      const int8_t st = W.b_state[i];
+      const PlaceRow p = place_row(W, i);
+      const int tgt = p.target, st = p.state;
       if (st >= BS_WON && st < BS_WON + 4 && tgt >= W.n && (int64_t)tgt < W.n + 2 * (int64_t)X &&
-          W.b_len[i] >= 0 && W.b_len[i] <= AVGPU_MAX_GENOME && W.owner[tgt] == (int)i)
+          p.len >= 0 && p.len <= AVGPU_MAX_GENOME && W.owner[tgt] == (int)i)
         mine = i;
     }
     for (unsigned long long m = __ballot(mine >= 0); m; m &= m - 1ull) {
     const int64_t i = (int64_t)__shfl((long long)mine, __ffsll((long long)m) - 1);
-    const int tgt = W.b_target[i];
+    const PlaceRow pi = place_row(W, i);
+    const int tgt = pi.target;
     const int d = (tgt - (int)W.n) / X, col = (tgt - (int)W.n) - d * X;
-    const int len = W.b_len[i];
+    const int len = pi.len;
     HaloHdr* hdr = reinterpret_cast<HaloHdr*>(W.r_send[d]);
     HaloRec* recs = reinterpret_cast<HaloRec*>(W.r_send[d] + sizeof(HaloHdr));
     uint8_t* arena = W.r_send[d] + sizeof(HaloHdr) + (int64_t)X * sizeof(HaloRec);
@@ -1325,7 +1442,7 @@
     const bool fits = (int64_t)off + len <= W.r_arena;
     if (lane == 0) {
       HaloRec r;
-      r.col = col; r.round = W.b_state[i] - BS_WON; r.len = fits ? len : -1;
+      r.col = col; r.round = pi.state - BS_WON; r.len = fits ? len : -1;
       const Child b = child_of_record(W, i);
       r.gen = b.gen; r.ccopied = b.ccopied; r.exec = b.exec; r.gest = b.gest;
       r.rng_lo = b.lo; r.rng_hi = b.hi; r.rng_ctr = b.ctr;
@@ -1670,7 +1787,7 @@
   auto soup_cells = [&](int m) {
     const int eb = (int)nblk(W.n, 256);
     hipLaunchKernelGGL(k_empty_count, dim3(eb), dim3(256), 0, s, W, m);
-    hipLaunchKernelGGL(k_empty_scan, dim3(1), dim3(1024), 0, s, W, eb);
+    hipLaunchKernelGGL(k_empty_scan, dim3(1), dim3(1024), 0, s, W, eb, m);
     hipLaunchKernelGGL(k_empty_scatter, dim3(eb), dim3(256), 0, s, W, m);
   };
   if (soup) soup_cells(0);
```

Result: faster. 25.32 billion organism-instructions/s, median of 6 (+1.4%).
